# georgeliu233/STrajNet

Measured on AMD Instinct MI355X. Metric: scenes/sec (fwd+bwd, 256x256 grids), higher is better.
Workload: dtype bf16; 1 GPU; STrajNet cfg-256 train step (fwd+OGMFlow_loss+bwd+Nadam), batch 8/GPU, 8 waypoints, obs+occ+flow heads, fg_msa+fg, random-init weights; global_batch=8, grid=256x256x11, parallelism=dp1, hipgraph=True, concurrent_branch_streams=True, optimizer_in_step=True, settle_steps=40

## Files before the change

include/strajnet_hip.h:

```cpp
#ifndef STRAJNET_HIP_H
#define STRAJNET_HIP_H
#include <hip/hip_runtime_api.h>
#ifdef __cplusplus
extern "C" {
#endif

enum stj_status { STJ_OK = 0, STJ_EINVAL = -1, STJ_ELAUNCH = -2, STJ_EUNSUPPORTED = -3 };
enum stj_dtype { STJ_F32 = 0, STJ_BF16 = 1, STJ_F16 = 2 };
enum stj_act { STJ_ACT_NONE = 0, STJ_ACT_GELU = 1, STJ_ACT_ELU = 2 };
enum stj_unary { STJ_U_GELU = 1, STJ_U_ELU = 2, STJ_U_TANH_SCALE = 3 };

const char* stj_last_error(void);
int stj_abi_version(void);

int stj_gemm(const void* A, const void* B, void* C, const float* bias, const void* res, float* colsum,
             int M, int N, int K, int nb1, int nb2,
             long long sAb1, long long sAb2, long long sAm, long long sAk,
             long long sBb1, long long sBb2, long long sBk, long long sBn,
             long long sCb1, long long sCb2, long long ldc,
             long long sBias1, long long sBias2, long long sRes1, long long sRes2, long long ldres,
             int act, float alpha, int dtype, int c_f32, int accumulate, int splitk,
             int nkb, long long sAkb, long long sBkb, void* group, hipStream_t stream);
long long stj_gemm_group_workspace_bytes(void);
int stj_gemm_group_begin(void* group);
// ... 146 lines not shown
  void* dq;
  float* d_w1; float* d_gamma; float* d_beta; float* d_bias;
} stj_fgoff_args;
int stj_fgoff_supported(int H, int W, int C, int G, int dtype);
long long stj_fgoff_pack_workspace_bytes(int dtype);
int stj_fgoff_pack(const float* w, void* out, int dtype, hipStream_t stream);
int stj_fgoff_fwd(const stj_fgoff_args* a, hipStream_t stream);
int stj_fgoff_bwd(const stj_fgoff_args* a, hipStream_t stream);
int stj_fg_bias_fwd(const void* off, const float* table, float* bias, int B, int G, int Hh, int Ww, int dtype, hipStream_t stream);
int stj_fg_bias_bwd(const void* off, const float* table, const void* dbias, float* dtable, float* doff,
                    int B, int G, int Hh, int Ww, int dtype, hipStream_t stream);
int stj_fg_attn_fwd(const void* q, const void* k, const void* v, const void* off, const float* table, void* a, float* lse, int B, int G,
                    int Hh, int Ww, float scale, int dtype, hipStream_t stream);
long long stj_fg_attn_bwd_workspace_bytes(int B, int G, int Hh, int Ww);
int stj_fg_attn_bwd(const void* q, const void* k, const void* v, const void* off, const float* table, const void* a, const float* lse,
                    const void* da, void* dq, void* dk, void* dv, float* dkp, float* dvp, float* dtable, float* doff, int B, int G,
                    int Hh, int Ww, float scale, int dtype, hipStream_t stream);
int stj_fg_offset_fwd(const void* o, const void* W1, const void* W2, const float* b2, const void* qres, void* off, void* fh,
                      int B, int HW, int G, int gc, int C2, float scale, int zmajor, int dtype, hipStream_t stream);
int stj_fg_offset_bwd(const void* o, const void* off, const void* W1, const void* W2, const void* doff, const void* dfh,
                      void* dO, void* dq, void* doff_out, float* dW1, float* dW2, float* db2, int B, int HW, int G, int gc,
                      int C2, float scale, int zmajor, int dtype, hipStream_t stream);

int stj_upconv_prep(const float* W, void* Wf, void* Wd, int Cin, int Cout, int dtype, hipStream_t stream);
int stj_upconv_fold(const float* dWeff, float* dW, int Cin, int Cout, hipStream_t stream);
int stj_upconv_fwd(const void* X, const void* Wf, const float* bias, void* Y, int F, int Hi, int Wi, int Cin,
                   int Cout, int act, int dtype, hipStream_t stream);
int stj_upconv_fwd_res(const void* X, const void* Wf, const float* bias, void* Y, const void* R1, void* Y2, const void* R2, int F, int Hi,
                       int Wi, int Cin, int Cout, int dtype, hipStream_t stream);
int stj_elu_res_bwd(const void* dy, const void* dy2, const void* y, const void* r, void* dpre, void* gsum, long long n, int dtype,
                    hipStream_t stream);
int stj_skip_junction_bwd(const void* dy1, const void* dy2, const void* y, const void* r1, const void* r2, void* dpre, void* dr1,
                          void* dr2, long long n, int dtype, hipStream_t stream);
int stj_upconv_dgrad(const void* dP, const void* Wd, void* dX, const void* Xelu, int F, int Hi, int Wi, int Cin, int Cout,
                     int dtype, hipStream_t stream);
int stj_upconv_wgrad(const void* X, const void* dP, float* dWeff, float* dbias, int db_parts, int F, int Hi, int Wi, int Cin,
                     int Cout, int wg_budget, int dtype, hipStream_t stream);
int stj_outconv_fwd(const void* X, const float* W, const float* bias, float* Y, int F, int Hh, int Ww, int C, int Tn,
                    long long y_bstride, long long y_tstride, long long y_pstride, int dtype, hipStream_t stream);
int stj_outconv_pair_fwd(const void* X0, const void* X1, const float* W0, const float* W1, const float* bias0, const float* bias1,
                         float* Y, int B, int Tn, int H, int W, int C, int t_major, int dtype, hipStream_t stream);
int stj_upconv_fwd_head(const void* X, const void* Wf, const float* bias, const float* Whead, void* Z, int F, int Hi, int Wi, int Cin,
                        int Cout, int dtype, hipStream_t stream);
int stj_outconv_pair_gather(const void* Z0, const void* Z1, const float* bias0, const float* bias1, float* Y, int B, int Tn, int H, int W,
                            int t_major, int dtype, hipStream_t stream);
int stj_quantize_waypoints(const float* Y, uint8_t* Q, int B, int Tn, int H, int W, hipStream_t stream);
int stj_outconv_pair_gather_q(const void* Z0, const void* Z1, const float* bias0, const float* bias1, uint8_t* Q, int B, int Tn, int H,
                              int W, int t_major, int dtype, hipStream_t stream);
int stj_compress_sizes(int B, int Tn, int H, int W, long long* work_bytes, long long* out_capacity);
int stj_compress_waypoints(const uint8_t* Q, void* work, uint8_t* out, uint32_t* offsets, int B, int Tn, int H, int W, hipStream_t stream);
int stj_compress_waypoints_level(const uint8_t* Q, void* work, uint8_t* out, uint32_t* offsets, int B, int Tn, int H, int W, int level,
                                 hipStream_t stream);
int stj_outconv_bwd(const void* X, const float* W, const float* dY, void* dX, float* dW, float* db, int F, int Hh, int Ww,
                    int C, int Tn, long long y_bstride, long long y_tstride, long long y_pstride, int elu_in, void* ws,
                    long long ws_bytes, int dtype, hipStream_t stream);
long long stj_outconv_bwd_workspace_bytes(void);
int stj_im2col_patch(const float* src, void* dst, int B, int H, int W, int Cin, long long pix_stride, int ch_stride,
                     int dtype, hipStream_t stream);
int stj_patch_embed_supported(int Cin, int Cout, int dtype);
int stj_patch_embed_fwd(const float* src, const void* w, const float* bias, const float* gamma, const float* beta, const void* add,
                        const float* gamma2, const float* beta2, void* cols, void* pre, void* x2, void* y, float* mean, float* rstd,
                        float* mean2, float* rstd2, int B, int H, int W, int Cin, long long pix_stride, int ch_stride, int Cout,
                        float eps, int dtype, hipStream_t stream);
int stj_im2col3(const void* x, void* cols, int N, int H, int W, int G, int Cg, int dtype, hipStream_t stream);
int stj_col2im3(const void* dcols, void* dx, int N, int H, int W, int G, int Cg, int dtype, hipStream_t stream);

int stj_loss_auc_gate(const float* gt_obs, const float* gt_occ, const float* gt_flow, const float* origin,
                      int* hist, float* gate, float* auc_out, int B, int H, int W, hipStream_t stream);
int stj_loss_fwd(const float* logits, const float* gt_obs, const float* gt_occ, const float* gt_flow, const float* origin,
                 const float* gate, float* sums, float* loss, float* coef, int B, int H, int W, float ogm_w, float occ_w,
                 float flow_origin_w, float replica, int flags, hipStream_t stream);
int stj_loss_bwd(const float* logits, const float* gt_obs, const float* gt_occ, const float* gt_flow, const float* origin,
                 const float* coef, const float* upstream, float* dlogits, int B, int H, int W, int flags, hipStream_t stream);
int stj_loss_coef(const float* gt_flow, const float* gate, int* cnt, float* coef, int B, int H, int W, float ogm_w, float occ_w,
                  float flow_origin_w, float replica, int flags, hipStream_t stream);
int stj_loss_finalize(const float* sums, const float* gate, float* loss, float* coef_out, int B, int H, int W, float ogm_w,
                      float occ_w, float flow_origin_w, float replica, int flags, hipStream_t stream);
int stj_loss_gate_coef(const float* gt_obs, const float* gt_occ, const float* gt_flow, const float* origin, int* hist, float* gate,
                       float* auc_out, float* coef, int B, int H, int W, float ogm_w, float occ_w, float flow_origin_w,
                       float replica, int flags, hipStream_t stream);
int stj_loss_fwd_bwd(const float* logits, const float* gt_obs, const float* gt_occ, const float* gt_flow, const float* origin,
                     const float* gate, const float* coef_in, float* sums, float* loss, float* coef_out, float* dlogits,
                     int B, int H, int W, float ogm_w, float occ_w, float flow_origin_w, float replica, int flags, hipStream_t stream);

int stj_decode_raw(const void* src, int kind, float* dst, long long n_outer, int H, int W, int C, int y0, int x0, int Ho,
                   int Wo, float scale, hipStream_t stream);

int stj_unpack_bits(const uint32_t* bits, float* dst, long long n_total, hipStream_t stream);
int stj_unpack_sparse(const uint32_t* mask, const uint32_t* offs, const uint32_t* val_base, const float* vals, long long n_vals,
                      float* dst, int B, long long n, hipStream_t stream);

int stj_gather_bits(const uint32_t* pool, const int* idx, int N, float* dst, int B, long long n, hipStream_t stream);
int stj_gather_sparse(const uint32_t* mask, const uint32_t* offs, const long long* val_base, const float* vals, long long n_vals,
                      const int* idx, int N, float* dst, int B, long long n, hipStream_t stream);
int stj_gather_raw(const void* pool, int kind, const int* idx, int N, float* dst, int B, long long n, float scale, hipStream_t stream);

int stj_pack_bits(const uint8_t* src, const int* ok, const int* slots, int N, uint32_t* pool_words, int B, int T, int H, int W, int C, int y0,
                  int x0, int Ho, int Wo, hipStream_t stream);
int stj_pack_sparse_count(const float* src, uint32_t* offs_stage, int B, int T, int H, int W, int C, int y0, int x0, int Ho, int Wo,
                          hipStream_t stream);
int stj_pool_admit(uint32_t* offs_stage, int nblk, const long long* val_base, const int* slots, int N, int* ok, int B, int first,
                   hipStream_t stream);
int stj_pack_sparse_commit(const float* src, const uint32_t* offs_stage, const int* ok, const int* slots, int N, uint32_t* mask_pool,
                           uint32_t* offs_pool, const long long* val_base, float* vals, long long n_vals, int B, int T, int H, int W, int C,
                           int y0, int x0, int Ho, int Wo, hipStream_t stream);
int stj_pool_put_raw(const void* src, int itemsize, const int* ok, const int* slots, int N, void* pool, int B, long long n, hipStream_t stream);

int stj_pool_draw(int* perm, int N, int tail, int n_live, const uint32_t* u, int* idx, int B, hipStream_t stream);
int stj_pool_admit_packed(const uint32_t* offs_src, int nblk, long long n, const long long* src_base, const long long* val_base,
                          const int* slots, int N, int* ok, int B, int first, hipStream_t stream);
int stj_pool_put_vals(const uint32_t* vals_src, const long long* src_base, const int* ok, const int* slots, int N,
                      const long long* val_base, uint32_t* vals, long long n_vals, int B, hipStream_t stream);

int stj_agent_prep(const float* obs, const float* occ, int n_obs, int n_occ, int B, int Tn, void* x5, void* v3, int* vt, int* cmi,
                   void* cmf, int dtype, hipStream_t stream);
int stj_agent_mix_fwd(const void* enc, const void* embed, const void* cm, void* concat, void* qin, int B, int A, int C, int dtype,
                      hipStream_t stream);
int stj_agent_mix_bwd(const void* dconcat, const void* dqin, const void* cm, void* denc, void* dembed, int B, int A, int C, int dtype,
                      hipStream_t stream);
int stj_agent_sum_fwd(const void* enc, const void* value, const void* embed, void* out, int B, int A, int C, int dtype, hipStream_t stream);
int stj_agent_sum_bwd(const void* dout, void* dembed, int B, int A, int C, int dtype, hipStream_t stream);
int stj_agent_out_fwd(const void* enc, const void* value, const void* embed, const float* g0, const float* b0, const float* g1, const float* b1,
                      void* out, void* y, float* mean, float* rstd, int B, int A, int n0, int C, float eps, int dtype, hipStream_t stream);
int stj_agent_out_bwd(const void* dy, const void* out, const float* mean, const float* rstd, const float* g0, const float* g1, void* dout,
                      void* dembed, float* dg0, float* db0, float* dg1, float* db1, int B, int A, int n0, int C, int dtype, hipStream_t stream);
int stj_time_collapse(const float* W, void* Wz, long long n, int dtype, hipStream_t stream);
int stj_time_fold(const float* dWz, float* dW, long long n, hipStream_t stream);
int stj_fold_parts(float* g, const long long* idx, float* parts, long long n, hipStream_t stream);

int stj_crc32c(const void* data, long long n, unsigned int* crc);

int stj_metrics(const float* pred, const float* gt_obs, const float* gt_occ, const float* gt_flow, const float* origin,
                int* hist, float* sums, float* auc, float* out, int B, int H, int W, int pred_is_logits, int use_warp,
                hipStream_t stream);

long long stj_eval_workspace_bytes(int B, int H, int W);
int stj_eval_fwd(const float* logits, const float* gt_obs, const float* gt_occ, const float* gt_flow, const float* origin,
                 void* workspace, float* loss, float* metrics, float* gate, float* auc, double* running, int B, int H, int W,
                 float ogm_w, float occ_w, float flow_origin_w, float replica, float loss_scale, int flags, hipStream_t stream);

int stj_rng_advance(long long* state, hipStream_t stream);
int stj_rng_advance_snap(long long* state, long long* snap, hipStream_t stream);
int stj_dropout(const void* x, const void* res, void* y, long long n, long long inner, float p, const long long* state,
                int site, int dtype, hipStream_t stream);
int stj_dropout_mask(unsigned char* mask, long long ndraw, float p, const long long* state, int site, hipStream_t stream);
int stj_nadam_step(float* w, const float* g, float* m, float* v, long long n, float lr, float b1, float b2, float eps,
                   float cg, float cm, float vhat_scale, float gscale, hipStream_t stream);

enum stj_optim { STJ_GRADNORM_PARTS = 256, STJ_SCHED_CONSTANT = 0, STJ_SCHED_COSINE_RESTARTS = 1, STJ_SCHED_CUSTOM = 2,
                 STJ_NADAM_SKIP_NONFINITE = 1, STJ_TENSOR_CHUNK = 4096, STJ_TENSOR_GRID = 1024 };
int stj_gradnorm_partials(const float* g, long long n, double* partials, hipStream_t stream);
int stj_nadam_prepare(double* state, const double* sched, const double* partials, float* coef, const float* losses, double* running,
                      float b1, float b2, float gscale, float clipnorm, float loss_scale, int flags, hipStream_t stream);
int stj_nadam_apply(float* w, const float* g, float* m, float* v, long long n, const float* coef, float b1, float b2, float eps,
                    hipStream_t stream);

int stj_tensor_partials(const float* g, long long n, const int* chunks, int n_chunks, int S, double* gpart, hipStream_t stream);
int stj_nadam_prepare_tensors(double* state, const double* sched, const double* gpart, const int* chunk0, int n_chunks, int S, float* coef,
                              float* mult, double* tsum, int* nfcount, const float* losses, double* running, float b1, float b2,
                              float gscale, float global_clipnorm, float clipnorm, float loss_scale, int flags, hipStream_t stream);
int stj_nadam_apply_tensors(float* w, const float* g, float* m, float* v, long long n, const int* chunks, int n_chunks, int S,
                            const float* coef, const float* mult, float b1, float b2, float eps, hipStream_t stream);

#ifdef __cplusplus
}
#endif
#endif
```

strajnet_amd/csrc/loss.hip:

```cpp
#include "loss_pixel.h"

#define LOSS_PARTS 32
enum { S_OBS = 0, S_OCC = 1, S_L1 = 2, S_EX = 3, S_WARP = 4, S_N = 5 };

__global__ __launch_bounds__(256) void auc_hist_kernel(const float* gt_obs, const float* gt_occ, const float* gt_flow,
                                                       const float* origin, int* hist, int* cnt, int B, int H, int W) {
  __shared__ int sh[2 * 101 + 1];
  const int k = blockIdx.y;
  for (int i = threadIdx.x; i < 203; i += 256) sh[i] = 0;
  __syncthreads();
  int nex = 0;
  const long long npix = (long long)B * H * W;
  for (long long i = blockIdx.x * 256ll + threadIdx.x; i < npix; i += gridDim.x * 256ll) {
    const int x = (int)(i % W); long long t = i / W;
    const int y = (int)(t % H); const long long b = t / H;
    const long long g = ((b * NWP + k) * H + y) * W + x;
    const float ta = fminf(fmaxf(gt_obs[g] + gt_occ[g], 0.f), 1.f);
    const float* img = origin + (b * NWP + k) * (long long)H * W;
    const float fx = gt_flow[2 * g], fy = gt_flow[2 * g + 1];
    nex += (fx != 0.f || fy != 0.f) ? 1 : 0;
    const float wp = warp_sample(img, H, W, (float)x + fx, (float)y + fy, nullptr, nullptr);
    const float pred = wp * ta;
    const int bk = auc_bucket(pred);
    atomicAdd(&sh[(ta != 0.f ? 101 : 0) + bk], 1);
  }
  if (cnt) {
#pragma unroll
    for (int o = 32; o > 0; o >>= 1) nex += __shfl_xor(nex, o, 64);
    if ((threadIdx.x & 63) == 0 && nex) atomicAdd(&sh[202], nex);
  }
  __syncthreads();
  for (int i = threadIdx.x; i < 202; i += 256)
    if (sh[i]) atomicAdd(hist + k * 202 + i, sh[i]);
  if (cnt && threadIdx.x == 0 && sh[202]) atomicAdd(cnt + k, sh[202]);
}
__global__ __launch_bounds__(128) void auc_gate_kernel(const int* hist, float* gate, float* auc_out) {
  __shared__ AucScratch s;
  const int k = blockIdx.x;
  const double auc = auc_pr_block(hist + k * 202, s);
  if (threadIdx.x == 0) {
    if (gate) gate[k] = ((1.0 - auc) < 1.0) ? 1.f : 0.f;
    if (auc_out) auc_out[k] = (float)auc;
  }
}

template <bool FOCAL, bool PRED>
__global__ __launch_bounds__(256) void loss_fwd_kernel(const float* logits, const float* gt_obs, const float* gt_occ,
                                                       const float* gt_flow, const float* origin, float* sums,
                                                       int B, int H, int W, int use_warp) {
  __shared__ float red[4][NWP * S_N];
  const float inv_hw = 1.f / ((float)H * (float)W);
  float acc[S_N];
#pragma unroll
  for (int i = 0; i < S_N; ++i) acc[i] = 0.f;
  const long long nitem = (long long)B * H * W * NWP;
  const int k = threadIdx.x & 7;
  for (long long it = blockIdx.x * 256ll + threadIdx.x; it < nitem; it += gridDim.x * 256ll) {
    const long long i = it >> 3;
    const int x = (int)(i % W); long long t = i / W;
    const int y = (int)(t % H); const long long b = t / H;
    const float4 lg = reinterpret_cast<const float4*>(logits)[it];
    const long long g = ((b * NWP + k) * H + y) * W + x;
    const float to = gt_obs[g], tc = gt_occ[g];
    const float2 fl = reinterpret_cast<const float2*>(gt_flow)[g];
    const float fx = fl.x, fy = fl.y;
    acc[S_OBS] += FOCAL ? xe_focal_logits(to, lg.x, nullptr) : xe_logits(to, lg.x);
    acc[S_OCC] += FOCAL ? xe_focal_logits(tc, lg.y, nullptr) : xe_logits(tc, lg.y);
    const float ex = (fx != 0.f || fy != 0.f) ? 1.f : 0.f;
    acc[S_L1] += (fabsf(fx - lg.z) + fabsf(fy - lg.w)) * ex;
    acc[S_EX] += ex;
    if (use_warp) {
      const float* img = origin + (b * NWP + k) * (long long)H * W;
      const float wp = warp_sample(img, H, W, (float)x + lg.z, (float)y + lg.w, nullptr, nullptr);
      const float sg = PRED ? fminf(fmaxf(sigmoidf(lg.x) + sigmoidf(lg.y), 0.f), 1.f)
                            : fminf(fmaxf(sigmoidf(to) + sigmoidf(tc), 0.f), 1.f);
      const float ta = fminf(fmaxf(to + tc, 0.f), 1.f);
      acc[S_WARP] += warp_term<FOCAL, PRED>(ta, sg * wp, inv_hw, nullptr);
    }
  }
  const int lane = threadIdx.x & 63, w = threadIdx.x >> 6;
#pragma unroll
  for (int i = 0; i < S_N; ++i) {
    float v = acc[i];
    v += __shfl_xor(v, 8, 64); v += __shfl_xor(v, 16, 64); v += __shfl_xor(v, 32, 64);
    if (lane < 8) red[w][lane * S_N + i] = v;
  }
  __syncthreads();
  if (threadIdx.x < NWP * S_N)
    atomicAdd(sums + (blockIdx.x % LOSS_PARTS) * (NWP * S_N) + threadIdx.x, red[0][threadIdx.x] + red[1][threadIdx.x] + red[2][threadIdx.x] + red[3][threadIdx.x]);
}

struct LossCfg { float ogm_w, occ_w, fow, replica; int use_warp; };

__global__ void loss_finalize_kernel(const float* sums_parts, int nparts, const float* gate, float* loss, float* coef, float npix, LossCfg c) {
  __shared__ float sums[NWP * S_N], part[6][NWP * S_N];
  if (threadIdx.x < 6 * NWP * S_N) {
    const int slot = threadIdx.x % (NWP * S_N), j = threadIdx.x / (NWP * S_N);
    float a = 0.f;
#pragma unroll 8
    for (int q = j; q < nparts; q += 6) a += sums_parts[q * (NWP * S_N) + slot];
    part[j][slot] = a;
  }
  __syncthreads();
  if (threadIdx.x < NWP * S_N) {
    const int t = threadIdx.x;
    sums[t] = ((((part[0][t] + part[1][t]) + part[2][t]) + part[3][t]) + part[4][t]) + part[5][t];
  }
  __syncthreads();
  if (threadIdx.x != 0) return;
  float so = 0.f, sc = 0.f, sf = 0.f, sw = 0.f, fc = 0.f;
  for (int k = 0; k < NWP; ++k) fc += gate[k];
  for (int k = 0; k < NWP; ++k) {
    const float* s = sums + k * S_N;
    so += c.ogm_w * s[S_OBS] / (npix * c.replica);
    sc += c.occ_w * s[S_OCC] / (npix * c.replica);
    const float den = s[S_EX] * c.replica / 2.f;
    const float fl = den != 0.f ? s[S_L1] / den : 0.f;
    sf += gate[k] * fl;
    sw += gate[k] * c.fow * s[S_WARP] / (npix * c.replica);
    coef[k * 4 + 0] = c.ogm_w / (npix * c.replica) / NWP;
    coef[k * 4 + 1] = c.occ_w / (npix * c.replica) / NWP;
    coef[k * 4 + 2] = den != 0.f ? gate[k] / fc / den : 0.f;
    coef[k * 4 + 3] = c.use_warp ? gate[k] / fc * c.fow / (npix * c.replica) : 0.f;
  }
  loss[0] = so / NWP;
  loss[1] = sc / NWP;
  loss[2] = sf / fc;
  loss[3] = c.use_warp ? sw / fc : 0.f;
  loss[4] = loss[0] + loss[1] + loss[2] + loss[3];
}

template <bool FOCAL, bool PRED>
__global__ __launch_bounds__(256) void loss_bwd_kernel(const float* logits, const float* gt_obs, const float* gt_occ,
                                                       const float* gt_flow, const float* origin, const float* coef,
                                                       const float* up, float* dlogits, int B, int H, int W, int use_warp, int up1) {
  const int k = threadIdx.x & 7;
  const float c0 = coef[4 * k] * up[0], c1 = coef[4 * k + 1] * up[up1 ? 0 : 1], c2 = coef[4 * k + 2] * up[up1 ? 0 : 2], c3 = coef[4 * k + 3] * up[up1 ? 0 : 3];
  const long long nitem = (long long)B * H * W * NWP;
  const float inv_hw = 1.f / ((float)H * (float)W);
  for (long long it = blockIdx.x * 256ll + threadIdx.x; it < nitem; it += gridDim.x * 256ll) {
    const long long i = it >> 3;
    const int x = (int)(i % W); long long t = i / W;
    const int y = (int)(t % H); const long long b = t / H;
    const float4 lg = reinterpret_cast<const float4*>(logits)[it];
    const long long g = ((b * NWP + k) * H + y) * W + x;
    const float to = gt_obs[g], tc = gt_occ[g];
    const float2 fl = reinterpret_cast<const float2*>(gt_flow)[g];
    const float fx = fl.x, fy = fl.y;
    float g0, g1;
    if (FOCAL) { xe_focal_logits(to, lg.x, &g0); xe_focal_logits(tc, lg.y, &g1); }
    else { g0 = sigmoidf(lg.x) - to; g1 = sigmoidf(lg.y) - tc; }
    g0 *= c0; g1 *= c1;
    const float ex = (fx != 0.f || fy != 0.f) ? 1.f : 0.f;
    const float d0 = fx - lg.z, d1 = fy - lg.w;
    float g2 = -c2 * ex * (d0 > 0.f ? 1.f : (d0 < 0.f ? -1.f : 0.f));
    float g3 = -c2 * ex * (d1 > 0.f ? 1.f : (d1 < 0.f ? -1.f : 0.f));
    if (use_warp && c3 != 0.f) {
      const float* img = origin + (b * NWP + k) * (long long)H * W;
      float ddx, ddy;
      const float wp = warp_sample(img, H, W, (float)x + lg.z, (float)y + lg.w, &ddx, &ddy);
      const float sa = sigmoidf(PRED ? lg.x : to), sb = sigmoidf(PRED ? lg.y : tc);
      const float ssum = sa + sb;
      const float sg = fminf(fmaxf(ssum, 0.f), 1.f);
      const float ta = fminf(fmaxf(to + tc, 0.f), 1.f);
      float dq;
      warp_term<FOCAL, PRED>(ta, sg * wp, inv_hw, &dq);
      dq *= c3;
      g2 += dq * sg * ddx;
      g3 += dq * sg * ddy;
      if (PRED && ssum <= 1.f) {
        g0 += dq * wp * sa * (1.f - sa);
        g1 += dq * wp * sb * (1.f - sb);
      }
    }
    reinterpret_cast<float4*>(dlogits)[it] = make_float4(g0, g1, g2, g3);
  }
}

#define LOSS_PARTS_FUSED 128
#ifndef LOSS_FB_MAXG
#define LOSS_FB_MAXG 16384
#endif
template <bool FOCAL, bool PRED>
__global__ __launch_bounds__(256) void loss_fwd_bwd_kernel(const float* logits, const float* gt_obs, const float* gt_occ,
                                                           const float* gt_flow, const float* origin, const float* coef,
                                                           float* sums, float* dlogits, int B, int H, int W, int use_warp) {
  __shared__ float red[4][NWP * S_N];
  const float inv_hw = 1.f / ((float)H * (float)W);
  float acc[S_N];
#pragma unroll
  for (int i = 0; i < S_N; ++i) acc[i] = 0.f;
  const long long nitem = (long long)B * H * W * NWP;
  const int k = threadIdx.x & 7;
  const float c0 = coef[4 * k], c1 = coef[4 * k + 1], c2 = coef[4 * k + 2], c3 = coef[4 * k + 3];
  for (long long it = blockIdx.x * 256ll + threadIdx.x; it < nitem; it += gridDim.x * 256ll) {
    const long long i = it >> 3;
    const int x = (int)(i % W); long long t = i / W;
    const int y = (int)(t % H); const long long b = t / H;
    const float4 lg = reinterpret_cast<const float4*>(logits)[it];
    const long long g = ((b * NWP + k) * H + y) * W + x;
    const float to = gt_obs[g], tc = gt_occ[g];
    const float2 fl = reinterpret_cast<const float2*>(gt_flow)[g];
    const float fx = fl.x, fy = fl.y;
    float g0, g1;
    if (FOCAL) { acc[S_OBS] += xe_focal_logits(to, lg.x, &g0); acc[S_OCC] += xe_focal_logits(tc, lg.y, &g1); }
    else {
      acc[S_OBS] += xe_logits(to, lg.x); acc[S_OCC] += xe_logits(tc, lg.y);
      g0 = sigmoidf(lg.x) - to; g1 = sigmoidf(lg.y) - tc;
    }
    g0 *= c0; g1 *= c1;
    const float ex = (fx != 0.f || fy != 0.f) ? 1.f : 0.f;
    const float d0 = fx - lg.z, d1 = fy - lg.w;
    acc[S_L1] += (fabsf(d0) + fabsf(d1)) * ex;
    acc[S_EX] += ex;
    float g2 = -c2 * ex * (d0 > 0.f ? 1.f : (d0 < 0.f ? -1.f : 0.f));
    float g3 = -c2 * ex * (d1 > 0.f ? 1.f : (d1 < 0.f ? -1.f : 0.f));
    if (use_warp) {
      const float* img = origin + (b * NWP + k) * (long long)H * W;
      float ddx, ddy;
      const float wp = warp_sample(img, H, W, (float)x + lg.z, (float)y + lg.w, &ddx, &ddy);
      const float sa = sigmoidf(PRED ? lg.x : to), sb = sigmoidf(PRED ? lg.y : tc);
      const float ssum = sa + sb;
      const float sg = fminf(fmaxf(ssum, 0.f), 1.f);
      const float ta = fminf(fmaxf(to + tc, 0.f), 1.f);
      float dq;
      acc[S_WARP] += warp_term<FOCAL, PRED>(ta, sg * wp, inv_hw, &dq);
      if (c3 != 0.f) {
        dq *= c3;
        g2 += dq * sg * ddx;
        g3 += dq * sg * ddy;
        if (PRED && ssum <= 1.f) {
          g0 += dq * wp * sa * (1.f - sa);
          g1 += dq * wp * sb * (1.f - sb);
        }
      }
    }
    reinterpret_cast<float4*>(dlogits)[it] = make_float4(g0, g1, g2, g3);
  }
  const int lane = threadIdx.x & 63, w = threadIdx.x >> 6;
#pragma unroll
  for (int i = 0; i < S_N; ++i) {
    float v = acc[i];
    v += __shfl_xor(v, 8, 64); v += __shfl_xor(v, 16, 64); v += __shfl_xor(v, 32, 64);
    if (lane < 8) red[w][lane * S_N + i] = v;
  }
  __syncthreads();
  if (threadIdx.x < NWP * S_N)
    atomicAdd(sums + (blockIdx.x % LOSS_PARTS_FUSED) * (NWP * S_N) + threadIdx.x, red[0][threadIdx.x] + red[1][threadIdx.x] + red[2][threadIdx.x] + red[3][threadIdx.x]);
}

template <bool VEC4>
__global__ __launch_bounds__(256) void loss_flow_count_kernel(const float* gt_flow, int* cnt, long long plane) {
  __shared__ int red[4];
  const int k = blockIdx.y % NWP;
  const float* fp = gt_flow + (long long)blockIdx.y * plane * 2;
  int n = 0;
  if (VEC4) {
    const float4* f = reinterpret_cast<const float4*>(fp);
    for (long long i = blockIdx.x * 256ll + threadIdx.x; i < plane / 2; i += gridDim.x * 256ll) {
      const float4 v = f[i];
      n += ((v.x != 0.f || v.y != 0.f) ? 1 : 0) + ((v.z != 0.f || v.w != 0.f) ? 1 : 0);
    }
  } else {
    const float2* f = reinterpret_cast<const float2*>(fp);
    for (long long i = blockIdx.x * 256ll + threadIdx.x; i < plane; i += gridDim.x * 256ll) {
      const float2 v = f[i];
      n += (v.x != 0.f || v.y != 0.f) ? 1 : 0;
    }
  }
#pragma unroll
  for (int o = 32; o > 0; o >>= 1) n += __shfl_xor(n, o, 64);
  if ((threadIdx.x & 63) == 0) red[threadIdx.x >> 6] = n;
  __syncthreads();
  if (threadIdx.x == 0) { const int s = red[0] + red[1] + red[2] + red[3]; if (s) atomicAdd(cnt + k, s); }
}
__global__ void loss_coef_kernel(const int* cnt, const float* gate, float* coef, float npix, LossCfg c) {
  if (threadIdx.x != 0) return;
  float fc = 0.f;
  for (int k = 0; k < NWP; ++k) fc += gate[k];
  for (int k = 0; k < NWP; ++k) {
    const float den = (float)cnt[k] * c.replica / 2.f;
    coef[k * 4 + 0] = c.ogm_w / (npix * c.replica) / NWP;
    coef[k * 4 + 1] = c.occ_w / (npix * c.replica) / NWP;
    coef[k * 4 + 2] = den != 0.f ? gate[k] / fc / den : 0.f;
    coef[k * 4 + 3] = c.use_warp ? gate[k] / fc * c.fow / (npix * c.replica) : 0.f;
  }
}

extern "C" int stj_loss_auc_gate(const float* gt_obs, const float* gt_occ, const float* gt_flow, const float* origin,
                                 int* hist, float* gate, float* auc_out, int B, int H, int W, hipStream_t stream) {
  const long long npix = (long long)B * H * W;
  const int gx = (int)min(256ll, (npix + 255) / 256);
  hipLaunchKernelGGL(auc_hist_kernel, dim3(gx, NWP), dim3(256), 0, stream, gt_obs, gt_occ, gt_flow, origin, hist, (int*)nullptr, B, H, W);
  hipLaunchKernelGGL(auc_gate_kernel, dim3(NWP), dim3(128), 0, stream, hist, gate, auc_out);
  return stj_check_launch("stj_loss_auc_gate");
}
extern "C" int stj_loss_fwd(const float* logits, const float* gt_obs, const float* gt_occ, const float* gt_flow, const float* origin,
                            const float* gate, float* sums, float* loss, float* coef, int B, int H, int W, float ogm_w, float occ_w,
                            float flow_origin_w, float replica, int flags, hipStream_t stream) {
  if (((uintptr_t)logits) & 15) { stj_set_error("loss: logits must be 16-byte aligned"); return STJ_EINVAL; }
  if (((uintptr_t)gt_flow) & 7) { stj_set_error("loss: gt_flow must be 8-byte aligned"); return STJ_EINVAL; }
  if (flags & ~7) { stj_set_error("loss: unknown flag bits %d", flags); return STJ_EINVAL; }
  const long long npix = (long long)B * H * W;
  const int gx = (int)min(4096ll, (npix * NWP + 255) / 256);
  const int use_warp = flags & 1, focal = (flags >> 1) & 1, pred = (flags >> 2) & 1;
#define LOSS_FWD(FO, PR) hipLaunchKernelGGL((loss_fwd_kernel<FO, PR>), dim3(gx), dim3(256), 0, stream, logits, gt_obs, gt_occ, gt_flow, origin, sums, B, H, W, use_warp)
  if (focal && pred) LOSS_FWD(true, true); else if (focal) LOSS_FWD(true, false); else if (pred) LOSS_FWD(false, true); else LOSS_FWD(false, false);
#undef LOSS_FWD
  LossCfg c; c.ogm_w = ogm_w; c.occ_w = occ_w; c.fow = flow_origin_w; c.replica = replica; c.use_warp = use_warp;
  hipLaunchKernelGGL(loss_finalize_kernel, dim3(1), dim3(256), 0, stream, sums, LOSS_PARTS, gate, loss, coef, (float)npix, c);
  return stj_check_launch("stj_loss_fwd");
}
extern "C" int stj_loss_bwd(const float* logits, const float* gt_obs, const float* gt_occ, const float* gt_flow, const float* origin,
                            const float* coef, const float* upstream, float* dlogits, int B, int H, int W, int flags, hipStream_t stream) {
  if (flags & ~15) { stj_set_error("loss: unknown flag bits %d", flags); return STJ_EINVAL; }
  if ((((uintptr_t)logits) | ((uintptr_t)dlogits)) & 15) { stj_set_error("loss: logits / dlogits must be 16-byte aligned"); return STJ_EINVAL; }
  if (((uintptr_t)gt_flow) & 7) { stj_set_error("loss: gt_flow must be 8-byte aligned"); return STJ_EINVAL; }
  const long long npix = (long long)B * H * W;
  const int gx = (int)min(8192ll, (npix * NWP + 255) / 256);
  const int use_warp = flags & 1, focal = (flags >> 1) & 1, pred = (flags >> 2) & 1;
#define LOSS_BWD(FO, PR) hipLaunchKernelGGL((loss_bwd_kernel<FO, PR>), dim3(gx), dim3(256), 0, stream, logits, gt_obs, gt_occ, gt_flow, origin, coef, upstream, dlogits, B, H, W, use_warp, (flags >> 3) & 1)
  if (focal && pred) LOSS_BWD(true, true); else if (focal) LOSS_BWD(true, false); else if (pred) LOSS_BWD(false, true); else LOSS_BWD(false, false);
#undef LOSS_BWD
  return stj_check_launch("stj_loss_bwd");
}

extern "C" int stj_loss_coef(const float* gt_flow, const float* gate, int* cnt, float* coef, int B, int H, int W, float ogm_w, float occ_w,
                             float flow_origin_w, float replica, int flags, hipStream_t stream) {
  if (((uintptr_t)gt_flow) & 7) { stj_set_error("loss: gt_flow must be 8-byte aligned"); return STJ_EINVAL; }
  if (flags & ~7) { stj_set_error("loss: unknown flag bits %d", flags); return STJ_EINVAL; }
  const long long plane = (long long)H * W;
  if (B > 0 && plane > 0) {
    const int gx = (int)min(16ll, (plane / 2 + 255) / 256);
    if (plane % 2 == 0 && (((uintptr_t)gt_flow) & 15) == 0)
      hipLaunchKernelGGL(loss_flow_count_kernel<true>, dim3(gx, B * NWP), dim3(256), 0, stream, gt_flow, cnt, plane);
    else
      hipLaunchKernelGGL(loss_flow_count_kernel<false>, dim3(gx, B * NWP), dim3(256), 0, stream, gt_flow, cnt, plane);
  }
  LossCfg c; c.ogm_w = ogm_w; c.occ_w = occ_w; c.fow = flow_origin_w; c.replica = replica; c.use_warp = flags & 1;
  hipLaunchKernelGGL(loss_coef_kernel, dim3(1), dim3(64), 0, stream, cnt, gate, coef, (float)((long long)B * H * W), c);
  return stj_check_launch("stj_loss_coef");
}
extern "C" int stj_loss_gate_coef(const float* gt_obs, const float* gt_occ, const float* gt_flow, const float* origin, int* hist, float* gate,
                                  float* auc_out, float* coef, int B, int H, int W, float ogm_w, float occ_w, float flow_origin_w,
                                  float replica, int flags, hipStream_t stream) {
  if (flags & ~7) { stj_set_error("loss: unknown flag bits %d", flags); return STJ_EINVAL; }
  const long long npix = (long long)B * H * W;
  const int gx = (int)min(256ll, (npix + 255) / 256);
  int* cnt = hist + NWP * 202;
  if (gx > 0) hipLaunchKernelGGL(auc_hist_kernel, dim3(gx, NWP), dim3(256), 0, stream, gt_obs, gt_occ, gt_flow, origin, hist, cnt, B, H, W);
  hipLaunchKernelGGL(auc_gate_kernel, dim3(NWP), dim3(128), 0, stream, hist, gate, auc_out);
  LossCfg c; c.ogm_w = ogm_w; c.occ_w = occ_w; c.fow = flow_origin_w; c.replica = replica; c.use_warp = flags & 1;
  hipLaunchKernelGGL(loss_coef_kernel, dim3(1), dim3(64), 0, stream, cnt, gate, coef, (float)npix, c);
  return stj_check_launch("stj_loss_gate_coef");
}
extern "C" int stj_loss_fwd_bwd(const float* logits, const float* gt_obs, const float* gt_occ, const float* gt_flow, const float* origin,
                                const float* gate, const float* coef_in, float* sums, float* loss, float* coef_out, float* dlogits,
                                int B, int H, int W, float ogm_w, float occ_w, float flow_origin_w, float replica, int flags,
                                hipStream_t stream) {
  if ((((uintptr_t)logits) | ((uintptr_t)dlogits)) & 15) { stj_set_error("loss: logits / dlogits must be 16-byte aligned"); return STJ_EINVAL; }
  if (((uintptr_t)gt_flow) & 7) { stj_set_error("loss: gt_flow must be 8-byte aligned"); return STJ_EINVAL; }
  if (flags & ~7) { stj_set_error("loss: unknown flag bits %d", flags); return STJ_EINVAL; }
  const long long npix = (long long)B * H * W;
  const int gx = (int)min((long long)LOSS_FB_MAXG, (npix * NWP + 255) / 256);
  const int use_warp = flags & 1, focal = (flags >> 1) & 1, pred = (flags >> 2) & 1;
  if (gx > 0) {
#define LOSS_FB(FO, PR) hipLaunchKernelGGL((loss_fwd_bwd_kernel<FO, PR>), dim3(gx), dim3(256), 0, stream, logits, gt_obs, gt_occ, gt_flow, origin, coef_in, sums, dlogits, B, H, W, use_warp)
    if (focal && pred) LOSS_FB(true, true); else if (focal) LOSS_FB(true, false); else if (pred) LOSS_FB(false, true); else LOSS_FB(false, false);
#undef LOSS_FB
  }
  if (loss == nullptr) return stj_check_launch("stj_loss_fwd_bwd");
  LossCfg c; c.ogm_w = ogm_w; c.occ_w = occ_w; c.fow = flow_origin_w; c.replica = replica; c.use_warp = use_warp;
  hipLaunchKernelGGL(loss_finalize_kernel, dim3(1), dim3(256), 0, stream, sums, LOSS_PARTS_FUSED, gate, loss, coef_out, (float)npix, c);
  return stj_check_launch("stj_loss_fwd_bwd");
}
extern "C" int stj_loss_finalize(const float* sums, const float* gate, float* loss, float* coef_out, int B, int H, int W, float ogm_w,
                                 float occ_w, float flow_origin_w, float replica, int flags, hipStream_t stream) {
  if (flags & ~7) { stj_set_error("loss: unknown flag bits %d", flags); return STJ_EINVAL; }
  LossCfg c; c.ogm_w = ogm_w; c.occ_w = occ_w; c.fow = flow_origin_w; c.replica = replica; c.use_warp = flags & 1;
  hipLaunchKernelGGL(loss_finalize_kernel, dim3(1), dim3(256), 0, stream, sums, LOSS_PARTS_FUSED, gate, loss, coef_out, (float)((long long)B * H * W), c);
  return stj_check_launch("stj_loss_finalize");
}


enum { M_IO = 0, M_TO, M_PO, M_IC, M_TC, M_PC, M_EPE, M_EX, M_IW, M_TW, M_PW, M_N };
__global__ __launch_bounds__(256) void metrics_kernel(const float* pred, const float* gt_obs, const float* gt_occ, const float* gt_flow,
                                                      const float* origin, int* hist, float* sums, int B, int H, int W,
                                                      int pred_is_logits, int use_warp) {
  __shared__ int sh[3 * 202];
  __shared__ float red[4][M_N];
  const int k = blockIdx.y;
  for (int i = threadIdx.x; i < 3 * 202; i += 256) sh[i] = 0;
  __syncthreads();
  float acc[M_N];
#pragma unroll
  for (int i = 0; i < M_N; ++i) acc[i] = 0.f;
  const long long npix = (long long)B * H * W;
  for (long long i = blockIdx.x * 256ll + threadIdx.x; i < npix; i += gridDim.x * 256ll) {
    const int x = (int)(i % W); long long t = i / W;
    const int y = (int)(t % H); const long long b = t / H;
    const float4 q = reinterpret_cast<const float4*>(pred + i * 32)[k];
    const float po = pred_is_logits ? sigmoidf(q.x) : q.x, pc = pred_is_logits ? sigmoidf(q.y) : q.y;
    const long long g = ((b * NWP + k) * H + y) * W + x;
    const float to = gt_obs[g], tc = gt_occ[g];
    const float fx = gt_flow[2 * g], fy = gt_flow[2 * g + 1];
    atomicAdd(&sh[0 * 202 + (to != 0.f ? 101 : 0) + auc_bucket(po)], 1);
    atomicAdd(&sh[1 * 202 + (tc != 0.f ? 101 : 0) + auc_bucket(pc)], 1);
    acc[M_IO] += po * to; acc[M_TO] += to; acc[M_PO] += po;
    acc[M_IC] += pc * tc; acc[M_TC] += tc; acc[M_PC] += pc;
    const float ex = (fx != 0.f || fy != 0.f) ? 1.f : 0.f;
    const float dx = (fx - q.z) * ex, dy = (fy - q.w) * ex;
    acc[M_EPE] += sqrtf(dx * dx + dy * dy);
    acc[M_EX] += ex;
    if (use_warp) {
      const float* img = origin + (b * NWP + k) * (long long)H * W;
      const float wp = warp_sample(img, H, W, (float)x + q.z, (float)y + q.w, nullptr, nullptr);
      const float ta = fminf(fmaxf(to + tc, 0.f), 1.f);
      const float fg = fminf(fmaxf(po + pc, 0.f), 1.f) * wp;
      atomicAdd(&sh[2 * 202 + (fg != 0.f ? 101 : 0) + auc_bucket(ta)], 1);
      acc[M_IW] += ta * fg; acc[M_TW] += fg; acc[M_PW] += ta;
    }
  }
  const int lane = threadIdx.x & 63, w = threadIdx.x >> 6;
#pragma unroll
  for (int i = 0; i < M_N; ++i) {
    const float s = wave_sum(acc[i]);
    if (lane == 0) red[w][i] = s;
  }
  __syncthreads();
  if (threadIdx.x < M_N) atomicAdd(sums + k * M_N + threadIdx.x, red[0][threadIdx.x] + red[1][threadIdx.x] + red[2][threadIdx.x] + red[3][threadIdx.x]);
  for (int i = threadIdx.x; i < 3 * 202; i += 256)
    if (sh[i]) atomicAdd(hist + (k * 3 + i / 202) * 202 + i % 202, sh[i]);
}
__global__ void metrics_finalize_kernel(const float* auc, const float* sums, float* out, int use_warp) {
  if (threadIdx.x != 0) return;
  float m[7] = {0.f, 0.f, 0.f, 0.f, 0.f, 0.f, 0.f};
  for (int k = 0; k < NWP; ++k) {
    const float* s = sums + k * M_N;
    auto iou = [](float i, float t, float p) { const float d = p + t - i; return d != 0.f ? i / d : 0.f; };
    m[0] += auc[k * 3 + 0]; m[1] += auc[k * 3 + 1];
    m[2] += iou(s[M_IO], s[M_TO], s[M_PO]); m[3] += iou(s[M_IC], s[M_TC], s[M_PC]);
    m[4] += s[M_EX] != 0.f ? s[M_EPE] / s[M_EX] : 0.f;
    if (use_warp) { m[5] += auc[k * 3 + 2]; m[6] += iou(s[M_IW], s[M_TW], s[M_PW]); }
  }
  for (int i = 0; i < 7; ++i) out[i] = m[i] / NWP;
}
extern "C" int stj_metrics(const float* pred, const float* gt_obs, const float* gt_occ, const float* gt_flow, const float* origin,
                           int* hist, float* sums, float* auc, float* out, int B, int H, int W, int pred_is_logits, int use_warp,
                           hipStream_t stream) {
  if (((uintptr_t)pred) & 15) { stj_set_error("metrics: pred must be 16-byte aligned"); return STJ_EINVAL; }
  const long long npix = (long long)B * H * W;
  if (npix <= 0) return STJ_OK;
  const int gx = (int)min(256ll, (npix + 255) / 256);
  hipLaunchKernelGGL(metrics_kernel, dim3(gx, NWP), dim3(256), 0, stream, pred, gt_obs, gt_occ, gt_flow, origin, hist, sums, B, H, W, pred_is_logits, use_warp);
  hipLaunchKernelGGL(auc_gate_kernel, dim3(NWP * 3), dim3(128), 0, stream, hist, (float*)nullptr, auc);
  hipLaunchKernelGGL(metrics_finalize_kernel, dim3(1), dim3(64), 0, stream, auc, sums, out, use_warp);
  return stj_check_launch("stj_metrics");
// ... 2 lines not shown
```

strajnet_amd/csrc/nadam.h:

```cpp
#pragma once

__device__ __forceinline__ void nadam_update(float& w, float g, float& m, float& v, float lr, float b1, float b2, float eps, float cg,
                                             float cm, float vhat_scale, float gscale) {
  const float gg = g * gscale;
  m = b1 * m + (1.f - b1) * gg;
  v = b2 * v + (1.f - b2) * gg * gg;
  w -= lr * (cg * gg + cm * m) / (sqrtf(v * vhat_scale) + eps);
}
```

strajnet_amd/csrc/optim.hip:

```cpp
#include "common.h"
#include "nadam.h"
#include "optim_dev.h"

#define GRADNORM_THREADS 512
static_assert(STJ_GRADNORM_PARTS == 256, "nadam_prepare_kernel folds one partial per thread of its 256");

__global__ __launch_bounds__(GRADNORM_THREADS) void gradnorm_partials_kernel(const float* __restrict__ g, long long n,
                                                                             double* __restrict__ partials) {
  __shared__ double red[GRADNORM_THREADS / 64];
  const long long nv = n / 4;
  double s = 0.0;
#pragma unroll 4
  for (long long i = blockIdx.x * (long long)GRADNORM_THREADS + threadIdx.x; i < nv; i += gridDim.x * (long long)GRADNORM_THREADS) {
    const float4 G = reinterpret_cast<const float4*>(g)[i];
    s += (double)G.x * (double)G.x + (double)G.y * (double)G.y + (double)G.z * (double)G.z + (double)G.w * (double)G.w;
  }
  if (blockIdx.x == 0 && threadIdx.x < (n & 3)) {
    const double x = g[nv * 4 + threadIdx.x];
    s += x * x;
  }
  s = block_sum_f64<GRADNORM_THREADS / 64>(s, red);
  if (threadIdx.x == 0) partials[blockIdx.x] = s;
}

__global__ __launch_bounds__(256) void nadam_prepare_kernel(double* __restrict__ state, const double* __restrict__ sched,
                                                            const double* __restrict__ partials, float* __restrict__ coef,
                                                            const float* __restrict__ losses, double* __restrict__ running, PrepareCfg c) {
  __shared__ double red[4];
  double sumsq = 0.0;
  if (partials) sumsq = block_sum_f64<4>(partials[threadIdx.x], red);
  if (threadIdx.x != 0) return;
  nadam_prepare_step(state, sched, coef, losses, running, c, partials != nullptr, sumsq);
}

__global__ __launch_bounds__(256) void nadam_apply_kernel(float* __restrict__ w, const float* __restrict__ g, float* __restrict__ m,
                                                          float* __restrict__ v, long long n, const float* __restrict__ coef, float b1,
                                                          float b2, float eps) {
  if (coef[5] == 0.f) return;
  const float lr = coef[0], cg = coef[1], cm = coef[2], vhat_scale = coef[3], gscale = coef[4];
  const long long nv = n / 4;
  for (long long i = blockIdx.x * 256ll + threadIdx.x; i < nv; i += gridDim.x * 256ll) {
    float4 W = reinterpret_cast<float4*>(w)[i], G = reinterpret_cast<const float4*>(g)[i];
    float4 M = reinterpret_cast<float4*>(m)[i], V = reinterpret_cast<float4*>(v)[i];
    float* wp = &W.x; float* gp = &G.x; float* mp = &M.x; float* vp = &V.x;
#pragma unroll
    for (int e = 0; e < 4; ++e) nadam_update(wp[e], gp[e], mp[e], vp[e], lr, b1, b2, eps, cg, cm, vhat_scale, gscale);
    reinterpret_cast<float4*>(w)[i] = W; reinterpret_cast<float4*>(m)[i] = M; reinterpret_cast<float4*>(v)[i] = V;
  }
  if (blockIdx.x == 0 && threadIdx.x < (n & 3)) {
    const long long i = nv * 4 + threadIdx.x;
    nadam_update(w[i], g[i], m[i], v[i], lr, b1, b2, eps, cg, cm, vhat_scale, gscale);
  }
}

extern "C" int stj_gradnorm_partials(const float* g, long long n, double* partials, hipStream_t stream) {
  if (n < 0) { stj_set_error("stj_gradnorm_partials: n must not be negative (got %lld)", n); return STJ_EINVAL; }
  if (!partials || (n > 0 && !g)) { stj_set_error("stj_gradnorm_partials: null pointer"); return STJ_EINVAL; }
  if (((uintptr_t)g) & 15) { stj_set_error("stj_gradnorm_partials: g must be 16-byte aligned"); return STJ_EINVAL; }
  if (((uintptr_t)partials) & 7) { stj_set_error("stj_gradnorm_partials: partials must be 8-byte aligned"); return STJ_EINVAL; }
  hipLaunchKernelGGL(gradnorm_partials_kernel, dim3(STJ_GRADNORM_PARTS), dim3(GRADNORM_THREADS), 0, stream, g, n, partials);
  return stj_check_launch("stj_gradnorm_partials");
}

extern "C" int stj_nadam_prepare(double* state, const double* sched, const double* partials, float* coef, const float* losses,
                                 double* running, float b1, float b2, float gscale, float clipnorm, float loss_scale, int flags,
                                 hipStream_t stream) {
  if (!state || !sched || !coef) { stj_set_error("stj_nadam_prepare: state, sched and coef must not be null"); return STJ_EINVAL; }
  if ((losses == nullptr) != (running == nullptr)) { stj_set_error("stj_nadam_prepare: losses and running go together"); return STJ_EINVAL; }
  if (((uintptr_t)state | (uintptr_t)sched | (uintptr_t)partials | (uintptr_t)running) & 7) {
    stj_set_error("stj_nadam_prepare: state, sched, partials and running must be 8-byte aligned"); return STJ_EINVAL;
  }
  if (((uintptr_t)coef) & 15) { stj_set_error("stj_nadam_prepare: coef must be 16-byte aligned"); return STJ_EINVAL; }
  if (((uintptr_t)losses) & 3) { stj_set_error("stj_nadam_prepare: losses must be 4-byte aligned"); return STJ_EINVAL; }
  if (flags & ~STJ_NADAM_SKIP_NONFINITE) { stj_set_error("stj_nadam_prepare: unknown flag bits %d", flags); return STJ_EINVAL; }
  PrepareCfg c; c.b1 = b1; c.b2 = b2; c.gscale = gscale; c.clipnorm = clipnorm; c.loss_scale = loss_scale; c.flags = flags;
  hipLaunchKernelGGL(nadam_prepare_kernel, dim3(1), dim3(256), 0, stream, state, sched, partials, coef, losses, running, c);
  return stj_check_launch("stj_nadam_prepare");
}

extern "C" int stj_nadam_apply(float* w, const float* g, float* m, float* v, long long n, const float* coef, float b1, float b2, float eps,
                               hipStream_t stream) {
  if (n < 0) { stj_set_error("stj_nadam_apply: n must not be negative (got %lld)", n); return STJ_EINVAL; }
  if (n == 0) return STJ_OK;
  if (!w || !g || !m || !v || !coef) { stj_set_error("stj_nadam_apply: null pointer"); return STJ_EINVAL; }
  if ((((uintptr_t)w) | ((uintptr_t)g) | ((uintptr_t)m) | ((uintptr_t)v) | ((uintptr_t)coef)) & 15) {
    stj_set_error("stj_nadam_apply: buffers must be 16-byte aligned"); return STJ_EINVAL;
  }
  long long b = (n / 4 + 255) / 256;
  const int grid = (int)(b < 1 ? 1 : (b > 4096 ? 4096 : b));
  hipLaunchKernelGGL(nadam_apply_kernel, dim3(grid), dim3(256), 0, stream, w, g, m, v, n, coef, b1, b2, eps);
  return stj_check_launch("stj_nadam_apply");
}
```

strajnet_amd/csrc/rng.hip:

```cpp
#include "common.h"
#include "nadam.h"
#include "rng.h"

template <typename T>
__global__ __launch_bounds__(256) void dropout_elem_kernel(const T* __restrict__ x, const T* __restrict__ res, T* __restrict__ y,
                                                           long long n, float p, float scale, const long long* __restrict__ state, int site) {
  const long long ng = (n + 3) / 4;
  for (long long gi = blockIdx.x * 256ll + threadIdx.x; gi < ng; gi += gridDim.x * 256ll) {
    bool k[4];
    keep4(state, site, gi, p, k);
#pragma unroll
    for (int e = 0; e < 4; ++e) {
      const long long i = gi * 4 + e;
      if (i < n) {
        float v = k[e] ? ldf(x + i) * scale : 0.f;
        if (res) v += ldf(res + i);
        stf(y + i, v);
      }
    }
  }
}
template <typename T>
__global__ __launch_bounds__(256) void dropout_group_kernel(const T* __restrict__ x, const T* __restrict__ res, T* __restrict__ y,
                                                            long long n, long long inner, float p, float scale,
// ... 16 lines not shown
  for (long long vi = blockIdx.x * 256ll + threadIdx.x; vi < nv; vi += gridDim.x * 256ll) {
    float v[VN], r[VN];
    ld16(x + vi * VN, v);
    if (res) ld16(res + vi * VN, r);
    bool k[VN];
    if constexpr (GROUP) {
      const long long d = vi * VN / inner;
      bool k4[4];
      keep4(state, site, d >> 2, p, k4);
#pragma unroll
      for (int e = 0; e < VN; ++e) k[e] = k4[d & 3];
    } else {
#pragma unroll
      for (int q = 0; q < VN / 4; ++q) keep4(state, site, vi * (VN / 4) + q, p, k + 4 * q);
    }
#pragma unroll
    for (int e = 0; e < VN; ++e) v[e] = (k[e] ? v[e] * scale : 0.f) + (res ? r[e] : 0.f);
    st16(y + vi * VN, v);
  }
}
__global__ __launch_bounds__(256) void dropout_mask_kernel(unsigned char* mask, long long ndraw, float p, const long long* state, int site) {
  const long long ng = (ndraw + 3) / 4;
  for (long long gi = blockIdx.x * 256ll + threadIdx.x; gi < ng; gi += gridDim.x * 256ll) {
    bool k[4];
    keep4(state, site, gi, p, k);
#pragma unroll
    for (int e = 0; e < 4; ++e)
      if (gi * 4 + e < ndraw) mask[gi * 4 + e] = k[e] ? 1 : 0;
  }
}
__global__ void rng_advance_kernel(long long* state) { state[1] += 1; }

static inline int rng_grid(long long n) {
  long long b = (n + 255) / 256;
  return (int)(b < 1 ? 1 : (b > 8192 ? 8192 : b));
}

extern "C" int stj_rng_advance(long long* state, hipStream_t stream) {
  hipLaunchKernelGGL(rng_advance_kernel, dim3(1), dim3(1), 0, stream, state);
  return stj_check_launch("stj_rng_advance");
}
__global__ void rng_advance_snap_kernel(long long* state, long long* snap) { const long long s = state[1] + 1; state[1] = s; snap[0] = state[0]; snap[1] = s; }
extern "C" int stj_rng_advance_snap(long long* state, long long* snap, hipStream_t stream) {
  if (!state || !snap) { stj_set_error("stj_rng_advance_snap: null pointer"); return STJ_EINVAL; }
  hipLaunchKernelGGL(rng_advance_snap_kernel, dim3(1), dim3(1), 0, stream, state, snap);
  return stj_check_launch("stj_rng_advance_snap");
}
extern "C" int stj_dropout(const void* x, const void* res, void* y, long long n, long long inner, float p, const long long* state,
                           int site, int dtype, hipStream_t stream) {
  if (n <= 0) return STJ_OK;
  if (!(p >= 0.f && p < 1.f) || inner < 1 || !state) { stj_set_error("stj_dropout: need 0 <= p < 1, inner >= 1, state != NULL"); return STJ_EINVAL; }
  const float scale = 1.0f / (1.0f - p);
  const int vn = stj_vec_elems(dtype);
  const bool vec = n % vn == 0 && (inner == 1 || inner % vn == 0) && !((((uintptr_t)x) | ((uintptr_t)res) | ((uintptr_t)y)) & 15);
  bool known;
  if (vec) {
    const int g = rng_grid(n / vn);
    known = stj_with_dtype(dtype, [&](auto t) { typedef typename decltype(t)::type T;
      if (inner == 1) hipLaunchKernelGGL((dropout_vec_kernel<T, false>), dim3(g), dim3(256), 0, stream, (const T*)x, (const T*)res, (T*)y, n, inner, p, scale, state, site);
      else hipLaunchKernelGGL((dropout_vec_kernel<T, true>), dim3(g), dim3(256), 0, stream, (const T*)x, (const T*)res, (T*)y, n, inner, p, scale, state, site);
    });
  } else if (inner == 1) {
    const int g = rng_grid((n + 3) / 4);
    known = stj_with_dtype(dtype, [&](auto t) { typedef typename decltype(t)::type T;
      hipLaunchKernelGGL(dropout_elem_kernel<T>, dim3(g), dim3(256), 0, stream, (const T*)x, (const T*)res, (T*)y, n, p, scale, state, site);
    });
  } else {
    const int g = rng_grid(n);
    known = stj_with_dtype(dtype, [&](auto t) { typedef typename decltype(t)::type T;
      hipLaunchKernelGGL(dropout_group_kernel<T>, dim3(g), dim3(256), 0, stream, (const T*)x, (const T*)res, (T*)y, n, inner, p, scale, state, site);
    });
  }
  if (!known) { stj_set_error("stj_dropout: bad dtype %d", dtype); return STJ_EINVAL; }
  return stj_check_launch("stj_dropout");
}
extern "C" int stj_dropout_mask(unsigned char* mask, long long ndraw, float p, const long long* state, int site, hipStream_t stream) {
  if (ndraw <= 0) return STJ_OK;
  hipLaunchKernelGGL(dropout_mask_kernel, dim3(rng_grid((ndraw + 3) / 4)), dim3(256), 0, stream, mask, ndraw, p, state, site);
  return stj_check_launch("stj_dropout_mask");
}

__global__ __launch_bounds__(256) void nadam_kernel(float* __restrict__ w, const float* __restrict__ g, float* __restrict__ m,
                                                    float* __restrict__ v, long long n, float lr, float b1, float b2, float eps,
                                                    float cg, float cm, float vhat_scale, float gscale) {
  const long long nv = n / 4;
  for (long long i = blockIdx.x * 256ll + threadIdx.x; i < nv; i += gridDim.x * 256ll) {
    float4 W = reinterpret_cast<float4*>(w)[i], G = reinterpret_cast<const float4*>(g)[i];
    float4 M = reinterpret_cast<float4*>(m)[i], V = reinterpret_cast<float4*>(v)[i];
    float* wp = &W.x; float* gp = &G.x; float* mp = &M.x; float* vp = &V.x;
#pragma unroll
    for (int e = 0; e < 4; ++e) nadam_update(wp[e], gp[e], mp[e], vp[e], lr, b1, b2, eps, cg, cm, vhat_scale, gscale);
    reinterpret_cast<float4*>(w)[i] = W; reinterpret_cast<float4*>(m)[i] = M; reinterpret_cast<float4*>(v)[i] = V;
  }
  if (blockIdx.x == 0 && threadIdx.x < (n & 3)) {
    const long long i = nv * 4 + threadIdx.x;
    nadam_update(w[i], g[i], m[i], v[i], lr, b1, b2, eps, cg, cm, vhat_scale, gscale);
  }
}
extern "C" int stj_nadam_step(float* w, const float* g, float* m, float* v, long long n, float lr, float b1, float b2, float eps,
                              float cg, float cm, float vhat_scale, float gscale, hipStream_t stream) {
  if (n <= 0) return STJ_OK;
  if ((((uintptr_t)w) | ((uintptr_t)g) | ((uintptr_t)m) | ((uintptr_t)v)) & 15) { stj_set_error("stj_nadam_step: buffers must be 16-byte aligned"); return STJ_EINVAL; }
  long long b = (n / 4 + 255) / 256;
  const int grid = (int)(b < 1 ? 1 : (b > 4096 ? 4096 : b));
  hipLaunchKernelGGL(nadam_kernel, dim3(grid), dim3(256), 0, stream, w, g, m, v, n, lr, b1, b2, eps, cg, cm, vhat_scale, gscale);
  return stj_check_launch("stj_nadam_step");
}
```

strajnet_amd/csrc/util.hip:

```cpp
#include "common.h"
#include "rawcast.h"
#include <stdarg.h>
#include <stdio.h>
#include <stdlib.h>
#include <string.h>

static thread_local char g_err[512] = "";

void stj_set_error(const char* fmt, ...) {
  va_list ap;
  va_start(ap, fmt);
  vsnprintf(g_err, sizeof(g_err), fmt, ap);
  va_end(ap);
}
int stj_check_launch(const char* what) {
  hipError_t e = hipGetLastError();
  if (e != hipSuccess) {
    stj_set_error("%s: launch failed: %s", what, hipGetErrorString(e));
    return STJ_ELAUNCH;
  }
  return STJ_OK;
}
extern "C" const char* stj_last_error(void) { return g_err; }
bool stj_no_ws() {
// ... 174 lines not shown

template <typename T>
__global__ __launch_bounds__(256) void maxpool_fwd_kernel(const T* x, T* y, int* idx, long long outer, int Tn, int C) {
  for (long long i = blockIdx.x * 256ll + threadIdx.x; i < outer * C; i += gridDim.x * 256ll) {
    long long o = i / C; int c = (int)(i % C);
    float best = -INFINITY; int bi = 0;
    for (int t = 0; t < Tn; ++t) {
      float v = ldf(x + (o * Tn + t) * C + c);
      if (v > best) { best = v; bi = t; }
    }
    stf(y + i, best);
    idx[i] = bi;
  }
}
template <typename T>
__global__ __launch_bounds__(256) void maxpool_bwd_kernel(const T* dy, const T* x, const T* y, T* dx, long long outer, int Tn, int C) {
  for (long long i = blockIdx.x * 256ll + threadIdx.x; i < outer * C; i += gridDim.x * 256ll) {
    long long o = i / C; int c = (int)(i % C);
    const float m = ldf(y + i), g = ldf(dy + i);
    int cnt = 0;
    for (int t = 0; t < Tn; ++t) cnt += ldf(x + (o * Tn + t) * C + c) == m ? 1 : 0;
    const float gg = g / (float)(cnt > 0 ? cnt : 1);
    for (int t = 0; t < Tn; ++t) stf(dx + (o * Tn + t) * C + c, ldf(x + (o * Tn + t) * C + c) == m ? gg : 0.f);
  }
}
extern "C" int stj_maxpool_fwd(const void* x, void* y, int* idx, long long outer, int Tn, int C, int dtype, hipStream_t stream) {
  if (outer <= 0) return STJ_OK;
  int g = ew_grid(outer * C);
  if (!stj_with_dtype(dtype, [&](auto t) { typedef typename decltype(t)::type T;
        hipLaunchKernelGGL(maxpool_fwd_kernel<T>, dim3(g), dim3(256), 0, stream, (const T*)x, (T*)y, idx, outer, Tn, C);
      })) { stj_set_error("stj_maxpool_fwd: bad dtype %d", dtype); return STJ_EINVAL; }
  return stj_check_launch("stj_maxpool_fwd");
}
extern "C" int stj_maxpool_bwd(const void* dy, const void* x, const void* y, void* dx, long long outer, int Tn, int C, int dtype, hipStream_t stream) {
  if (outer <= 0) return STJ_OK;
  int g = ew_grid(outer * C);
  if (!stj_with_dtype(dtype, [&](auto t) { typedef typename decltype(t)::type T;
        hipLaunchKernelGGL(maxpool_bwd_kernel<T>, dim3(g), dim3(256), 0, stream, (const T*)dy, (const T*)x, (const T*)y, (T*)dx, outer, Tn, C);
      })) { stj_set_error("stj_maxpool_bwd: bad dtype %d", dtype); return STJ_EINVAL; }
  return stj_check_launch("stj_maxpool_bwd");
}

template <int KIND>
__global__ __launch_bounds__(256) void decode_raw_kernel(const void* __restrict__ src, float* __restrict__ dst, long long n_out, int H, int W,
                                                         int C, int y0, int x0, int Ho, int Wo, float scale) {
  for (long long i = blockIdx.x * 256ll + threadIdx.x; i < n_out; i += gridDim.x * 256ll) {
    const int c = (int)(i % C); long long t = i / C;
    const int x = (int)(t % Wo); t /= Wo;
    const int y = (int)(t % Ho); const long long n = t / Ho;
    const long long s = ((n * H + y0 + y) * W + x0 + x) * C + c;
    dst[i] = raw_to_f32<KIND>(src, s) * scale;
  }
}
extern "C" int stj_decode_raw(const void* src, int kind, float* dst, long long n_outer, int H, int W, int C, int y0, int x0, int Ho,
                              int Wo, float scale, hipStream_t stream) {
  if (n_outer <= 0) return STJ_OK;
  if (kind < 0 || kind > 3 || y0 < 0 || x0 < 0 || y0 + Ho > H || x0 + Wo > W || C <= 0) { stj_set_error("stj_decode_raw: bad kind / crop"); return STJ_EINVAL; }
  const long long n_out = n_outer * Ho * Wo * C;
  const int g = ew_grid(n_out);
  if (kind == 0) hipLaunchKernelGGL(decode_raw_kernel<0>, dim3(g), dim3(256), 0, stream, src, dst, n_out, H, W, C, y0, x0, Ho, Wo, scale);
  else if (kind == 1) hipLaunchKernelGGL(decode_raw_kernel<1>, dim3(g), dim3(256), 0, stream, src, dst, n_out, H, W, C, y0, x0, Ho, Wo, scale);
  else if (kind == 2) hipLaunchKernelGGL(decode_raw_kernel<2>, dim3(g), dim3(256), 0, stream, src, dst, n_out, H, W, C, y0, x0, Ho, Wo, scale);
  else hipLaunchKernelGGL(decode_raw_kernel<3>, dim3(g), dim3(256), 0, stream, src, dst, n_out, H, W, C, y0, x0, Ho, Wo, scale);
  return stj_check_launch("stj_decode_raw");
}

template <typename T>
__global__ __launch_bounds__(256) void time_collapse_kernel(const float* __restrict__ W, T* __restrict__ Wz, long long n) {
  for (long long i = blockIdx.x * 256ll + threadIdx.x; i < n; i += gridDim.x * 256ll) {
    float w[8];
#pragma unroll
    for (int j = 0; j < 8; ++j) w[j] = W[j * n + i];
#pragma unroll
    for (int t = 0; t < 8; ++t) {
      float a = 0.f;
#pragma unroll
      for (int j = 0; j < 8; ++j)
        if (j >= 3 - t && j <= 10 - t) a += w[j];
      stf(Wz + t * n + i, a);
    }
  }
}
__global__ __launch_bounds__(256) void time_fold_kernel(const float* __restrict__ dWz, float* __restrict__ dW, long long n) {
  for (long long i = blockIdx.x * 256ll + threadIdx.x; i < n; i += gridDim.x * 256ll) {
    float g[8];
#pragma unroll
    for (int t = 0; t < 8; ++t) g[t] = dWz[t * n + i];
#pragma unroll
    for (int j = 0; j < 8; ++j) {
      float a = 0.f;
#pragma unroll
      for (int t = 0; t < 8; ++t)
        if (j >= 3 - t && j <= 10 - t) a += g[t];
      dW[j * n + i] += a;
    }
  }
}
template <typename T>
__global__ __launch_bounds__(256) void agent_prep_kernel(const float* __restrict__ obs, const float* __restrict__ occ, int n_obs, int n_occ, int B,
                                                         int Tn, T* __restrict__ x5, T* __restrict__ v3, int* __restrict__ vt,
                                                         int* __restrict__ cmi, T* __restrict__ cmf) {
  const int A = n_obs + n_occ;
  for (int it = blockIdx.x * 256 + threadIdx.x; it < B * A * Tn; it += gridDim.x * 256) {
    const int i = it / Tn, t = it % Tn;
    const int b = i / A, a = i % A;
    const float* src = a < n_obs ? obs + ((long long)b * n_obs + a) * Tn * 8 : occ + ((long long)b * n_occ + (a - n_obs)) * Tn * 8;
    const float4 lo = *reinterpret_cast<const float4*>(src + t * 8), hi = *reinterpret_cast<const float4*>(src + t * 8 + 4);
    T* o = x5 + (long long)it * 5;
    stf(o, lo.x); stf(o + 1, lo.y); stf(o + 2, lo.z); stf(o + 3, lo.w); stf(o + 4, hi.x);
    vt[it] = lo.x != 0.f;
    if (t == 0) {
      stf(v3 + i * 3, hi.y); stf(v3 + i * 3 + 1, hi.z); stf(v3 + i * 3 + 2, hi.w);
      int any = 0;
      for (int u = 0; u < Tn; ++u) any |= src[u * 8] != 0.f;
      cmi[i] = any;
      stf(cmf + i, any ? 1.f : 0.f);
    }
  }
}
template <typename T>
__global__ __launch_bounds__(256) void agent_mix_fwd_kernel(const T* __restrict__ enc, const T* __restrict__ embed, const T* __restrict__ cm,
                                                            T* __restrict__ concat, T* __restrict__ qin, int B, int A, int C) {
  const long long n = (long long)B * A * C;
  for (long long i = blockIdx.x * 256ll + threadIdx.x; i < n; i += gridDim.x * 256ll) {
    const int c = (int)(i % C); const long long ba = i / C; const int a = (int)(ba % A);
    T t;
    stf(&t, ldf(enc + i) * ldf(cm + ba));
    concat[i] = t;
    stf(qin + i, ldf(&t) + ldf(embed + (long long)a * C + c));
  }
}
template <typename T>
__global__ __launch_bounds__(256) void agent_mix_bwd_kernel(const T* __restrict__ dconcat, const T* __restrict__ dqin, const T* __restrict__ cm,
                                                            T* __restrict__ denc, T* __restrict__ dembed, int B, int A, int C) {
  for (int j = blockIdx.x * 256 + threadIdx.x; j < A * C; j += gridDim.x * 256) {
    const int a = j / C;
    float s = 0.f;
    for (int b = 0; b < B; ++b) {
      const long long i = (long long)b * A * C + j;
      const float dq = dqin ? ldf(dqin + i) : 0.f;
      s += dq;
      stf(denc + i, ((dconcat ? ldf(dconcat + i) : 0.f) + dq) * ldf(cm + (long long)b * A + a));
    }
    if (dembed) stf(dembed + j, s);
  }
}
template <typename T>
__global__ __launch_bounds__(256) void agent_sum_fwd_kernel(const T* __restrict__ enc, const T* __restrict__ value, const T* __restrict__ embed,
                                                            T* __restrict__ out, int B, int A, int C) {
  const long long n = (long long)B * A * C;
  for (long long i = blockIdx.x * 256ll + threadIdx.x; i < n; i += gridDim.x * 256ll) {
    T t;
    stf(&t, ldf(enc + i) + ldf(value + i));
    stf(out + i, ldf(&t) + ldf(embed + i % ((long long)A * C)));
  }
}
template <typename T>
__global__ __launch_bounds__(256) void agent_sum_bwd_kernel(const T* __restrict__ dout, T* __restrict__ dembed, int B, int A, int C) {
  for (int j = blockIdx.x * 256 + threadIdx.x; j < A * C; j += gridDim.x * 256) {
    float s = 0.f;
    for (int b = 0; b < B; ++b) s += ldf(dout + (long long)b * A * C + j);
    stf(dembed + j, s);
  }
}
extern "C" int stj_agent_prep(const float* obs, const float* occ, int n_obs, int n_occ, int B, int Tn, void* x5, void* v3, int* vt, int* cmi,
                              void* cmf, int dtype, hipStream_t stream) {
// ... 101 lines not shown
#pragma unroll
  for (int j = 0; j < NJ; ++j)
#pragma unroll
    for (int e = 0; e < 2; ++e) { de[j][e] = dg[j][e] = db[j][e] = 0.f; gv[j][e] = gm[128 * j + 2 * lane + e]; }
  for (int b = 0; b < B; ++b) {
    const long long row = (long long)b * A + a;
    const float mu = mean[row], rs = rstd[row];
    float xh[NJ][2], t[NJ][2];
    float s1 = 0.f, s2 = 0.f;
#pragma unroll
    for (int j = 0; j < NJ; ++j)
#pragma unroll
      for (int e = 0; e < 2; ++e) {
        const int c = 128 * j + 2 * lane + e;
        const float d = ldf(dy + row * C + c);
        xh[j][e] = (ldf(out + row * C + c) - mu) * rs;
        dg[j][e] += d * xh[j][e];
        db[j][e] += d;
        t[j][e] = d * gv[j][e];
        s1 += t[j][e]; s2 += t[j][e] * xh[j][e];
      }
#pragma unroll
    for (int o = 32; o > 0; o >>= 1) { s1 += __shfl_xor(s1, o, 64); s2 += __shfl_xor(s2, o, 64); }
    s1 *= (1.f / C); s2 *= (1.f / C);
#pragma unroll
    for (int j = 0; j < NJ; ++j)
#pragma unroll
      for (int e = 0; e < 2; ++e) {
        const int c = 128 * j + 2 * lane + e;
        T r;
        stf(&r, rs * (t[j][e] - s1 - xh[j][e] * s2));
        dout[row * C + c] = r;
        de[j][e] += ldf(&r);
      }
  }
  float* dgp = a < n0 ? dg0 : dg1;
  float* dbp = a < n0 ? db0 : db1;
#pragma unroll
  for (int j = 0; j < NJ; ++j)
#pragma unroll
    for (int e = 0; e < 2; ++e) {
      const int c = 128 * j + 2 * lane + e;
      stf(dembed + (long long)a * C + c, de[j][e]);
      atomicAdd(dgp + c, dg[j][e]);
      atomicAdd(dbp + c, db[j][e]);
    }
}
extern "C" int stj_agent_out_fwd(const void* enc, const void* value, const void* embed, const float* g0, const float* b0, const float* g1,
                                 const float* b1, void* out, void* y, float* mean, float* rstd, int B, int A, int n0, int C, float eps, int dtype,
                                 hipStream_t stream) {
  if ((long long)B * A <= 0) return STJ_OK;
  if (C != 384 || n0 < 0 || n0 > A) { stj_set_error("stj_agent_out_fwd: C must be 384 and 0 <= n0 <= A (got C = %d, n0 = %d)", C, n0); return STJ_EUNSUPPORTED; }
  const int g = (B * A + 3) / 4;
  if (!stj_with_dtype(dtype, [&](auto t) { typedef typename decltype(t)::type T;
        hipLaunchKernelGGL((agent_out_fwd_kernel<T, 3>), dim3(g), dim3(256), 0, stream, (const T*)enc, (const T*)value, (const T*)embed, g0, b0, g1, b1, (T*)out, (T*)y, mean, rstd, B, A, n0, eps);
      })) { stj_set_error("stj_agent_out_fwd: bad dtype %d", dtype); return STJ_EINVAL; }
  return stj_check_launch("stj_agent_out_fwd");
}
extern "C" int stj_agent_out_bwd(const void* dy, const void* out, const float* mean, const float* rstd, const float* g0, const float* g1, void* dout,
                                 void* dembed, float* dg0, float* db0, float* dg1, float* db1, int B, int A, int n0, int C, int dtype,
                                 hipStream_t stream) {
  if ((long long)B * A <= 0) return STJ_OK;
  if (C != 384 || n0 < 0 || n0 > A) { stj_set_error("stj_agent_out_bwd: C must be 384 and 0 <= n0 <= A (got C = %d, n0 = %d)", C, n0); return STJ_EUNSUPPORTED; }
  const int g = (A + 3) / 4;
  if (!stj_with_dtype(dtype, [&](auto t) { typedef typename decltype(t)::type T;
        hipLaunchKernelGGL((agent_out_bwd_kernel<T, 3>), dim3(g), dim3(256), 0, stream, (const T*)dy, (const T*)out, mean, rstd, g0, g1, (T*)dout, (T*)dembed, dg0, db0, dg1, db1, B, A, n0);
      })) { stj_set_error("stj_agent_out_bwd: bad dtype %d", dtype); return STJ_EINVAL; }
  return stj_check_launch("stj_agent_out_bwd");
}

extern "C" int stj_time_collapse(const float* W, void* Wz, long long n, int dtype, hipStream_t stream) {
  if (n <= 0) return STJ_OK;
  const int g = ew_grid(n);
  if (!stj_with_dtype(dtype, [&](auto t) { typedef typename decltype(t)::type T;
        hipLaunchKernelGGL(time_collapse_kernel<T>, dim3(g), dim3(256), 0, stream, W, (T*)Wz, n);
      })) { stj_set_error("stj_time_collapse: bad dtype %d", dtype); return STJ_EINVAL; }
  return stj_check_launch("stj_time_collapse");
}
extern "C" int stj_time_fold(const float* dWz, float* dW, long long n, hipStream_t stream) {
  if (n <= 0) return STJ_OK;
  hipLaunchKernelGGL(time_fold_kernel, dim3(ew_grid(n)), dim3(256), 0, stream, dWz, dW, n);
  return stj_check_launch("stj_time_fold");
}

__global__ __launch_bounds__(256) void fold_parts_kernel(float* __restrict__ g, const long long* __restrict__ idx, float* __restrict__ parts, long long n) {
  for (long long i = blockIdx.x * 256ll + threadIdx.x; i < n; i += gridDim.x * 256ll) {
    const float v = parts[i];
    parts[i] = 0.f;
    if (v != 0.f) atomicAdd(g + idx[i], v);
  }
}
extern "C" int stj_fold_parts(float* g, const long long* idx, float* parts, long long n, hipStream_t stream) {
  if (n <= 0) return STJ_OK;
  if (!g || !idx || !parts) { stj_set_error("stj_fold_parts: null pointer"); return STJ_EINVAL; }
  hipLaunchKernelGGL(fold_parts_kernel, dim3(ew_grid(n)), dim3(256), 0, stream, g, idx, parts, n);
  return stj_check_launch("stj_fold_parts");
}

namespace {
struct Crc32cTables {
  uint32_t t[8][256];
  Crc32cTables() {
    for (uint32_t i = 0; i < 256; i++) {
      uint32_t c = i;
      for (int k = 0; k < 8; k++) c = (c & 1) ? (c >> 1) ^ 0x82F63B78u : c >> 1;
      t[0][i] = c;
    }
    for (uint32_t i = 0; i < 256; i++)
      for (int s = 1; s < 8; s++) t[s][i] = (t[s - 1][i] >> 8) ^ t[0][t[s - 1][i] & 0xFF];
  }
};
}
extern "C" int stj_crc32c(const void* data, long long n, unsigned int* crc) {
  if (!crc || (n > 0 && !data) || n < 0) { stj_set_error("stj_crc32c: null pointer / negative size"); return STJ_EINVAL; }
  static const Crc32cTables T;
  const unsigned char* p = (const unsigned char*)data;
  uint32_t c = ~*crc;
  while (n > 0 && ((uintptr_t)p & 7)) { c = T.t[0][(c ^ *p++) & 0xFF] ^ (c >> 8); n--; }
  while (n >= 8) {
    uint64_t w;
    memcpy(&w, p, 8);
    w ^= c;
    c = T.t[7][w & 0xFF] ^ T.t[6][(w >> 8) & 0xFF] ^ T.t[5][(w >> 16) & 0xFF] ^ T.t[4][(w >> 24) & 0xFF] ^
        T.t[3][(w >> 32) & 0xFF] ^ T.t[2][(w >> 40) & 0xFF] ^ T.t[1][(w >> 48) & 0xFF] ^ T.t[0][w >> 56];
    p += 8; n -= 8;
  }
  while (n-- > 0) c = T.t[0][(c ^ *p++) & 0xFF] ^ (c >> 8);
  *crc = ~c;
  return STJ_OK;
}
```

strajnet_amd/graph.py:

```python
import torch

from . import ops
from .loss import get_pred_waypoint_logits, warpped_gt


class GraphedTrainStep:

    def __init__(self, model, loss_fn, batch, warmup=2, training=True, split=False, keep_graph=False, optimizer=None):
        if optimizer is not None and split:
            raise ValueError('GraphedTrainStep: optimizer= cannot be captured with split=True (the update must follow the all-reduce, '
                             'which stays outside the graph): call optimizer.step() after sync.head_and_wait()')
        if optimizer is not None and not getattr(optimizer, 'capturable', False):
            raise ValueError('GraphedTrainStep: optimizer= needs an optimizer whose step() is launches only (optim.DeviceNadam); a '
                             'host-state optimizer\'s coefficients would freeze at capture time')
        self.model, self.loss_fn, self.training, self.split, self.optimizer = model, loss_fn, training, split, optimizer
        self.static = {k: v.clone() for k, v in batch.items()}
        self.graph = self.graph_b = None
        self._side = None
        self.losses = None
        self._one = torch.ones((), dtype=torch.float32, device=next(iter(batch.values())).device)
        if hasattr(loss_fn, 'unit_grad'):
            loss_fn.unit_grad = self._one
        if split:
            model.cut_encoder = True
        trained = optimizer.tensors() if optimizer is not None else []
        snap = [t.clone() for t in trained]
        side = ops.role_stream(torch.cuda.current_device(), 'warmup')
        side.wait_stream(torch.cuda.current_stream())
        with torch.cuda.stream(side):
            for _ in range(warmup):
                self._eager()
                if split:
                    model.backward_encoder()
            for t, s in zip(trained, snap):
                t.copy_(s)
            if trained:
                model._sync_compute_weights()
        torch.cuda.current_stream().wait_stream(side)
        torch.cuda.synchronize()
        g = torch.cuda.CUDAGraph(keep_graph=True) if keep_graph else torch.cuda.CUDAGraph()
        with torch.cuda.graph(g, capture_error_mode='thread_local'):
            self.losses = self._eager()
        self.graph = g
        if split:
            gb = torch.cuda.CUDAGraph()
            with torch.cuda.graph(gb, pool=g.pool(), capture_error_mode='thread_local'):
                model.backward_encoder()
            self.graph_b = gb

    def _eager(self):
        x, m = self.static, self.model
        m.zero_grad()
        tw = warpped_gt(x['gt_obs'], x['gt_occ'], x['gt_flow'], x['origin_flow'])
        main = torch.cuda.current_stream()
        if hasattr(self.loss_fn, 'prepare'):
            if self._side is None:
                self._side = ops.role_stream(torch.cuda.current_device(), 'loss_prep')

            def prepare():
                self._side.wait_stream(torch.cuda.current_stream())
                with torch.cuda.stream(self._side):
                    self.loss_fn.prepare(tw)
            m.mid_forward_hook = prepare
        try:
            out = m(x['ogm'], x['map_img'], training=self.training, obs=x['obs'], occ=x['occ'], mapt=x.get('mapt'), flow=x['flow'])
        finally:
            m.mid_forward_hook = None
        if self._side is not None:
            main.wait_stream(self._side)
        d = self.loss_fn(get_pred_waypoint_logits(out), tw, None)
        total = d.total
        total.backward(self._one)
        self.total = total.detach()
        if self.optimizer is not None:
            if self.optimizer.loss_scale is not None:
                self.optimizer.attach_loss_means(d.packed, self.optimizer.loss_scale)
            self.optimizer.step()
        return d.packed

    def load(self, batch):
        for k, v in batch.items():
            if k in self.static:
                self.static[k].copy_(v, non_blocking=True)

    def __call__(self, batch=None, between=None):
        if batch is not None:
            self.load(batch)
        self.graph.replay()
        if self.graph_b is not None:
            if between is not None:
                between()
            self.graph_b.replay()
        return self.losses


class GraphedForward:

    def __init__(self, model, batch, warmup=2, pipeline_agents=False, quantized=False, compressed=False, compress_level=1):
        if compressed and not quantized:
            raise ValueError('GraphedForward: compressed=True compresses the quantised output: pass quantized=True with it')
        if compress_level not in (1, 2):
            raise ValueError(f'GraphedForward: compress_level 1 or 2, got {compress_level!r}')
        self.compress_level = compress_level
        self.model = model
        self.quantized = quantized
        self.compressed = compressed
        self.static = {k: v.clone() for k, v in batch.items() if k in ('ogm', 'map_img', 'obs', 'occ', 'flow')}
        self.pipeline_agents = pipeline_agents
        self._prefetched = False
        self._staged = None
        self._weights_seen = -1
        side = ops.role_stream(torch.cuda.current_device(), 'warmup')
        side.wait_stream(torch.cuda.current_stream())
        with torch.cuda.stream(side), torch.no_grad():
            for _ in range(warmup):
                self._eager()
        torch.cuda.current_stream().wait_stream(side)
        torch.cuda.synchronize()
        if pipeline_agents:
            self.agent_stream = model._streams[0] if model._streams[0] is not None else ops.role_stream(torch.cuda.current_device(), 'side')
            self.agent_done, self.agent_free = torch.cuda.Event(), torch.cuda.Event()
            with torch.no_grad():
                self.agent_next = model.agent_encode(self.static['obs'], self.static['occ'])
            self.agent_cur = tuple(t.clone() for t in self.agent_next)
            torch.cuda.synchronize()
            model.agent_override = self.agent_cur
        try:
            self.graph = torch.cuda.CUDAGraph()
            with torch.no_grad(), torch.cuda.graph(self.graph, capture_error_mode='thread_local'):
                self.out = self._eager()
        finally:
            model.agent_override = None
        if pipeline_agents:
            self.agent_free.record(torch.cuda.current_stream())

    def _eager(self):
        x = self.static
        if self.compressed:
            return self.model.predict_compressed(x['ogm'], x['map_img'], obs=x['obs'], occ=x['occ'], mapt=None, flow=x['flow'],
                                                 level=self.compress_level)
        if self.quantized:
            return self.model.predict_quantized(x['ogm'], x['map_img'], obs=x['obs'], occ=x['occ'], mapt=None, flow=x['flow'])
        return self.model(x['ogm'], x['map_img'], training=False, obs=x['obs'], occ=x['occ'], mapt=None, flow=x['flow'])

    def prefetch_agents(self, batch=None, ready=None):
        if not self.pipeline_agents:
            return
        st = self.agent_stream
        st.wait_event(self.agent_free)
        if batch is not None:
            if ready is not None:
                st.wait_event(ready)
            else:
                st.wait_stream(torch.cuda.current_stream())
        if self._staged is not None:
            st.wait_event(self._staged)
            self._staged = None
        with torch.cuda.stream(st):
            if batch is not None:
                for k in ('obs', 'occ'):
                    if k in batch:
                        self.static[k].copy_(batch[k], non_blocking=True)
                        batch[k].record_stream(st)
            with torch.no_grad():
                self.agent_next = self.model.agent_encode(self.static['obs'], self.static['occ'], cast=False)
            self.agent_done.record(st)
        self._prefetched = True
        self._weights_seen = self.model.weights_version

    def __call__(self, batch=None, next_batch=None):
        main = torch.cuda.current_stream()
        if self.pipeline_agents and self._prefetched and self._weights_seen != self.model.weights_version:
            self._prefetched = False
        if self.pipeline_agents and not self._prefetched:
            self.model._sync_compute_weights()
            self.agent_stream.wait_stream(main)
            self.prefetch_agents(batch)
        if batch is not None:
            for k, v in batch.items():
                if k in self.static and not (self.pipeline_agents and k in ('obs', 'occ')):
                    self.static[k].copy_(v, non_blocking=True)
        if self.pipeline_agents:
            main.wait_event(self.agent_done)
            for d, s_ in zip(self.agent_cur, self.agent_next):
                d.copy_(s_, non_blocking=True)
            self.agent_free.record(main)
            self._prefetched = False
            if next_batch is not None:
                for k in ('obs', 'occ'):
                    if k in next_batch:
                        self.static[k].copy_(next_batch[k], non_blocking=True)
                self._staged = torch.cuda.Event()
                self._staged.record(main)
        self.graph.replay()
        if self.pipeline_agents and next_batch is not None:
            self.prefetch_agents()
        return self.out


class GraphedEvalStep:

    KEYS = ('ogm', 'map_img', 'obs', 'occ', 'flow', 'gt_obs', 'gt_occ', 'gt_flow', 'origin_flow')

    def __init__(self, model, loss_fn, batch, warmup=2, no_warp=False):
        from .evaluate import eval_loss_metrics
        self._pass = eval_loss_metrics
        self.model, self.loss_fn, self.no_warp = model, loss_fn, no_warp
        self.static = {k: v.clone() for k, v in batch.items() if k in self.KEYS}
        dev = self.static['ogm'].device
        self.running = torch.zeros(12, dtype=torch.float64, device=dev)
        B, H, W = self.static['gt_obs'].shape[0], self.static['gt_obs'].shape[2], self.static['gt_obs'].shape[3]
        self._ws = ops.eval_workspace(B, H, W, dev)
        side = ops.role_stream(torch.cuda.current_device(), 'warmup')
        side.wait_stream(torch.cuda.current_stream())
        with torch.cuda.stream(side), torch.no_grad():
            for _ in range(warmup):
                self._eager()
        torch.cuda.current_stream().wait_stream(side)
        torch.cuda.synchronize()
        self.running.zero_()
        torch.cuda.synchronize()
        self.graph = torch.cuda.CUDAGraph()
        with torch.no_grad(), torch.cuda.graph(self.graph, capture_error_mode='thread_local'):
            self.logits, self.losses, self.metrics = self._eager()

    def _eager(self):
        x = self.static
        out = self.model(x['ogm'], x['map_img'], training=False, obs=x['obs'], occ=x['occ'], mapt=None, flow=x['flow'])
        d, m = self._pass(self.loss_fn, get_pred_waypoint_logits(out), warpped_gt(x['gt_obs'], x['gt_occ'], x['gt_flow'], x['origin_flow']),
                          no_warp=self.no_warp, running=self.running, workspace=self._ws)
        return out, d.packed, m.values

    def load(self, batch):
        for k, v in batch.items():
            if k in self.static:
                self.static[k].copy_(v, non_blocking=True)

    def __call__(self, batch=None):
        if batch is not None:
            self.load(batch)
        self.graph.replay()
        return self.losses, self.metrics

    def result(self):
        from .evaluate import LOSS_KEYS, METRIC_KEYS
        r = self.running.tolist()
        n = r[0]
        keys = LOSS_KEYS + (METRIC_KEYS[:5] if self.no_warp else METRIC_KEYS)
        return {k: (v / n if n else 0.0) for k, v in zip(keys, r[1:])}

    def reset(self):
        self.running.zero_()
```

strajnet_amd/modules.py:

```python
import math
import os
from collections import OrderedDict

import numpy as np
import torch

from . import ops
from .ops import Param, ACT_NONE, ACT_ELU


def _param_spec(cfg, hb, fg_msa, fg):
    C, ws, heads, depths = cfg['embed_dim'], cfg['window_size'], cfg['num_heads'], cfg['depths']
    sp = OrderedDict()

    def add(name, shape, init):
        assert name not in sp
        sp[name] = (tuple(shape), init)

    def dense(n, i, o, bias=True):
        add(n + '/kernel', (i, o), 'glorot')
        if bias:
            add(n + '/bias', (o,), 'zeros')

    def conv(n, kh, kw, i, o, bias=True):
# ... 153 lines not shown
        self._zstride = offs['cross_attn_obs1/norm1/gamma'] - offs['cross_attn_obs0/norm1/gamma']
        for n in spec:
            if n.startswith('cross_attn_obs0/'):
                for z in range(1, 8):
                    assert offs[n.replace('obs0', f'obs{z}')] - offs[n] == z * self._zstride
        self._flat = torch.zeros(off, dtype=torch.float32, device=self.device)
        self._goff8 = (off + ops._ZeroArena.ALIGN - 1) // ops._ZeroArena.ALIGN * ops._ZeroArena.ALIGN
        self._gbuf = torch.zeros(self._goff8 + ops._ZeroArena.FLOATS, dtype=torch.float32, device=self.device)
        self._gflat = self._gbuf[:off]
        self._cflat = self._flat if dtype == torch.float32 else torch.zeros(off, dtype=dtype, device=self.device)
        gen = torch.Generator().manual_seed(seed)
        dpr = np.linspace(0.0, 0.1, sum(cfg['depths']))
        self.drop_path_rate = {}
        for i, d in enumerate(cfg['depths']):
            for j in range(d):
                self.drop_path_rate[f'layers{i}/blocks{j}'] = float(dpr[sum(cfg['depths'][:i]) + j])
        for j in range(cfg['depths'][0]):
            self.drop_path_rate[f'flow_layers0/blocks{j}'] = float(dpr[j])
        self._seg_onehot = {}
        self.dropctx = ops.DropCtx(self.device, seed if dropout_seed is None else dropout_seed)
        self._arena = ops._ZeroArena()
        self._arena.adopt(self._gbuf[self._goff8:])
        self._dctx = None
        self._side = ops.role_stream(self.device, 'side') if (self.device.type == 'cuda' and os.environ.get('STJ_NO_SIDE_STREAM') != '1') else None
        self._side2 = ops.role_stream(self.device, 'side2') if (self._side is not None and os.environ.get('STJ_NO_SIDE_STREAM') != '2') else None
        self._streams = (self._side, self._side2)
        self.serial = False
        self.taps = None
        self.fused_mlp = self.fused_attn = os.environ.get('STJ_FUSED_SWIN', '1') != '0'
        self.fused_attn_dims = (96, 192, 384)
        self.fused_mlp_dims = (96, 192, 384)
        self.fused_xattn = True
        self.fused_stem = True
        self.agent_override = None
        self._quantize_heads = False
        self.mid_forward_hook = None
        self.fused_fgattn = True
        self.fused_agent = True
        self.fused_agent_int = True
        self.fused_quantize = True
        self.fused_fgoff = True
        self._agent_pack = None
        self._agent_pack_event = None
        self._agent_pack_stale = True
        self._fgoff_pack = None
        self._fgoff_pack_event = None
        self._fgoff_pack_stale = True
        self._xattn_pack = None
        self.params = OrderedDict()
        for n, (s, kind) in spec.items():
            k = int(np.prod(s))
            sl = slice(offs[n], offs[n] + k)
            self._flat[sl] = _init_tensor(s, kind, gen).reshape(-1).to(self.device)
            master = self._flat[sl].view(s).requires_grad_(True)
            grad = self._gflat[sl].view(s)
            master.grad = grad
            self.params[n] = Param(n, s, master, self._cflat[sl].view(s), grad)
        def wants_parts(n):
            leaf = n.rsplit('/', 1)[-1]
            if n.startswith('cross_attn_obs'):
                return False
            return leaf in ('gamma', 'beta', 'relative_position_bias_table') or (leaf == 'bias' and '/upconv' in n)
        names = [n for n in spec if wants_parts(n)]
        P = self.PARTS
        self._parts = torch.zeros(P * sum(int(np.prod(spec[n][0])) for n in names), dtype=torch.float32, device=self.device)
        idx, o = [], 0
        for n in names:
            k = int(np.prod(spec[n][0]))
            self.params[n].part = (self._parts[o:o + k], P, k)
            idx.append(torch.arange(offs[n], offs[n] + k).repeat(P))
            o += P * k
        self._fold_index = torch.cat(idx).to(self.device)
        enc = ('patch_embed', 'flow_norm', 'all_patch_norm', 'flow_layers', 'layers')
        first_tail = next(n for n in spec if not n.startswith(enc))
        assert all(not n.startswith(enc) for n in list(spec)[list(spec).index(first_tail):])
        self.bucket_split = offs[first_tail]
        self._parts_split = P * sum(int(np.prod(spec[n][0])) for n in names if n.startswith(enc))
        self.cut_encoder = False
        self._cut_src = self._cut_leaf = None
        self._upconv_prep = {}
        self._xattn_pack_stale = True
        self._prep_event = None
        self.weights_version = 0
        self._sync_compute_weights()

    def _sync_compute_weights(self):
        if self.dtype != torch.float32:
            ops.call('stj_cast', ops._p(self._flat), 0, ops._p(self._cflat), ops.DTYPE_CODE[self.dtype], self._flat.numel(), ops._st())

    def state_dict(self):
        return OrderedDict((n, p.master.detach().cpu().numpy().copy()) for n, p in self.params.items())

    def save_weights(self, path):
        from . import checkpoint
        checkpoint.save_tf_checkpoint(path, self.state_dict(), self.cfg, self.fg_msa, self.fg)

    def load_weights(self, weights):
        if isinstance(weights, (str, os.PathLike)):
            from . import checkpoint
            weights = checkpoint.load_tf_checkpoint(os.fspath(weights), self.cfg, self.fg_msa, self.fg)
        missing = [n for n in self.params if n not in weights]
        extra = [n for n in weights if n not in self.params]
        if missing or extra:
            raise KeyError(f'load_weights: missing {missing[:5]} extra {extra[:5]}')
        with torch.no_grad():
            for n, p in self.params.items():
                w = torch.from_numpy(np.array(weights[n], dtype=np.float32))
                if tuple(w.shape) != p.shape:
                    raise ValueError(f'{n}: shape {tuple(w.shape)} != {p.shape}')
                p.master.copy_(w.to(self.device))
        self.weights_version += 1
        self._sync_compute_weights()

    def trainable_weights(self):
        return [p.master for p in self.params.values()]

    def parameters(self):
        return self.trainable_weights()

    def flat_grads(self):
        return self._gflat

    def flat_weights(self):
        return self._flat

    def zero_grad(self):
        self._gbuf[:self._goff8 + self._arena.off].zero_()
        self._arena.rearm()
        ops.use_arena(self._arena)

    def _fold_partials(self, which=None):
        k = self._parts_split
        lo, hi = {None: (0, self._parts.numel()), 'encoder': (0, k), 'tail': (k, self._parts.numel())}[which]
        if hi > lo:
            ops.call('stj_fold_parts', ops._p(self._gflat), ops._p(self._fold_index[lo:hi]), ops._p(self._parts[lo:hi]), hi - lo, ops._st())

    def backward_encoder(self):
        if self._cut_src is None:
            raise RuntimeError('backward_encoder(): no cut forward pending (set model.cut_encoder = True before the call)')
        src, leaf = self._cut_src, self._cut_leaf
        self._cut_src = self._cut_leaf = None
        pairs = [(s_, l.grad) for s_, l in zip(src, leaf) if l.grad is not None]
        sched = ops.wgrad_schedule(self.device)
        sched.begin()
        try:
            torch.autograd.backward([a for a, _ in pairs], [g for _, g in pairs])
        finally:
            sched.join(torch.cuda.current_stream(self.device), [st for st in self._streams if st is not None],
                       lambda: self._fold_partials('encoder'))

    def grads(self):
        return OrderedDict((n, p.grad) for n, p in self.params.items())

    def _p(self, name):
        return self.params[name]

    def _ln(self, x, name, eps, gather_res=0, res=None):
        return ops.layernorm(x, self._p(name + '/gamma'), self._p(name + '/beta'), eps, gather_res, res=res)

    def _ln_skip(self, x, name, eps):
        return ops.layernorm_skip(x, self._p(name + '/gamma'), self._p(name + '/beta'), eps)

    def _dense(self, x, name, act=ACT_NONE, res=None, bias=True):
        return ops.linear(x, self._p(name + '/kernel'), self._p(name + '/bias') if bias else None, act, res)

    def _swin_block(self, x, pre, B, res, heads, shift):
        if res <= 8:
            shift = 0
        dpr = self.drop_path_rate.get(pre, 0.0) if self._dctx is not None else 0.0
        fused_mlp = self.fused_mlp and x.shape[-1] in self.fused_mlp_dims
        if self.fused_attn and x.shape[-1] in self.fused_attn_dims:
            x = ops.swin_attn_half(x, self._p(pre + '/norm1/gamma'), self._p(pre + '/norm1/beta'), self._p(pre + '/attn/qkv/kernel'),
                                   self._p(pre + '/attn/qkv/bias'), self._p(pre + '/attn/relative_position_bias_table'),
                                   self._p(pre + '/attn/proj/kernel'), self._p(pre + '/attn/proj/bias'), B, res, shift, 1e-5,
                                   self._dctx, pre + '/drop_path_attn', dpr)
            if fused_mlp:
                return ops.swin_mlp(x, self._p(pre + '/norm2/gamma'), self._p(pre + '/norm2/beta'), self._p(pre + '/mlp/fc1/kernel'),
                                    self._p(pre + '/mlp/fc1/bias'), self._p(pre + '/mlp/fc2/kernel'), self._p(pre + '/mlp/fc2/bias'), 1e-5,
                                    self._dctx, pre + '/drop_path_mlp', dpr, rows_per_sample=res * res)
            h, x = self._ln_skip(x, pre + '/norm2', 1e-5)
            h = ops.gelu(self._dense(h, pre + '/mlp/fc1'))
            if dpr == 0.0:
                return self._dense(h, pre + '/mlp/fc2', res=x)
            h = self._dense(h, pre + '/mlp/fc2').view(B, -1)
            return ops.dropout(h, dpr, self._dctx, pre + '/drop_path_mlp', res=x.view(B, -1), per_sample=True).view(x.shape)
        h, x = self._ln_skip(x, pre + '/norm1', 1e-5)
        qkv = self._dense(h, pre + '/attn/qkv')
        a = ops.win_attn(qkv, self._p(pre + '/attn/relative_position_bias_table'), B, res, heads, shift)

        def mlp_fused(x):
            return ops.swin_mlp(x, self._p(pre + '/norm2/gamma'), self._p(pre + '/norm2/beta'), self._p(pre + '/mlp/fc1/kernel'),
                                self._p(pre + '/mlp/fc1/bias'), self._p(pre + '/mlp/fc2/kernel'), self._p(pre + '/mlp/fc2/bias'), 1e-5,
                                self._dctx, pre + '/drop_path_mlp', dpr, rows_per_sample=res * res)
        if dpr == 0.0:
            x = self._dense(a, pre + '/attn/proj', res=x)
            if fused_mlp:
                return mlp_fused(x)
            h, x = self._ln_skip(x, pre + '/norm2', 1e-5)
            h = ops.gelu(self._dense(h, pre + '/mlp/fc1'))
            return self._dense(h, pre + '/mlp/fc2', res=x)
        a = self._dense(a, pre + '/attn/proj').view(B, -1)
        x = ops.dropout(a, dpr, self._dctx, pre + '/drop_path_attn', res=x.view(B, -1), per_sample=True).view(x.shape)
        if fused_mlp:
            return mlp_fused(x)
        h, x = self._ln_skip(x, pre + '/norm2', 1e-5)
        h = ops.gelu(self._dense(h, pre + '/mlp/fc1'))
# ... 70 lines not shown
        for i in range(3):
            r, c = self.stage_res[i], self.stage_dim[i]
            x, res = self._basic_layer(x, f'layers{i}', B, r, depths[i], heads[i], i < 2, add=joined_flow_x if i == 0 else None)
            if i < 2:
                x = ops.wgrad_flush_point(x)
            if i == 0:
                res_list.append(crop(flow_res, r, c) if self.large_ogm else flow_res)
                if hook is not None:
                    hook()
            res_list.append(crop(res, r, c) if self.large_ogm else res)
        return res_list

    def _fgmsa(self, x):
        B, Hh, Ww, C = x.shape
        G = 8
        gc = C // G
        HW = Hh * Ww
        with ops.gemm_group():
            q = self._dense(x, 'fg_msa/proj_q')
            k = self._dense(x, 'fg_msa/proj_k')
            v = self._dense(x, 'fg_msa/proj_v')
        if self.fused_fgoff and ops.fgoff_ok(self.dtype, Hh, Ww, C, G):
            pw = self._p('fg_msa/conv_offset_0/kernel')
            if self._fgoff_pack_stale:
                self._fgoff_pack = ops.fgoff_pack(pw, self.dtype, out=self._fgoff_pack)
                self._fgoff_pack_stale = False
            elif self._fgoff_pack_event is not None:
                torch.cuda.current_stream(self.device).wait_event(self._fgoff_pack_event)
                self._fgoff_pack_event = None
            off = ops.fgoff_chain(q, pw, self._p('fg_msa/conv_offset_0/bias'), self._p('fg_msa/conv_norm/gamma'), self._p('fg_msa/conv_norm/beta'),
                                  self._p('fg_msa/conv_offset_proj/kernel'), self._fgoff_pack, Hh / 2.0, 1e-3)
        else:
            o = ops.grouped_conv3(q, self._p('fg_msa/conv_offset_0/kernel'), self._p('fg_msa/conv_offset_0/bias'), G)
            o = ops.gelu(self._ln(o, 'fg_msa/conv_norm', 1e-3))
            off = ops.fg_offset(o, self._p('fg_msa/conv_offset_proj/kernel'), Hh / 2.0, G)
        if self.fused_fgattn and ops.fg_attn_ok(self.dtype, Hh, Ww, gc):
            a = ops.fg_attn(q.view(B, HW, C), k.view(B, HW, C), v.view(B, HW, C), off, self._p('fg_msa/warp_attn_rel_table'), Hh, Ww, gc ** -0.5)
        else:
            a = ops.mha_core(q.view(B, HW, C), k.view(B, HW, C), v.view(B, HW, C), G, gc, gc ** -0.5,
                             fg_off=off, fg=(self._p('fg_msa/warp_attn_rel_table'), Hh, Ww))
        if self.taps is not None:
            y = self._dense(a.view(B, Hh, Ww, C), 'fg_msa/proj_out')
            self._tap('fg_msa_out', y)
            xy = x + y
        else:
            xy = self._dense(a.view(B, Hh, Ww, C), 'fg_msa/proj_out', res=x)
        if self.fg:
            query = ops.fg_query(off, self._p('fg_msa/conv_offset_proj2/kernel'), self._p('fg_msa/conv_offset_proj2/bias'),
                                 qres=xy.view(B, HW, C))
        else:
            query = xy.reshape(1, B, HW, C).expand(8, B, HW, C).contiguous()
        return xy, query

    def _tfa_mha(self, pre, query, key, H, qvalid, kvalid):
        pq, pk, pv = self._p(pre + '/query_kernel'), self._p(pre + '/key_kernel'), self._p(pre + '/value_kernel')
        hs = pq.shape[-1]
        with ops.gemm_group():
            q = ops.linear_heads_in(query, pq)
            k = ops.linear_heads_in(key, pk)
            v = ops.linear_heads_in(key, pv)
        o = ops.mha_core(q, k, v, H, hs, 1.0 / math.sqrt(hs), qvalid=qvalid, kvalid=kvalid,
                         drop=self._attn_drop(pre + '/dropout', (q.shape[0], H, q.shape[1], k.shape[1])))
        return ops.linear_heads_out(o, self._p(pre + '/projection_kernel'), self._p(pre + '/projection_bias'))

    def _attn_drop(self, name, shape, p=0.1):
        if self._dctx is None:
            return None
        return (p, self._dctx.snap, self._dctx.site(name, shape, p))

    def _drop(self, x, name, p=0.1):
        return x if self._dctx is None else ops.dropout(x, p, self._dctx, name)

    def _cross_attention(self, pre, query, key, H, qvalid, kvalid):
        v = self._tfa_mha(pre + '/mha', query, key, H, qvalid, kvalid)
        v = self._ln(v, pre + '/norm1', 1e-3)
        v = self._drop(self._dense(v, pre + '/FFN1', act=ACT_ELU), pre + '/dropout1')
        v = self._drop(self._dense(v, pre + '/FFN2'), pre + '/dropout2')
        return self._ln(v, pre + '/norm2', 1e-3)

    def agent_encode(self, obs, occ, cast=True):
        ops.set_serial(self.serial)
        ops.use_arena(self._arena)
        if cast:
            self._sync_compute_weights()
        self._agent_pack_stale = True
        self._dctx = None
        return tuple(self._traj_net(obs, occ))

    def _agent_ws(self):
        e, c = 'traj_net/traj_encoder', 'traj_net/cross_attention'
        p = self._p
        return {'wn': p(e + '/node_feature/kernel'), 'bn': p(e + '/node_feature/bias'), 'wv3': p(e + '/vector_feature/kernel'),
                'e_wq': p(e + '/node_attention/query_kernel'), 'e_wk': p(e + '/node_attention/key_kernel'),
                'e_wv': p(e + '/node_attention/value_kernel'), 'e_wo': p(e + '/node_attention/projection_kernel'),
                'e_bo': p(e + '/node_attention/projection_bias'), 'e_ws': p(e + '/sublayer/kernel'), 'e_bs': p(e + '/sublayer/bias'),
                'i_wq': p(c + '/mha/query_kernel'), 'i_wk': p(c + '/mha/key_kernel'), 'i_wv': p(c + '/mha/value_kernel'),
                'i_wo': p(c + '/mha/projection_kernel'), 'i_w1': p(c + '/FFN1/kernel'), 'i_w2': p(c + '/FFN2/kernel'),
                'i_bo': p(c + '/mha/projection_bias'), 'g1': p(c + '/norm1/gamma'), 'be1': p(c + '/norm1/beta'), 'b1': p(c + '/FFN1/bias'),
                'b2': p(c + '/FFN2/bias'), 'g2': p(c + '/norm2/gamma'), 'be2': p(c + '/norm2/beta'), 'seg': p('traj_net/seg_embed/kernel'),
                'g_obs': p('traj_net/obs_norm/gamma'), 'b_obs': p('traj_net/obs_norm/beta'), 'g_occ': p('traj_net/occ_norm/gamma'),
                'b_occ': p('traj_net/occ_norm/beta')}

    def _traj_net(self, obs, occ):
        pre = 'traj_net/traj_encoder'
        B, n_obs, T = obs.shape[0], obs.shape[1], obs.shape[2]
        A = n_obs + occ.shape[1]
        if self.fused_agent and ops.agent_enc_ok(n_obs, occ.shape[1], T, self.dtype):
            if self._agent_pack_stale:
                self._agent_pack = ops.agent_pack(self._agent_ws(), self.dtype, out=self._agent_pack)
                self._agent_pack_stale = False
            drop_e = self._attn_drop(pre + '/node_attention/dropout', (B * A, 4, T, T))
            if self.fused_agent_int and ops.agent_int_ok(n_obs, occ.shape[1], self.dtype):
                drop = None
                if self._dctx is not None:
                    c, d = 'traj_net/cross_attention', self._dctx
                    drop = (0.1, d.snap, (drop_e[2], d.site(c + '/mha/dropout', (B, 6, A, A), 0.1), d.site(c + '/dropout1', (B, A, 1536), 0.1),
                                          d.site(c + '/dropout2', (B, A, 384), 0.1)))
                return ops.agent_branch(obs, occ, self._agent_ws(), self._agent_pack, self.dtype, drop)
            enc, cmi = ops.agent_enc(obs, occ, self._agent_ws(), self._agent_pack, self.dtype, drop_e)
            cmf = cmi.to(self.dtype)
        else:
            x5, v3, vt, cmi, cmf = ops.agent_prep(obs, occ, self.dtype)
            nodes = ops.linear(x5, self._p(pre + '/node_feature/kernel'), self._p(pre + '/node_feature/bias'), act=ACT_ELU)
            nodes = nodes.view(B * A, T, 64)
            nodes = self._tfa_mha(pre + '/node_attention', nodes, nodes, 4, vt, vt)
            nodes = ops.maxpool_time(nodes).view(B, A, 320)
            vec = ops.linear(v3.view(B, A, 3), self._p(pre + '/vector_feature/kernel'))
            enc = ops.linear(torch.cat([nodes, vec], -1), self._p(pre + '/sublayer/kernel'), self._p(pre + '/sublayer/bias'), act=ACT_ELU)
        onehot = self._seg_onehot.get((A, n_obs))
        if onehot is None:
            onehot = torch.zeros((A, 2), dtype=self.dtype, device=self.device)
            onehot[:n_obs, 0] = 1
            onehot[n_obs:, 1] = 1
            self._seg_onehot[(A, n_obs)] = onehot
        embed = ops.linear(onehot, self._p('traj_net/seg_embed/kernel'))
        concat, q_in = ops.agent_mix(enc, embed, cmf)
        value = self._cross_attention('traj_net/cross_attention', q_in, concat, 6, cmi, cmi)
        if enc.shape[-1] == 384:
            key = ops.agent_out(enc, value, embed, self._p('traj_net/obs_norm/gamma'), self._p('traj_net/obs_norm/beta'),
                                self._p('traj_net/occ_norm/gamma'), self._p('traj_net/occ_norm/beta'), n_obs, 1e-3)
            return key, cmi
        out = ops.agent_sum(enc, value, embed)
        o1 = self._ln(out[:, :n_obs].contiguous(), 'traj_net/obs_norm', 1e-3)
        o2 = self._ln(out[:, n_obs:].contiguous(), 'traj_net/occ_norm', 1e-3)
        return torch.cat([o1, o2], 1), cmi

    def _resconv(self, skip, name, grad_is_pre):
        pw, pb = self._p(name + '/kernel'), self._p(name + '/bias')
        Ci, Co = pw.shape[3], pw.shape[4]
        wz = torch.empty((8, Ci, Co), dtype=self.dtype, device=self.device)
        ops.call('stj_time_collapse', ops._p(pw.master), ops._p(wz), Ci * Co, ops.DTYPE_CODE[self.dtype], ops._st())
        gwz = ops.zeros_f32((8, Ci, Co), self.device)

        def fold():
            ops.call('stj_time_fold', ops._p(gwz), ops._p(pw.grad), Ci * Co, ops._st())
        return ops.linear_z(skip, pw.master, wz[0], Ci * Co, pb.master.detach(), 0, gwz[0], Ci * Co, pb.grad, 8,
                            act=ACT_ELU, shared_x=True, fold=fold, grad_is_pre=grad_is_pre)

    def _zp(self, suffix):
        return self._p('cross_attn_obs0/' + suffix)

    def _xattn_params(self):
        z = self._zp
        return {'wq': z('mha/query_kernel'), 'wo': z('mha/projection_kernel'), 'bo': z('mha/projection_bias'), 'g1': z('norm1/gamma'),
                'be1': z('norm1/beta'), 'w1': z('FFN1/kernel'), 'b1': z('FFN1/bias'), 'w2': z('FFN2/kernel'), 'b2': z('FFN2/bias'),
                'g2': z('norm2/gamma'), 'be2': z('norm2/beta')}

    def _pack_xattn(self):
        self._xattn_pack = ops.xattn_pack(self._xattn_params(), self._zstride, 8, self.dtype, out=self._xattn_pack)
        self._xattn_pack_stale = False

    def _xattn_kv(self, key):
        zs = self._zstride
        with ops.gemm_group():
            pk, pv = self._zp('mha/key_kernel'), self._zp('mha/value_kernel')
            k = ops.linear_heads_in_z(key, pk.master, pk.c, pk.grad, zs, 8, True)
            v = ops.linear_heads_in_z(key, pv.master, pv.c, pv.grad, zs, 8, True)
        return k, v

    def _cross_attention_z(self, query, key, tmask):
        Z, B, HW, Cb = query.shape
        zs = self._zstride
        hs = 128 // 3
        A = key.shape[1]

        def proj_in(x, suffix, shared):
            p0 = self._zp(suffix)
            return ops.linear_heads_in_z(x, p0.master, p0.c, p0.grad, zs, 8, shared)
        if self.fused_xattn and A == 64 and HW % 64 == 0 and Cb == 384:
            k, v = self._xattn_kv(key)
            ps = self._xattn_params()
            if self._xattn_pack_stale:
                self._pack_xattn()
            return ops.xattn(query, k, v, tmask, self._xattn_pack, ps, zs, self._dctx,
                             ('cross_attn_obs/mha/dropout', 'cross_attn_obs/dropout1', 'cross_attn_obs/dropout2'))
        with ops.gemm_group():
            q = proj_in(query, 'mha/query_kernel', False)
            k = proj_in(key, 'mha/key_kernel', True)
            v = proj_in(key, 'mha/value_kernel', True)
        kvalid = tmask[None].expand(Z, B, A).reshape(Z * B, A).contiguous()
        o = ops.mha_core(q.view(Z * B, HW, 3 * hs), k.view(Z * B, A, 3 * hs), v.view(Z * B, A, 3 * hs), 3, hs,
                         1.0 / math.sqrt(hs), kvalid=kvalid, drop=self._attn_drop('cross_attn_obs/mha/dropout', (Z, B, 3, HW, A)))
        pw, pb = self._zp('mha/projection_kernel'), self._zp('mha/projection_bias')
        H_, hs_, O_ = pw.shape
        v1 = ops.linear_z(o.view(Z, B * HW, 3 * hs), pw.master, pw.c.view(H_ * hs_, O_), zs, pb.master.detach(), zs,
                          pw.grad.view(H_ * hs_, O_), zs, pb.grad, 8)
        v1 = ops.layernorm(v1, self._zp('norm1/gamma'), self._zp('norm1/beta'), 1e-3, group_rows=B * HW, ngroups=8, gstride=zs)
        pw, pb = self._zp('FFN1/kernel'), self._zp('FFN1/bias')
        v1 = self._drop(ops.linear_z(v1, pw.master, pw.c, zs, pb.master.detach(), zs, pw.grad, zs, pb.grad, 8, act=ACT_ELU),
                        'cross_attn_obs/dropout1')
        pw, pb = self._zp('FFN2/kernel'), self._zp('FFN2/bias')
        v1 = self._drop(ops.linear_z(v1, pw.master, pw.c, zs, pb.master.detach(), zs, pw.grad, zs, pb.grad, 8),
                        'cross_attn_obs/dropout2')
        v1 = ops.layernorm(v1, self._zp('norm2/gamma'), self._zp('norm2/beta'), 1e-3, group_rows=B * HW, ngroups=8, gstride=zs,
                           res=query.reshape(v1.shape))
        return v1.view(Z, B, HW, Cb)

    def _decoder(self, x, res_list, B, skips=None, skips_pre=False):
        hb = self.hb
        flow_res, r0, r1 = res_list[0], res_list[1], res_list[2]

        def up(t, name, grad_is_pre=False, x_is_elu_out=False):
            return ops.upconv(t, self._p(name + '/kernel'), self._p(name + '/bias'), grad_is_pre, x_is_elu_out,
                              prep=self._upconv_prep.get(name))
        x = x.view(8 * B, hb, hb, -1)
        if self._prep_event is not None:
            torch.cuda.current_stream(self.device).wait_event(self._prep_event)
        if skips is not None:
            main = torch.cuda.current_stream(self.device)
            main.wait_stream(self._side2)
            for t in skips:
                t.record_stream(main)
            s3, s2, sf = skips
        else:
            s3, s2, sf = (self._resconv(r1, 'decoder/resconv_3', skips_pre), self._resconv(r0, 'decoder/resconv_2', skips_pre),
                          self._resconv(flow_res, 'decoder/resconv_f', skips_pre))

        def up_add(t, name, ra, rb=None):
            return ops.upconv_add(t, self._p(name + '/kernel'), self._p(name + '/bias'), ra, rb, prep=self._upconv_prep.get(name),
                                  skips_pre=skips_pre)
        x = up_add(x, 'decoder/upconv_3_0', s3)
        self._tap('decoder/level3', x)
        x, fx = up_add(x, 'decoder/upconv_2_0', s2, sf)
        self._tap('decoder/level2', x)
        self._tap('decoder/level2_flow', fx)
        oc = ('decoder/outconv/kernel', 'decoder/outconv/bias', 'decoder/outconv_f/kernel', 'decoder/outconv_f/bias')
        if ops.upconv_head_ok(2 * x.shape[1], 2 * x.shape[2], self._p('decoder/upconv_0_0/kernel'), x.dtype, 8) and self.taps is None:
            def last(t, n1, n0, head):
                t = up(t, n1)
                return ops.upconv_head(t, self._p(n0 + '/kernel'), self._p(n0 + '/bias'), self._p(head), prep=self._upconv_prep.get(n0))
            zo = last(x, 'decoder/upconv_1_0', 'decoder/upconv_0_0', oc[0])
            zf = last(fx, 'decoder/upconvf_1_0', 'decoder/upconvf_0_0', oc[2])
            if self._quantize_heads and self.fused_quantize:
                return ops.heads_gather_q(zo, zf, self._p(oc[1]), self._p(oc[3]), B, 8, t_major=True)
            return ops.heads_gather(zo, zf, self._p(oc[1]), self._p(oc[3]), B, 8, t_major=True)
        if self._side2 is not None:
            main = torch.cuda.current_stream(self.device)
            self._side2.wait_stream(main)
            fx.record_stream(self._side2)
            with torch.cuda.stream(self._side2):
                fx = up(up(fx, 'decoder/upconvf_1_0', grad_is_pre=True), 'decoder/upconvf_0_0', grad_is_pre=True, x_is_elu_out=True)
            x = up(up(x, 'decoder/upconv_1_0', grad_is_pre=True), 'decoder/upconv_0_0', grad_is_pre=True, x_is_elu_out=True)
            main.wait_stream(self._side2)
            fx.record_stream(main)
        else:
            x = up(up(x, 'decoder/upconv_1_0', grad_is_pre=True), 'decoder/upconv_0_0', grad_is_pre=True, x_is_elu_out=True)
            fx = up(up(fx, 'decoder/upconvf_1_0', grad_is_pre=True), 'decoder/upconvf_0_0', grad_is_pre=True, x_is_elu_out=True)
        self._tap('decoder/level0', x)
        self._tap('decoder/level0_flow', fx)
        return ops.outconv_pair(x, fx, self._p('decoder/outconv/kernel'), self._p('decoder/outconv/bias'),
                                self._p('decoder/outconv_f/kernel'), self._p('decoder/outconv_f/bias'), B, 8, t_major=True, x_is_elu_out=True,
                                side=self._side2)

    def __call__(self, ogm, map_img, training=True, obs=None, occ=None, mapt=None, flow=None, dense_vec=None, dense_map=None):
        return self.call(ogm, map_img, training, obs, occ, mapt, flow, dense_vec, dense_map)

    def predict_quantized(self, ogm, map_img, obs=None, occ=None, mapt=None, flow=None):
        from .submission import QuantizedWaypoints, quantize_waypoints
        with torch.no_grad():
            self._quantize_heads = True
            try:
                out = self.call(ogm, map_img, False, obs, occ, mapt, flow)
            finally:
                self._quantize_heads = False
            if out.dtype == torch.uint8:
                H = self.cfg['input_size'][0]
                return QuantizedWaypoints(out, H, H)
            return quantize_waypoints(out)

    def predict_compressed(self, ogm, map_img, obs=None, occ=None, mapt=None, flow=None, out=None, level=1):
        from .submission import compress_waypoints
        if level not in (1, 2):
            raise ValueError(f'predict_compressed: level 1 or 2, got {level!r}')
        return compress_waypoints(self.predict_quantized(ogm, map_img, obs=obs, occ=occ, mapt=mapt, flow=flow), out=out, level=level)

    def call(self, ogm, map_img, training=True, obs=None, occ=None, mapt=None, flow=None, dense_vec=None, dense_map=None):
        if obs is None or occ is None or flow is None:
            raise ValueError('obs, occ and flow are required (reference modules.py:818,834)')
        H = self.cfg['input_size'][0]
        if ogm.dim() != 5 or tuple(ogm.shape[1:]) != (H, H, 11, 2):
            raise ValueError(f'ogm must be [B,{H},{H},11,2], got {tuple(ogm.shape)}')
        B = ogm.shape[0]
        if tuple(map_img.shape) != (B, self.map_size, self.map_size, 3):
            raise ValueError(f'map_img must be [B,{self.map_size},{self.map_size},3], got {tuple(map_img.shape)}')
        if tuple(flow.shape) != (B, H, H, 2):
            raise ValueError(f'flow must be [B,{H},{H},2], got {tuple(flow.shape)}')
        if tuple(obs.shape[2:]) != (11, 8) or tuple(occ.shape[2:]) != (11, 8):
            raise ValueError('obs/occ must be [B,n,11,8]')
        for t in (ogm, map_img, flow, obs, occ):
            if not t.is_cuda:
                raise RuntimeError('inputs must be CUDA (ROCm) tensors: the HIP path has no CPU fallback')
        self._side, self._side2 = (None, None) if self.serial else self._streams
        ops.set_serial(self.serial)
        ops.wgrad_schedule(self.device).reset()
        ops.use_arena(self._arena)
        self._sync_compute_weights()
        self._dctx = None
        if training:
            self.dropctx.begin()
            self._dctx = self.dropctx
        ogm, map_img, flow = ogm.float().contiguous(), map_img.float().contiguous(), flow.float().contiguous()
        hb, Cb = self.hb, self.stage_dim[2]
        names = ('decoder/upconv_3_0', 'decoder/upconv_2_0', 'decoder/upconv_1_0', 'decoder/upconv_0_0', 'decoder/upconvf_1_0',
                 'decoder/upconvf_0_0')
        self._prep_event = None
        self._xattn_pack_stale = True
        self._agent_pack_stale = True
        self._agent_pack_event = None
        self._fgoff_pack_stale = True
        self._fgoff_pack_event = None

        def issue_prep():
            if self._side2 is not None:
                self._side2.wait_stream(torch.cuda.current_stream(self.device))
                with torch.cuda.stream(self._side2):
                    if self.fused_fgoff and self.fg_msa and ops.fgoff_ok(self.dtype, hb, hb, Cb, 8):
                        self._fgoff_pack = ops.fgoff_pack(self._p('fg_msa/conv_offset_0/kernel'), self.dtype, out=self._fgoff_pack)
                        self._fgoff_pack_stale = False
                        self._fgoff_pack_event = torch.cuda.Event()
                        self._fgoff_pack_event.record(self._side2)
                    if self.fused_agent and self._agent_pack_stale:
                        self._agent_pack = ops.agent_pack(self._agent_ws(), self.dtype, out=self._agent_pack)
                        self._agent_pack_stale = False
                        self._agent_pack_event = torch.cuda.Event()
                        self._agent_pack_event.record(self._side2)
                    if self.fused_xattn:
                        self._pack_xattn()
                    self._upconv_prep = {n: ops.upconv_prep(self._p(n + '/kernel'), self.dtype) for n in names}
                    self._prep_event = torch.cuda.Event()
                    self._prep_event.record(self._side2)
            else:
                if self.fused_xattn:
                    self._pack_xattn()
                self._upconv_prep = {n: ops.upconv_prep(self._p(n + '/kernel'), self.dtype) for n in names}
        agent = []
        if self.agent_override is not None:
            agent.extend(self.agent_override)
        elif self._side is None:
            agent.extend(self._traj_net(obs, occ))
        branch = self._side is not None and self.agent_override is None
        if branch:
            main = torch.cuda.current_stream(self.device)
            fork = torch.cuda.Event()
            fork.record(main)

        def issue_agent():
            self._side.wait_event(fork)
            if self._agent_pack_event is not None:
                self._side.wait_event(self._agent_pack_event)
            with torch.cuda.stream(self._side):
                agent.extend(self._traj_net(obs, occ))
        late = branch and self._side2 is not None
        if not late:
            issue_prep()

        def hook():
            if late:
                issue_prep()
            if branch:
                issue_agent()
            if self.mid_forward_hook is not None:
                self.mid_forward_hook()
        res_list = self._encoder(ogm, map_img, flow, hook=hook)
        fold = self._fold_partials
        if self.cut_encoder and torch.is_grad_enabled():
            self._cut_src = res_list
            res_list = [t.detach().requires_grad_(True) for t in res_list]
            self._cut_leaf = res_list
            fold = lambda: self._fold_partials('tail')
        skips_pre = ops.skips_pre_ok(self.dtype)
        skips = None
        if self._side2 is not None:
            self._side2.wait_stream(torch.cuda.current_stream(self.device))
            for t in res_list[:3]:
                t.record_stream(self._side2)
            with torch.cuda.stream(self._side2):
                skips = (self._resconv(res_list[2], 'decoder/resconv_3', skips_pre), self._resconv(res_list[1], 'decoder/resconv_2', skips_pre),
                         self._resconv(res_list[0], 'decoder/resconv_f', skips_pre))
        q = ops.wgrad_flush_point(res_list[-1]).reshape(B, hb, hb, Cb)
# ... 20 lines not shown
```

strajnet_amd/ops.py:

```python
import contextlib
import ctypes

import os
import threading

import torch

from . import prof
from ._lib import call as _raw_call, ENUMS as _ENUMS


def call(name, *args):
    if prof.ACTIVE is None:
        return _raw_call(name, *args)
    prof.record(name, args, lambda: _raw_call(name, *args))


GROUP_GEMMS = os.environ.get('STJ_GEMM_GROUP', '1') != '0'
WS_KERNELS = os.environ.get('STJ_NO_WS') != '1'
class _GroupState(threading.local):
    def __init__(self):
        self.h = [None, None]
        self.depth = [0]

# ... 85 lines not shown
    ws = _WS.get(key)
    if ws is None:
        from ._lib import lib
        ws = _WS[key] = torch.zeros(int(getattr(lib(), size_fn)()), dtype=torch.uint8, device=device)
    return ws


class _ZeroArena:
    FLOATS = 8 << 20
    ALIGN = 64

    def __init__(self):
        self.buf, self.off, self.armed = None, 0, False
        self.split_ws = {}
        self.split_ws_stream = {}
        self.split_ws_captured = {}

    def _here(self, device):
        d = torch.device(device)
        return self.buf is not None and self.buf.device.type == d.type and (d.index is None or d.index == self.buf.device.index)

    def adopt(self, buf):
        self.buf, self.off, self.armed, self.external = buf, 0, False, True

    def rearm(self):
        self.off, self.armed = 0, True

    def arm(self, device):
        if not self._here(device):
            self.buf = torch.zeros(self.FLOATS, dtype=torch.float32, device=device)
        elif self.off:
            self.buf[:self.off].zero_()
        self.off, self.armed = 0, True

    def take(self, n, device):
        A = self.ALIGN
        n8 = (n + A - 1) // A * A
        if not self.armed or not self._here(device) or self.off + n8 > self.buf.numel():
            return None
        v = self.buf[self.off:self.off + n]
        self.off += n8
        return v


_ARENA = _ZeroArena()


def use_arena(arena):
    global _ARENA
    _ARENA = arena


def zeros_f32(shape, device):
    n = 1
    for d in (shape if isinstance(shape, (tuple, list)) else (shape,)):
        n *= int(d)
    v = _ARENA.take(n, device)
    if v is None:
        return torch.zeros(shape, dtype=torch.float32, device=device)
    return v.view(shape)


_ROLE_STREAMS = {}


def role_stream(device, role, priority=0):
    dev = torch.device(device)
    idx = dev.index if dev.index is not None else torch.cuda.current_device()
    st = _ROLE_STREAMS.get((idx, role))
    if st is None:
        st = _ROLE_STREAMS[(idx, role)] = torch.cuda.Stream(torch.device('cuda', idx), priority=priority)
    return st


_SERIAL = False


def set_serial(flag):
    global _SERIAL
    _SERIAL = bool(flag)


WGRAD_SK = os.environ.get('STJ_WGRAD_SK', '1') != '0'


class _WgradSchedule:
    def __init__(self, idx):
        self.idx = idx
        self.side = None
        self.keep, self.armed, self.main = [], False, None
        self.dense_on, self.jobs = False, []
        self.defer, self.upconvs = False, []

    def side_stream(self, *operands):
        if _SERIAL:
            return contextlib.nullcontext()
        if self.side is None:
            self.side = role_stream(self.idx, 'wgrad')
        main = torch.cuda.current_stream(self.idx)
        self.side.wait_stream(main)
        self.keep.extend(operands)
        if not self.armed:
            self.armed, self.main = True, main
            torch.autograd.Variable._execution_engine.queue_callback(self._join_side)
        return torch.cuda.stream(self.side)

    def _join_side(self):
        self.main.wait_stream(self.side)
        self.keep.clear()
        self.armed = False

    def begin(self):
        assert not self.jobs, 'wgrad schedule: jobs of another backward pass are still queued on this device'
        self.dense_on = WGRAD_SK

    def reset(self):
        self.dense_on, self.jobs = False, []

    def push(self, job, post):
        st = torch.cuda.current_stream(self.idx)
        ev = None
        if not _SERIAL:
            ev = torch.cuda.Event()
            ev.record(st)
        self.jobs.append((job, post, st, ev))

    def flush(self):
        self._flush_upconvs()
        self._flush_dense()

    def _flush_upconvs(self):
        items, self.upconvs = self.upconvs, []
        if not items:
            return
        items = sorted(items, key=lambda it: -it[1].shape[-1])
        with self.side_stream(*[t for it in items for t in it[1:]]):
            for wg, _, _ in items:
                wg()

    def _flush_dense(self):
        items, self.jobs = self.jobs, []
        if not items:
            return
        cur = torch.cuda.current_stream(self.idx)
        last = {}
        for job, post, st, ev in items:
            if ev is not None and st != cur:
                last[st] = ev
                for t in (job.x, job.dy):
                    if isinstance(t, torch.Tensor):
                        t.record_stream(cur)
        for ev in last.values():
            cur.wait_event(ev)
        wgrad_group([it[0] for it in items])
        for _, post, _, _ in items:
            if post is not None:
                post()

    def join(self, main, streams, post):
        for s in streams:
            main.wait_stream(s)
        with torch.cuda.stream(main), torch.no_grad():
            self._flush_dense()
            self.dense_on = False
            self._flush_upconvs()
            if self.armed:
                main.wait_stream(self.side)
            if post is not None:
                post()


_SCHEDULES = {}


def wgrad_schedule(dev=None):
    if dev is not None and getattr(dev, 'type', 'cuda') == 'cuda' and getattr(dev, 'index', None) is not None:
        idx = dev.index
    else:
        idx = torch.cuda.current_device() if torch.cuda.is_available() else -1
    s = _SCHEDULES.get(idx)
    if s is None:
        s = _SCHEDULES[idx] = _WgradSchedule(idx)
    return s


def wgrad_join_now(main):
    side = wgrad_schedule(main.device).side
    if side is not None:
        main.wait_stream(side)


class _FlushWgrads(torch.autograd.Function):
    @staticmethod
    def forward(ctx, x):
        return x.view_as(x)

    @staticmethod
    def backward(ctx, g):
        wgrad_schedule(g.device).flush()
        return g


def wgrad_flush_point(x):
    if WGRAD_SK and x.requires_grad and torch.is_grad_enabled():
        return _FlushWgrads.apply(x)
    return x


@contextlib.contextmanager
def deferred_upconv_wgrads(x):
    s = wgrad_schedule(x.device)
    s.defer, s.upconvs = x.requires_grad and torch.is_grad_enabled(), []
    try:
        yield _FlushWgrads.apply(x) if s.defer else x
    finally:
        s.defer = False


class _JoinAfterBackward(torch.autograd.Function):
    @staticmethod
    def forward(ctx, out, streams, post):
        ctx.streams, ctx.post = streams, post
        return out.view_as(out)

    @staticmethod
    def backward(ctx, g):
        streams, post = ctx.streams, ctx.post
        main = torch.cuda.current_stream(g.device)
        s = wgrad_schedule(g.device)
        s.begin()
        torch.autograd.Variable._execution_engine.queue_callback(lambda: s.join(main, streams, post))
        return g, None, None


def join_after_backward(out, streams, post=None):
    streams = [s for s in streams if s is not None]
    if (not streams and post is None) or not out.requires_grad:
        return out
    return _JoinAfterBackward.apply(out, streams, post)

# ... 1730 lines not shown
            call('stj_outconv_fwd', _p(xf), _p(p2w.master), _p(p2b.master), vp(out.data_ptr() + 8), F_, H, W, C, inner, ybs, yts, yps, dt, _st())
        ctx.ps = (p1w, p1b, p2w, p2b)
        ctx.geo = (F_, H, W, C, inner, ybs, yts, yps)
        ctx.elu_in = int(bool(x_is_elu_out))
        ctx.save_for_backward(xo, xf)
        return out

    @staticmethod
    def backward(ctx, dout):
        xo, xf = ctx.saved_tensors
        p1w, p1b, p2w, p2b = ctx.ps
        F_, H, W, C, Tn, ybs, yts, yps = ctx.geo
        dout = dout.contiguous().float()
        dt = _dt(xo)
        dxo, dxf = torch.empty_like(xo), torch.empty_like(xf)
        ws = _outconv_workspace(xo.device)
        call('stj_outconv_bwd', _p(xo), _p(p1w.master), vp(dout.data_ptr()), _p(dxo), _p(p1w.grad), _p(p1b.grad), F_, H, W, C, Tn,
             ybs, yts, yps, ctx.elu_in, _p(ws), ws.numel(), dt, _st())
        side = None if _SERIAL else ctx.side
        if side is not None:
            ws2 = _workspace(xo.device, 'stj_outconv_bwd_workspace_bytes', 1)
            main = torch.cuda.current_stream(xo.device)
            side.wait_stream(main)
            with torch.cuda.stream(side):
                call('stj_outconv_bwd', _p(xf), _p(p2w.master), vp(dout.data_ptr() + 8), _p(dxf), _p(p2w.grad), _p(p2b.grad), F_, H, W, C, Tn,
                     ybs, yts, yps, ctx.elu_in, _p(ws2), ws2.numel(), dt, _st())
            for t in (dxf, dout, xf):
                t.record_stream(side)
        else:
            call('stj_outconv_bwd', _p(xf), _p(p2w.master), vp(dout.data_ptr() + 8), _p(dxf), _p(p2w.grad), _p(p2b.grad), F_, H, W, C, Tn,
                 ybs, yts, yps, ctx.elu_in, _p(ws), ws.numel(), dt, _st())
        return (dxo, dxf) + (None,) * 13


def upconv_head_ok(Hi, Wi, pw, dtype, Tn):
    return (not torch.is_grad_enabled() and dtype != torch.float32 and tuple(pw.master.shape[2:]) == (96, 48) and Hi % 8 == 0 and Wi % 16 == 0
            and Tn == 8 and WS_KERNELS)


HEAD_CZ = 20


def upconv_head(x, pw, pb, phead, prep=None):
    _req_cuda(x)
    F_, Hi, Wi, Cin = x.shape
    wf, _ = prep if prep is not None else upconv_prep(pw, x.dtype)
    z = torch.empty((F_, 2 * Hi, 2 * Wi, HEAD_CZ), dtype=x.dtype, device=x.device)
    call('stj_upconv_fwd_head', _p(x.contiguous()), _p(wf), _p(pb.master), _p(phead.master), _p(z), F_, Hi, Wi, Cin, 48, _dt(x), _st())
    return z


def heads_gather(zo, zf, p1b, p2b, B, Tn, t_major=False):
    F_, H, W, _ = zo.shape
    out = torch.empty((B, H, W, 4 * Tn), dtype=torch.float32, device=zo.device)
    call('stj_outconv_pair_gather', _p(zo), _p(zf), _p(p1b.master), _p(p2b.master), _p(out), B, Tn, H, W, 1 if t_major else 0, _dt(zo), _st())
    return out


def heads_gather_q(zo, zf, p1b, p2b, B, Tn, t_major=False):
    F_, H, W, _ = zo.shape
    q = torch.empty((B, 4 * Tn * H * W), dtype=torch.uint8, device=zo.device)
    call('stj_outconv_pair_gather_q', _p(zo), _p(zf), _p(p1b.master), _p(p2b.master), _p(q), B, Tn, H, W, 1 if t_major else 0, _dt(zo), _st())
    return q


def outconv_pair(xo, xf, p1w, p1b, p2w, p2b, B, Tn, t_major=False, x_is_elu_out=False, side=None):
    return _OutConvPair.apply(xo, xf, p1w.master, p1b.master, p2w.master, p2b.master, p1w, p1b, p2w, p2b, B, Tn, t_major, x_is_elu_out, side)


class _OgmFlowLoss(torch.autograd.Function):
    @staticmethod
    def forward(ctx, logits, gt_obs, gt_occ, gt_flow, origin, gate, ogm_w, occ_w, fow, replica, flags, coef_pre=None, unit=None):
        _req_cuda(logits)
        logits = logits.contiguous().float()
        B, H, W, _ = logits.shape
        dev = logits.device
        loss = torch.empty(5, dtype=torch.float32, device=dev)
        coef = torch.empty(32, dtype=torch.float32, device=dev)
        ctx.unit_grad = None
        if coef_pre is not None and unit is not None and LOSS_FUSED_BWD:
            sums = zeros_f32(128 * 40, dev)
            dlogits = torch.empty_like(logits)
            w = (B, H, W, float(ogm_w), float(occ_w), float(fow), float(replica), int(flags))
            call('stj_loss_fwd_bwd', _p(logits), _p(gt_obs), _p(gt_occ), _p(gt_flow), _p(origin), _p(gate), _p(coef_pre), _p(sums), _p(loss),
                 _p(coef), _p(dlogits), *w, _st())
            ctx.unit_grad, ctx.dlogits = unit, dlogits
        else:
            sums = zeros_f32(32 * 40, dev)
            call('stj_loss_fwd', _p(logits), _p(gt_obs), _p(gt_occ), _p(gt_flow), _p(origin), _p(gate), _p(sums), _p(loss), _p(coef),
                 B, H, W, float(ogm_w), float(occ_w), float(fow), float(replica), int(flags), _st())
        ctx.geo = (B, H, W, int(flags))
        ctx.set_materialize_grads(False)
        ctx.save_for_backward(logits, gt_obs, gt_occ, gt_flow, origin, coef)
        terms = loss[:4]
        ctx.mark_non_differentiable(terms)
        return tuple(terms.unbind(0)) + (loss[4], terms)

    @staticmethod
    def backward(ctx, g0, g1, g2, g3, gt, _gvec):
        logits, gt_obs, gt_occ, gt_flow, origin, coef = ctx.saved_tensors
        B, H, W, flags = ctx.geo
        parts = (g0, g1, g2, g3)
        if all(g is None for g in parts) and gt is None:
            return (None,) * 13
        if ctx.unit_grad is not None and ctx.dlogits is not None and all(g is None for g in parts) and gt.data_ptr() == ctx.unit_grad.data_ptr():
            LOSS_FUSED_STATS['hits'] += 1
            dl, ctx.dlogits = ctx.dlogits, None
            return (dl,) + (None,) * 12
        if ctx.unit_grad is not None:
            LOSS_FUSED_STATS['misses'] += 1
            ctx.dlogits = None
        if all(g is None for g in parts):
            up = gt.float().contiguous()
            flags |= 8
        else:
            z = torch.zeros((), dtype=torch.float32, device=logits.device)
            up = torch.stack([(g.float() if g is not None else z) for g in parts])
            if gt is not None:
                up = up + gt.float()
        dlogits = torch.empty_like(logits)
        call('stj_loss_bwd', _p(logits), _p(gt_obs), _p(gt_occ), _p(gt_flow), _p(origin), _p(coef), _p(up), _p(dlogits), B, H, W,
             flags, _st())
        return (dlogits,) + (None,) * 12


LOSS_FUSED_BWD = True
LOSS_FUSED_STATS = {'hits': 0, 'misses': 0}


def loss_coef(gt_flow, gate, ogm_w, occ_w, fow, replica, flags):
    _req_cuda(gt_flow)
    B, _, H, W, _ = gt_flow.shape
    cnt = zeros_f32(8, gt_flow.device).view(torch.int32)
    coef = torch.empty(32, dtype=torch.float32, device=gt_flow.device)
    call('stj_loss_coef', _p(gt_flow), _p(gate), _p(cnt), _p(coef), B, H, W, float(ogm_w), float(occ_w), float(fow), float(replica),
         int(flags) & 7, _st())
    return coef


def auc_gate_coef(gt_obs, gt_occ, gt_flow, origin, ogm_w, occ_w, fow, replica, flags):
    _req_cuda(gt_obs)
    B, _, H, W, _ = gt_obs.shape
    dev = gt_obs.device
    hist = zeros_f32(8 * 202 + 8, dev).view(torch.int32)
    gate = torch.empty(8, dtype=torch.float32, device=dev)
    coef = torch.empty(32, dtype=torch.float32, device=dev)
    call('stj_loss_gate_coef', _p(gt_obs), _p(gt_occ), _p(gt_flow), _p(origin), _p(hist), _p(gate), None, _p(coef), B, H, W,
         float(ogm_w), float(occ_w), float(fow), float(replica), int(flags) & 7, _st())
    return gate, coef


def auc_gate(gt_obs, gt_occ, gt_flow, origin, return_auc=False):
    _req_cuda(gt_obs)
    B, _, H, W, _ = gt_obs.shape
    dev = gt_obs.device
    hist = zeros_f32(8 * 202, dev).view(torch.int32)
    gate = torch.empty(8, dtype=torch.float32, device=dev)
    auc = torch.empty(8, dtype=torch.float32, device=dev)
    call('stj_loss_auc_gate', _p(gt_obs), _p(gt_occ), _p(gt_flow), _p(origin), _p(hist), _p(gate), _p(auc), B, H, W, _st())
    return (gate, auc) if return_auc else gate


def ogm_flow_loss(logits, gt_obs, gt_occ, gt_flow, origin, gate, ogm_w, occ_w, fow, replica, use_warp, coef=None, unit=None):
    return _OgmFlowLoss.apply(logits, gt_obs, gt_occ, gt_flow, origin, gate, ogm_w, occ_w, fow, replica, use_warp, coef, unit)


EVAL_USE_GT, EVAL_NO_WARP = 8, 16


def eval_workspace_bytes(B, H, W):
    from ._lib import lib
    return int(lib().stj_eval_workspace_bytes(int(B), int(H), int(W)))


def eval_workspace(B, H, W, device):
    return torch.empty(eval_workspace_bytes(B, H, W), dtype=torch.uint8, device=device)


def eval_loss_metrics(logits, gt_obs, gt_occ, gt_flow, origin, ogm_w, occ_w, fow, replica, flags, running=None, loss_scale=1.0,
                      workspace=None, with_gate=False):
    _req_cuda(logits, gt_obs, gt_occ, gt_flow, origin, running, workspace)
    logits = logits.detach().contiguous().float()
    gt_obs, gt_occ, gt_flow, origin = (t.detach().contiguous().float() for t in (gt_obs, gt_occ, gt_flow, origin))
    B, H, W, C = logits.shape
    if C != 32 or tuple(gt_obs.shape) != (B, 8, H, W, 1) or tuple(gt_occ.shape) != (B, 8, H, W, 1) or \
            tuple(gt_flow.shape) != (B, 8, H, W, 2) or tuple(origin.shape) != (B, 8, H, W, 1):
        raise ValueError('eval_loss_metrics: logits must be [B,H,W,32] and the ground truth [B,8,H,W,{1,1,2,1}]')
    if running is not None and (running.dtype != torch.float64 or running.numel() != 12 or not running.is_contiguous()):
        raise ValueError('eval_loss_metrics: running must be a contiguous float64 tensor of 12 elements')
    dev = logits.device
    if workspace is None:
        workspace = eval_workspace(B, H, W, dev)
    elif workspace.numel() * workspace.element_size() < eval_workspace_bytes(B, H, W):
        raise ValueError('eval_loss_metrics: the workspace is smaller than stj_eval_workspace_bytes')
    loss = torch.empty(5, dtype=torch.float32, device=dev)
    met = torch.empty(7, dtype=torch.float32, device=dev)
    gate = torch.empty(8, dtype=torch.float32, device=dev) if with_gate else None
    auc = torch.empty(8, 4, dtype=torch.float32, device=dev) if with_gate else None
    if B * H * W == 0:
        loss.zero_(), met.zero_()
    call('stj_eval_fwd', _p(logits), _p(gt_obs), _p(gt_occ), _p(gt_flow), _p(origin), _p(workspace), _p(loss), _p(met), _p(gate), _p(auc),
         _p(running), B, H, W, float(ogm_w), float(occ_w), float(fow), float(replica), float(loss_scale), int(flags), _st())
    return (loss, met, gate, auc) if with_gate else (loss, met)
```

strajnet_amd/optim.py:

```python
import math
from collections import OrderedDict

import numpy as np
import torch

from ._lib import ENUMS
from .ops import _p, _st, call

_OPT = ENUMS['stj_optim']
LOSS_MEAN_KEYS = ('train_loss', 'train_loss_occ', 'train_loss_flow', 'train_loss_wp')


class Nadam:
    def __init__(self, flat_weights, flat_grads, lr=1e-4, beta_1=0.9, beta_2=0.999, epsilon=1e-7):
        if flat_weights.dtype != torch.float32 or flat_grads.dtype != torch.float32 or flat_weights.shape != flat_grads.shape:
            raise ValueError('Nadam needs matching flat float32 weight and gradient buffers')
        if not flat_weights.is_cuda:
            raise RuntimeError('Nadam: CUDA (ROCm) buffers only: the HIP path has no CPU fallback')
        self.w, self.g = flat_weights, flat_grads
        self.lr, self.b1, self.b2, self.eps = float(lr), float(beta_1), float(beta_2), float(epsilon)
        self.m = torch.zeros_like(flat_weights)
        self.v = torch.zeros_like(flat_weights)
        self.t = 0
        self.m_schedule = 1.0

    @classmethod
    def for_model(cls, model, **kw):
        return cls(model._flat, model._gflat, **kw)

    def _mu(self, t):
        return self.b1 * (1.0 - 0.5 * 0.96 ** (0.004 * t))

    def step(self, grad_scale=1.0):
        self.t += 1
        mu_t, mu_n = self._mu(self.t), self._mu(self.t + 1)
        sched_t = self.m_schedule * mu_t
        sched_n = sched_t * mu_n
        self.m_schedule = sched_t
        cg = (1.0 - mu_t) / (1.0 - sched_t)
        cm = mu_n / (1.0 - sched_n)
        vs = 1.0 / (1.0 - self.b2 ** self.t)
        call('stj_nadam_step', _p(self.w), _p(self.g), _p(self.m), _p(self.v), self.w.numel(), self.lr, self.b1, self.b2, self.eps,
             cg, cm, vs, float(grad_scale), _st())


class CosineDecayRestarts:

    def __init__(self, initial_learning_rate, first_decay_steps, t_mul=2.0, m_mul=1.0, alpha=0.0):
        self.initial_learning_rate, self.first_decay_steps = float(initial_learning_rate), float(first_decay_steps)
        self.t_mul, self.m_mul, self.alpha = float(t_mul), float(m_mul), float(alpha)
        if self.first_decay_steps <= 0 or self.t_mul <= 0:
            raise ValueError('CosineDecayRestarts: first_decay_steps and t_mul must be positive')

    def __call__(self, step):
        frac = float(step) / self.first_decay_steps
        if self.t_mul == 1.0:
            i_restart = math.floor(frac)
            frac -= i_restart
        else:
            i_restart = math.floor(math.log(1.0 - frac * (1.0 - self.t_mul)) / math.log(self.t_mul))
            length = self.t_mul ** i_restart
            frac = (frac - (1.0 - length) / (1.0 - self.t_mul)) / length
        cosine = 0.5 * self.m_mul ** i_restart * (1.0 + math.cos(math.pi * frac))
        return self.initial_learning_rate * ((1.0 - self.alpha) * cosine + self.alpha)

    def encode(self):
        return [_OPT['STJ_SCHED_COSINE_RESTARTS'], self.initial_learning_rate, self.first_decay_steps, self.t_mul, self.m_mul, self.alpha, 0.0, 0.0]


class CustomSchedule:

    def __init__(self, d_model, warmup_steps=4000):
        self.d_model, self.warmup_steps = float(d_model), float(warmup_steps)
        if self.d_model <= 0 or self.warmup_steps <= 0:
            raise ValueError('CustomSchedule: d_model and warmup_steps must be positive')

    def __call__(self, step):
        step = float(step)
        arg1 = math.inf if step == 0.0 else 1.0 / math.sqrt(step)
        return (1.0 / math.sqrt(self.d_model)) * min(arg1, step * self.warmup_steps ** -1.5)

    def encode(self):
        return [_OPT['STJ_SCHED_CUSTOM'], self.d_model, self.warmup_steps, 0.0, 0.0, 0.0, 0.0, 0.0]


def check_tensor_options(global_clipnorm, clipnorm, locate_nonfinite, segments):
    if clipnorm is not None and not float(clipnorm) > 0.0:
        raise ValueError('DeviceNadam: clipnorm must be positive (None: off)')
    if clipnorm is not None and global_clipnorm is not None:
        raise ValueError('DeviceNadam: global_clipnorm and clipnorm exclude each other')
    on = clipnorm is not None or bool(locate_nonfinite)
    if on and segments is None:
        raise ValueError('DeviceNadam: clipnorm and locate_nonfinite need segments= (DeviceNadam.for_model derives them from the model)')
    return on


def model_segments(model):
    return OrderedDict((n, (p.master.storage_offset() - model._flat.storage_offset(), p.master.numel())) for n, p in model.params.items())


def validate_segments(segments, n):
    if segments is None or not hasattr(segments, 'items') or len(segments) < 1:
        raise ValueError('DeviceNadam: segments must be a non-empty ordered mapping of name -> (start, len)')
    names, starts, lens = [], [], []
    end = 0
    for name, (start, length) in segments.items():
        start, length = int(start), int(length)
        if length < 1:
            raise ValueError(f'DeviceNadam: segment {name!r} has len {length} (must be at least 1)')
        if start % 4 != 0:
            raise ValueError(f'DeviceNadam: segment {name!r} starts at {start}, not a multiple of 4')
        if not names and start != 0:
            raise ValueError(f'DeviceNadam: the first segment ({name!r}) must start at 0, not {start}')
        if start < end:
            raise ValueError(f'DeviceNadam: segment {name!r} at {start} overlaps its predecessor, which ends at {end} (ascending, disjoint)')
        end = start + length
        names.append(name)
        starts.append(start)
        lens.append(length)
    if end > int(n):
        raise ValueError(f'DeviceNadam: the last segment ends at {end}, past the buffer\'s {int(n)} elements')
    if int(n) // 4 >= 2 ** 31:
        raise ValueError('DeviceNadam: the chunk table indexes 16-byte vectors with 32 bits: n must be below 2^33')
    return names, starts, lens


def chunk_table(starts, lens, n, chunk=_OPT['STJ_TENSOR_CHUNK']):
    starts, lens = np.asarray(starts, dtype=np.int64), np.asarray(lens, dtype=np.int64)
    ends = np.append(starts[1:], np.int64(n))
    per = (ends - starts + chunk - 1) // chunk
    chunk0 = np.zeros(len(starts) + 1, dtype=np.int64)
    np.cumsum(per, out=chunk0[1:])
    tensor = np.repeat(np.arange(len(starts), dtype=np.int64), per)
    first = starts[tensor] + (np.arange(chunk0[-1], dtype=np.int64) - chunk0[tensor]) * chunk
    n_apply = np.minimum(ends[tensor] - first, chunk)
    n_stat = np.clip(starts[tensor] + lens[tensor] - first, 0, n_apply)
    chunks = np.stack([first // 4, n_stat, n_apply, tensor], axis=1).astype(np.int32)
    return np.ascontiguousarray(chunks), chunk0.astype(np.int32)


class DeviceNadam:

    capturable = True

    def __init__(self, flat_weights, flat_grads, lr=1e-4, beta_1=0.9, beta_2=0.999, epsilon=1e-7, global_clipnorm=None, skip_nonfinite=False,
                 clipnorm=None, locate_nonfinite=False, segments=None):
        if flat_weights.dtype != torch.float32 or flat_grads.dtype != torch.float32 or flat_weights.shape != flat_grads.shape:
            raise ValueError('DeviceNadam needs matching flat float32 weight and gradient buffers')
        if not flat_weights.is_cuda or not flat_grads.is_cuda:
            raise RuntimeError('DeviceNadam: CUDA (ROCm) buffers only: the HIP path has no CPU fallback')
        if flat_weights.device != flat_grads.device or not flat_weights.is_contiguous() or not flat_grads.is_contiguous():
            raise ValueError('DeviceNadam needs contiguous weight and gradient buffers on one device')
        if global_clipnorm is not None and not float(global_clipnorm) > 0.0:
            raise ValueError('DeviceNadam: global_clipnorm must be positive (None: no clipping)')
        self.per_tensor = check_tensor_options(global_clipnorm, clipnorm, locate_nonfinite, segments)
        table = None
        if self.per_tensor:
            if flat_weights.dim() != 1:
                raise ValueError('DeviceNadam: the per-tensor options need one-dimensional flat buffers')
            names, starts, lens = validate_segments(segments, flat_weights.numel())
            table = chunk_table(starts, lens, flat_weights.numel())
            self.segments = OrderedDict((k, (a, b)) for k, a, b in zip(names, starts, lens))
        self.tensor_clipnorm = 0.0 if clipnorm is None else float(clipnorm)
        self.w, self.g = flat_weights, flat_grads
        self.schedule = lr if hasattr(lr, 'encode') else None
        self.b1, self.b2, self.eps = float(beta_1), float(beta_2), float(epsilon)
        self.clipnorm = 0.0 if global_clipnorm is None else float(global_clipnorm)
        self.skip_nonfinite = bool(skip_nonfinite)
        dev = flat_weights.device
        self.m = torch.zeros_like(flat_weights)
        self.v = torch.zeros_like(flat_weights)
        sched = self.schedule.encode() if self.schedule is not None else [_OPT['STJ_SCHED_CONSTANT'], float(lr)] + [0.0] * 6
        self.state = torch.tensor([0.0, 1.0] + [0.0] * 6, dtype=torch.float64).to(dev)
        self.sched = torch.tensor(sched, dtype=torch.float64).to(dev)
        self.coef = torch.zeros(8, dtype=torch.float32, device=dev)
        self.partials = torch.zeros(_OPT['STJ_GRADNORM_PARTS'], dtype=torch.float64, device=dev)
        self.running = torch.zeros(5, dtype=torch.float64, device=dev)
        self.loss_scale = None
        self._losses = None
        if self.per_tensor:
            chunks, chunk0 = table
            S, C = len(chunk0) - 1, len(chunks)
            self.n_tensors, self.n_chunks = S, C
            self.chunks, self.chunk0 = torch.from_numpy(chunks).to(dev), torch.from_numpy(chunk0).to(dev)
            self.gpart = torch.zeros(C, dtype=torch.float64, device=dev)
            self.mult = torch.zeros(S, dtype=torch.float32, device=dev)
            self.tsum = torch.zeros(S, dtype=torch.float64, device=dev)
            self.nfcount = torch.zeros(S, dtype=torch.int32, device=dev)

    @classmethod
    def for_model(cls, model, **kw):
        if 'segments' not in kw and any(kw.get(k) for k in ('clipnorm', 'locate_nonfinite')):
            kw['segments'] = model_segments(model)
        return cls(model._flat, model._gflat, **kw)

    iterations = property(lambda self: self.state[0], doc='updates applied (device scalar)')
    skipped = property(lambda self: self.state[2], doc='steps skipped for a non-finite gradient (device scalar)')
    grad_norm = property(lambda self: self.state[3], doc='global gradient norm of the last step, after grad_scale and before clipping; 0 '
                                                         'when neither global_clipnorm nor skip_nonfinite asks for it (device scalar)')
    lr = property(lambda self: self.state[4], doc='learning rate of the last applied step (device scalar)')

    first_nonfinite = property(lambda self: self.state[5], doc='with a per-tensor option: lowest index of a tensor whose gradient was '
                                                               'non-finite in the last step(), -1 for none; without one: always 0, '
                                                               'meaningless (device scalar)')
    nonfinite_tensors = property(lambda self: self.state[6], doc='with a per-tensor option: how many tensors were; without one: always 0, '
                                                                 'meaningless (device scalar)')
    calls = property(lambda self: self.state[7], doc='with a per-tensor option: step() calls, skipped ones included; without one: always 0 '
                                                     '(device scalar)')

    def _step_tensors(self, grad_scale):
        st, n, S, C = _st(), self.w.numel(), self.n_tensors, self.n_chunks
        means = self.loss_scale is not None
        if means and self._losses is None:
            raise RuntimeError('DeviceNadam: the loss means are on but no loss tensor is attached (attach_loss_means(losses, loss_scale))')
        flags = _OPT['STJ_NADAM_SKIP_NONFINITE'] if self.skip_nonfinite else 0
        call('stj_tensor_partials', _p(self.g), n, _p(self.chunks), C, S, _p(self.gpart), st)
        call('stj_nadam_prepare_tensors', _p(self.state), _p(self.sched), _p(self.gpart), _p(self.chunk0), C, S, _p(self.coef), _p(self.mult),
             _p(self.tsum), _p(self.nfcount), _p(self._losses if means else None), _p(self.running if means else None), self.b1, self.b2,
             float(grad_scale), self.clipnorm, self.tensor_clipnorm, self.loss_scale if means else 1.0, flags, st)
        call('stj_nadam_apply_tensors', _p(self.w), _p(self.g), _p(self.m), _p(self.v), n, _p(self.chunks), C, S, _p(self.coef), _p(self.mult),
             self.b1, self.b2, self.eps, st)

    grad_sumsq = property(lambda self: self.tsum if self.per_tensor else None,
                          doc='with a per-tensor option: each tensor\'s sum of g^2 of the last step(), float64[S] on the device')

    def nonfinite_counts(self):
        if not self.per_tensor:
            raise RuntimeError('DeviceNadam.nonfinite_counts(): built without a per-tensor option')
        return OrderedDict(zip(self.segments, self.nfcount.tolist()))

    def step(self, grad_scale=1.0):
        if self.per_tensor:
            return self._step_tensors(grad_scale)
        st, n = _st(), self.w.numel()
        partials = None
        if self.clipnorm > 0.0 or self.skip_nonfinite:
            partials = self.partials
            call('stj_gradnorm_partials', _p(self.g), n, _p(partials), st)
        means = self.loss_scale is not None
        if means and self._losses is None:
            raise RuntimeError('DeviceNadam: the loss means are on but no loss tensor is attached (attach_loss_means(losses, loss_scale))')
        call('stj_nadam_prepare', _p(self.state), _p(self.sched), _p(partials), _p(self.coef), _p(self._losses if means else None),
             _p(self.running if means else None), self.b1, self.b2, float(grad_scale), self.clipnorm, self.loss_scale if means else 1.0,
             _OPT['STJ_NADAM_SKIP_NONFINITE'] if self.skip_nonfinite else 0, st)
        call('stj_nadam_apply', _p(self.w), _p(self.g), _p(self.m), _p(self.v), n, _p(self.coef), self.b1, self.b2, self.eps, st)

    def attach_loss_means(self, losses, loss_scale=1.0):
        if losses is not None:
            if losses.dtype != torch.float32 or losses.numel() != 4 or not losses.is_contiguous() or losses.device != self.w.device:
                raise ValueError('DeviceNadam.attach_loss_means: losses must be a contiguous float32[4] on the optimizer\'s device')
        self._losses, self.loss_scale = losses, float(loss_scale)

    def loss_result(self):
        r = self.running.tolist()
        return {k: (v / r[0] if r[0] else 0.0) for k, v in zip(LOSS_MEAN_KEYS, r[1:])}

    def reset_loss_means(self):
        self.running.zero_()

    def tensors(self):
        out = [self.w, self.m, self.v, self.state, self.running]
        if self.per_tensor:
            out += [self.nfcount, self.tsum, self.mult]
        return out

    def state_dict(self):
        src = {'m': self.m, 'v': self.v, 'state': self.state}
        if self.per_tensor:
            src['nonfinite_counts'] = self.nfcount
        out = {k: torch.empty(t.shape, dtype=t.dtype, pin_memory=True) for k, t in src.items()}
        for k, t in src.items():
            out[k].copy_(t, non_blocking=True)
        torch.cuda.current_stream(self.w.device).synchronize()
        return out

    def load_state_dict(self, sd):
        dst = {'m': self.m, 'v': self.v, 'state': self.state}
        for k, t in dst.items():
            if k not in sd or tuple(sd[k].shape) != tuple(t.shape) or sd[k].dtype != t.dtype:
                raise ValueError(f'DeviceNadam.load_state_dict: {k} missing or of another shape / dtype')
        counts = sd.get('nonfinite_counts') if self.per_tensor else None
        if counts is not None:
            if tuple(counts.shape) != tuple(self.nfcount.shape) or counts.dtype != self.nfcount.dtype:
                raise ValueError('DeviceNadam.load_state_dict: nonfinite_counts of another shape / dtype')
            dst['nonfinite_counts'] = self.nfcount
        for k, t in dst.items():
            t.copy_(sd[k], non_blocking=True)
        torch.cuda.current_stream(self.w.device).synchronize()
```

strajnet_amd/prof.py:

```python
import torch

ACTIVE = None
COST = {}


def enable():
    global ACTIVE
    ACTIVE = {}


def disable():
    global ACTIVE
    p, ACTIVE = ACTIVE, None
    return p


def _es(dt):
    return 4 if dt == 0 else 2


def _gemm(a):
    (M, N, K, nb1, nb2) = a[6:11]
    sAb1, sAb2, sAm, sAk, sBb1, sBb2, sBk, sBn = a[11:19]
    act, alpha, dt, c_f32, acc, splitk, nkb = a[27], a[28], a[29], a[30], a[31], a[32], a[33]
# ... 94 lines not shown
    return f'outconv_pair_fwd[{H}x{W},{C}->2,F{F}x2]', 'outconv_fwd', fl, fl, by


def _ln(kind):
    def f(a):
        if kind == 'fwd':
            rows, C, dt = a[6], a[7], a[14]
            by = 2 * _es(dt) * rows * C
        elif kind == 'res_fwd':
            rows, C, dt = a[7], a[8], a[13]
            by = 3 * _es(dt) * rows * C
            return f'layernorm_res_fwd[{rows}x{C}]', 'layernorm_fwd', 9.0 * rows * C, 9.0 * rows * C, by
        else:
            rows, C, dt = a[8], a[9], a[18]
            by = (4 if getattr(a[15], 'value', None) else 3) * _es(dt) * rows * C
        return f'layernorm_{kind}[{rows}x{C}]', 'layernorm_' + kind, 8.0 * rows * C, 8.0 * rows * C, by
    return f


def _win(kind):
    def f(a):
        if kind == 'fwd':
            B, res, heads, dt = a[3], a[4], a[5], a[7]
            nmm, tens = 2, 4
        else:
            B, res, heads, dt = a[6], a[7], a[8], a[10]
            nmm, tens = 5, 8
        items = B * (res // 8) ** 2 * heads
        fl = items * nmm * 2.0 * 64 * 64 * 32
        by = _es(dt) * B * res * res * heads * 32 * tens
        return f'win_attn_{kind}[B{B} {res}x{res} h{heads}]', 'win_attn_' + kind, fl, fl, by
    return f


def _elem(fam, n_idx, dt_idx, tensors, f32=False):
    def f(a):
        n = a[n_idx]
        es = 4 if f32 else _es(a[dt_idx])
        return f'{fam}[{n}]', fam, 0.0, 0.0, tensors * es * n
    return f


def _loss(fam, tens):
    def f(a):
        B, H, W = (a[9], a[10], a[11]) if fam == 'loss_fwd' else ((a[11], a[12], a[13]) if fam == 'loss_fwd_bwd' else (a[8], a[9], a[10]))
        by = 4.0 * B * H * W * (32 * tens + 8 * 5)
        return f'{fam}[B{B} {H}x{W}]', fam, 0.0, 0.0, by
    return f


def _eval(a):
    B, H, W = a[11], a[12], a[13]
    return f'eval_fwd[B{B} {H}x{W}]', 'eval_fwd', 0.0, 0.0, 4.0 * B * H * W * (32 + 8 * 5)


def _patch_embed(a):
    B, H, W, Cin, pix, Cout, dt = a[16], a[17], a[18], a[19], a[20], a[22], a[24]
    es = _es(dt)
    M = B * (H // 4) * (W // 4)
    nz = lambda i: bool(getattr(a[i], 'value', None))
    by = 4.0 * B * H * W * pix + es * M * Cout * (1 + nz(5) + nz(9) + nz(10)) + es * M * 16 * Cin * nz(8)
    fl = 2.0 * M * 16 * Cin * Cout
    return f'patch_embed[{H}x{W},{Cin}->{Cout},B{B}]', 'patch_embed_fwd', fl, fl, by


def _ln_chain(a):
    rows, C, dt = a[15], a[16], a[21]
    return f'ln_bwd_chain[{rows}x{C}]', 'layernorm_bwd', 0.0, 0.0, _es(dt) * rows * C * (4 + bool(getattr(a[9], 'value', None)))


MODELS = {
    'stj_gemm': _gemm,
    'stj_patch_embed_fwd': _patch_embed, 'stj_layernorm_bwd_chain': _ln_chain,
    'stj_upconv_fwd': _upconv('fwd'), 'stj_upconv_fwd_head': _upconv_head, 'stj_outconv_pair_gather': _pair_gather, 'stj_outconv_pair_gather_q': _pair_gather_q, 'stj_quantize_waypoints': _quantize, 'stj_compress_waypoints': _compress, 'stj_upconv_fwd_res': _upconv_res, 'stj_elu_res_bwd': _elu_res, 'stj_upconv_dgrad': _upconv('dgrad'), 'stj_upconv_wgrad': _upconv('wgrad'),
    'stj_outconv_fwd': _outconv('fwd'), 'stj_outconv_pair_fwd': _outconv_pair, 'stj_outconv_bwd': _outconv('bwd'),
    'stj_layernorm_fwd': _ln('fwd'), 'stj_layernorm_bwd': _ln('bwd'), 'stj_layernorm_res_fwd': _ln('res_fwd'),
    'stj_win_attn_fwd': _win('fwd'), 'stj_win_attn_bwd': _win('bwd'),
    'stj_unary_fwd': _elem('unary_fwd', 2, 5, 2), 'stj_unary_bwd': _elem('unary_bwd', 3, 6, 3),
    'stj_dropout': _elem('dropout', 3, 8, 2),
    'stj_loss_fwd': _loss('loss_fwd', 1), 'stj_loss_bwd': _loss('loss_bwd', 2), 'stj_loss_fwd_bwd': _loss('loss_fwd_bwd', 2),
    'stj_eval_fwd': _eval,
    'stj_nadam_step': _elem('nadam', 4, 0, 7, f32=True),
    'stj_gradnorm_partials': _elem('gradnorm', 1, 0, 1, f32=True), 'stj_nadam_apply': _elem('nadam_apply', 4, 0, 7, f32=True),
}
EXTRA_MODELS = {}


def record(name, args, launch):
    m = MODELS.get(name) or EXTRA_MODELS.get(name)
    if m is not None:
        try:
            key, fam, fa, fe, by = m(args)
        except Exception:
            key, fam, fa, fe, by = name, name.replace('stj_', ''), 0.0, 0.0, 0.0
    else:
        key, fam, fa, fe, by = name, name.replace('stj_', ''), 0.0, 0.0, 0.0
    st = torch.cuda.current_stream()
    e0, e1 = torch.cuda.Event(enable_timing=True), torch.cuda.Event(enable_timing=True)
    e0.record(st)
    launch()
    e1.record(st)
    COST[key] = (fam, fa, fe, by)
    ACTIVE.setdefault(key, []).append((e0, e1))


def summarize(events, steps):
    keys = {}
    for k, evs in events.items():
        ms = [a.elapsed_time(b) for a, b in evs]
        fam, fa, fe, by = COST[k]
        keys[k] = dict(family=fam, launches=len(ms) / steps, avg_ms=sum(ms) / len(ms), ms_per_step=sum(ms) / steps,
                       flops_alg=fa, flops_exec=fe, bytes_alg=by)
    fams = {}
    for k, v in keys.items():
        f = fams.setdefault(v['family'], dict(ms_per_step=0.0, launches=0.0, flop_alg=0.0, flop_exec=0.0, bytes=0.0))
        f['ms_per_step'] += v['ms_per_step']
        f['launches'] += v['launches']
        f['flop_alg'] += v['flops_alg'] * v['launches']
        f['flop_exec'] += v['flops_exec'] * v['launches']
        f['bytes'] += v['bytes_alg'] * v['launches']
    return keys, fams
```

Baseline: 1409 scenes/s.

## Fuse optimizer bf16 weight shadow, batch time-fold posts, add in-launch loss finalize

The Nadam apply kernels can now also write a bf16/f16 shadow copy of the updated weights, so a separate cast of the fp32 master weights to the compute dtype is not needed after each step. Consecutive time-fold wgrad post-ops are batched into a single multi-segment launch. An optional loss finalize runs inside the last workgroup of the fused loss kernel, tracked with arrival counters, but it is off by default. The shadow write adds store traffic to the optimizer, and the in-launch finalize depends on cross-workgroup atomic ordering.

```diff
diff --git a/include/strajnet_hip.h b/include/strajnet_hip.h
--- a/include/strajnet_hip.h
+++ b/include/strajnet_hip.h
@@ -252,6 +252,11 @@
 int stj_loss_fwd_bwd(const float* logits, const float* gt_obs, const float* gt_occ, const float* gt_flow, const float* origin,
                      const float* gate, const float* coef_in, float* sums, float* loss, float* coef_out, float* dlogits,
                      int B, int H, int W, float ogm_w, float occ_w, float flow_origin_w, float replica, int flags, hipStream_t stream);
+enum stj_loss { STJ_LOSS_ARRIVE_INTS = 160 };
+int stj_loss_fwd_bwd_fin(const float* logits, const float* gt_obs, const float* gt_occ, const float* gt_flow, const float* origin,
+                         const float* gate, const float* coef_in, float* sums, float* loss, float* coef_out, float* dlogits,
+                         int B, int H, int W, float ogm_w, float occ_w, float flow_origin_w, float replica, int flags, int* arrive,
+                         hipStream_t stream);
 
 int stj_decode_raw(const void* src, int kind, float* dst, long long n_outer, int H, int W, int C, int y0, int x0, int Ho,
                    int Wo, float scale, hipStream_t stream);
@@ -296,6 +301,7 @@
                       void* dembed, float* dg0, float* db0, float* dg1, float* db1, int B, int A, int n0, int C, int dtype, hipStream_t stream);
 int stj_time_collapse(const float* W, void* Wz, long long n, int dtype, hipStream_t stream);
 int stj_time_fold(const float* dWz, float* dW, long long n, hipStream_t stream);
+int stj_time_fold_multi(const float* const* src, float* const* dst, const long long* n, int nseg, hipStream_t stream);
 int stj_fold_parts(float* g, const long long* idx, float* parts, long long n, hipStream_t stream);
 
 int stj_crc32c(const void* data, long long n, unsigned int* crc);
@@ -316,6 +322,8 @@
 int stj_dropout_mask(unsigned char* mask, long long ndraw, float p, const long long* state, int site, hipStream_t stream);
 int stj_nadam_step(float* w, const float* g, float* m, float* v, long long n, float lr, float b1, float b2, float eps,
                    float cg, float cm, float vhat_scale, float gscale, hipStream_t stream);
+int stj_nadam_step_shadow(float* w, const float* g, float* m, float* v, long long n, float lr, float b1, float b2, float eps,
+                          float cg, float cm, float vhat_scale, float gscale, void* shadow, int shadow_dtype, hipStream_t stream);
 
 enum stj_optim { STJ_GRADNORM_PARTS = 256, STJ_SCHED_CONSTANT = 0, STJ_SCHED_COSINE_RESTARTS = 1, STJ_SCHED_CUSTOM = 2,
                  STJ_NADAM_SKIP_NONFINITE = 1, STJ_TENSOR_CHUNK = 4096, STJ_TENSOR_GRID = 1024 };
@@ -324,6 +332,8 @@
                       float b1, float b2, float gscale, float clipnorm, float loss_scale, int flags, hipStream_t stream);
 int stj_nadam_apply(float* w, const float* g, float* m, float* v, long long n, const float* coef, float b1, float b2, float eps,
                     hipStream_t stream);
+int stj_nadam_apply_shadow(float* w, const float* g, float* m, float* v, long long n, const float* coef, float b1, float b2, float eps,
+                           void* shadow, int shadow_dtype, hipStream_t stream);
 
 int stj_tensor_partials(const float* g, long long n, const int* chunks, int n_chunks, int S, double* gpart, hipStream_t stream);
 int stj_nadam_prepare_tensors(double* state, const double* sched, const double* gpart, const int* chunk0, int n_chunks, int S, float* coef,
diff --git a/strajnet_amd/csrc/loss.hip b/strajnet_amd/csrc/loss.hip
--- a/strajnet_amd/csrc/loss.hip
+++ b/strajnet_amd/csrc/loss.hip
@@ -92,22 +92,7 @@
 
 struct LossCfg { float ogm_w, occ_w, fow, replica; int use_warp; };
 
-__global__ void loss_finalize_kernel(const float* sums_parts, int nparts, const float* gate, float* loss, float* coef, float npix, LossCfg c) {
-  __shared__ float sums[NWP * S_N], part[6][NWP * S_N];
-  if (threadIdx.x < 6 * NWP * S_N) {
-    const int slot = threadIdx.x % (NWP * S_N), j = threadIdx.x / (NWP * S_N);
-    float a = 0.f;
-#pragma unroll 8
-    for (int q = j; q < nparts; q += 6) a += sums_parts[q * (NWP * S_N) + slot];
-    part[j][slot] = a;
-  }
-  __syncthreads();
-  if (threadIdx.x < NWP * S_N) {
-    const int t = threadIdx.x;
-    sums[t] = ((((part[0][t] + part[1][t]) + part[2][t]) + part[3][t]) + part[4][t]) + part[5][t];
-  }
-  __syncthreads();
-  if (threadIdx.x != 0) return;
+__device__ __attribute__((noinline)) void loss_write(const float* sums, const float* gate, float* loss, float* coef, float npix, LossCfg c) {
   float so = 0.f, sc = 0.f, sf = 0.f, sw = 0.f, fc = 0.f;
   for (int k = 0; k < NWP; ++k) fc += gate[k];
   for (int k = 0; k < NWP; ++k) {
@@ -128,6 +113,31 @@
   loss[2] = sf / fc;
   loss[3] = c.use_warp ? sw / fc : 0.f;
   loss[4] = loss[0] + loss[1] + loss[2] + loss[3];
+}
+template <bool AGENT>
+__device__ __forceinline__ float loss_fold_share(const float* sums_parts, int nparts, int slot, int j) {
+  float a = 0.f;
+#pragma unroll 8
+  for (int q = j; q < nparts; q += 6) {
+    const float* p = sums_parts + q * (NWP * S_N) + slot;
+    a += AGENT ? __hip_atomic_load(p, __ATOMIC_RELAXED, __HIP_MEMORY_SCOPE_AGENT) : *p;
+  }
+  return a;
+}
+__device__ __forceinline__ float loss_fold_six(const float (*part)[NWP * S_N], int t) {
+  return ((((part[0][t] + part[1][t]) + part[2][t]) + part[3][t]) + part[4][t]) + part[5][t];
+}
+__global__ void loss_finalize_kernel(const float* sums_parts, int nparts, const float* gate, float* loss, float* coef, float npix, LossCfg c) {
+  __shared__ float sums[NWP * S_N], part[6][NWP * S_N];
+  if (threadIdx.x < 6 * NWP * S_N) {
+    const int slot = threadIdx.x % (NWP * S_N), j = threadIdx.x / (NWP * S_N);
+    part[j][slot] = loss_fold_share<false>(sums_parts, nparts, slot, j);
+  }
+  __syncthreads();
+  if (threadIdx.x < NWP * S_N) sums[threadIdx.x] = loss_fold_six(part, threadIdx.x);
+  __syncthreads();
+  if (threadIdx.x != 0) return;
+  loss_write(sums, gate, loss, coef, npix, c);
 }
 
 template <bool FOCAL, bool PRED>
@@ -181,10 +191,12 @@
 #ifndef LOSS_FB_MAXG
 #define LOSS_FB_MAXG 16384
 #endif
-template <bool FOCAL, bool PRED>
+struct LossFin { const float* gate; float* loss; float* coef_out; int* arrive; float npix; LossCfg c; };
+static_assert(NWP * S_N <= 64, "loss_fwd_bwd_kernel<FIN>: one wave issues the workgroup's adds and folds 6 shares of NWP * S_N slots");
+template <bool FOCAL, bool PRED, bool FIN>
 __global__ __launch_bounds__(256) void loss_fwd_bwd_kernel(const float* logits, const float* gt_obs, const float* gt_occ,
                                                            const float* gt_flow, const float* origin, const float* coef,
-                                                           float* sums, float* dlogits, int B, int H, int W, int use_warp) {
+                                                           float* sums, float* dlogits, int B, int H, int W, int use_warp, LossFin fin) {
   __shared__ float red[4][NWP * S_N];
   const float inv_hw = 1.f / ((float)H * (float)W);
   float acc[S_N];
@@ -247,6 +259,29 @@
   __syncthreads();
   if (threadIdx.x < NWP * S_N)
     atomicAdd(sums + (blockIdx.x % LOSS_PARTS_FUSED) * (NWP * S_N) + threadIdx.x, red[0][threadIdx.x] + red[1][threadIdx.x] + red[2][threadIdx.x] + red[3][threadIdx.x]);
+  if constexpr (FIN) {
+    if (threadIdx.x >= 64) return;
+    asm volatile("s_waitcnt vmcnt(0)" ::: "memory");
+    const int copy = blockIdx.x % LOSS_PARTS_FUSED;
+    const int ncopies = min((int)gridDim.x, LOSS_PARTS_FUSED);
+    const int mine = ((int)gridDim.x - copy + LOSS_PARTS_FUSED - 1) / LOSS_PARTS_FUSED;
+    int last = 0;
+    if (threadIdx.x == 0 && __hip_atomic_fetch_add(fin.arrive + copy, 1, __ATOMIC_RELAXED, __HIP_MEMORY_SCOPE_AGENT) == mine - 1) {
+      __hip_atomic_store(fin.arrive + copy, 0, __ATOMIC_RELAXED, __HIP_MEMORY_SCOPE_AGENT);
+      if (__hip_atomic_fetch_add(fin.arrive + LOSS_PARTS_FUSED, 1, __ATOMIC_RELAXED, __HIP_MEMORY_SCOPE_AGENT) == ncopies - 1) {
+        __hip_atomic_store(fin.arrive + LOSS_PARTS_FUSED, 0, __ATOMIC_RELAXED, __HIP_MEMORY_SCOPE_AGENT);
+        last = 1;
+      }
+    }
+    if (!__shfl(last, 0, 64)) return;
+    __shared__ float part[6][NWP * S_N], tot[NWP * S_N];
+    for (int p = threadIdx.x; p < 6 * NWP * S_N; p += 64)
+      part[p / (NWP * S_N)][p % (NWP * S_N)] = loss_fold_share<true>(sums, LOSS_PARTS_FUSED, p % (NWP * S_N), p / (NWP * S_N));
+    __builtin_amdgcn_fence(__ATOMIC_ACQ_REL, "workgroup"); __builtin_amdgcn_wave_barrier();
+    if (threadIdx.x < NWP * S_N) tot[threadIdx.x] = loss_fold_six(part, threadIdx.x);
+    __builtin_amdgcn_fence(__ATOMIC_ACQ_REL, "workgroup"); __builtin_amdgcn_wave_barrier();
+    if (threadIdx.x == 0) loss_write(tot, fin.gate, fin.loss, fin.coef_out, fin.npix, fin.c);
+  }
 }
 
 template <bool VEC4>
@@ -354,25 +389,39 @@
   hipLaunchKernelGGL(loss_coef_kernel, dim3(1), dim3(64), 0, stream, cnt, gate, coef, (float)npix, c);
   return stj_check_launch("stj_loss_gate_coef");
 }
+extern "C" int stj_loss_fwd_bwd_fin(const float* logits, const float* gt_obs, const float* gt_occ, const float* gt_flow, const float* origin,
+                                    const float* gate, const float* coef_in, float* sums, float* loss, float* coef_out, float* dlogits,
+                                    int B, int H, int W, float ogm_w, float occ_w, float flow_origin_w, float replica, int flags,
+                                    int* arrive, hipStream_t stream) {
+  static_assert(STJ_LOSS_ARRIVE_INTS >= LOSS_PARTS_FUSED + 1, "one counter per copy and the final one");
+  if ((((uintptr_t)logits) | ((uintptr_t)dlogits)) & 15) { stj_set_error("loss: logits / dlogits must be 16-byte aligned"); return STJ_EINVAL; }
+  if (((uintptr_t)gt_flow) & 7) { stj_set_error("loss: gt_flow must be 8-byte aligned"); return STJ_EINVAL; }
+  if (flags & ~7) { stj_set_error("loss: unknown flag bits %d", flags); return STJ_EINVAL; }
+  if (((uintptr_t)arrive) & 3) { stj_set_error("loss: arrive must be 4-byte aligned"); return STJ_EINVAL; }
+  if (arrive && (!loss || !coef_out || !gate)) { stj_set_error("loss: arrive needs gate, loss and coef_out"); return STJ_EINVAL; }
+  const long long npix = (long long)B * H * W;
+  const int gx = (int)min((long long)LOSS_FB_MAXG, (npix * NWP + 255) / 256);
+  const int use_warp = flags & 1, focal = (flags >> 1) & 1, pred = (flags >> 2) & 1;
+  LossCfg c; c.ogm_w = ogm_w; c.occ_w = occ_w; c.fow = flow_origin_w; c.replica = replica; c.use_warp = use_warp;
+  LossFin fin; fin.gate = gate; fin.loss = loss; fin.coef_out = coef_out; fin.arrive = arrive; fin.npix = (float)npix; fin.c = c;
+  const bool in_launch = arrive != nullptr && gx > 0;
+  if (gx > 0) {
+#define LOSS_FB(FO, PR, FI) hipLaunchKernelGGL((loss_fwd_bwd_kernel<FO, PR, FI>), dim3(gx), dim3(256), 0, stream, logits, gt_obs, gt_occ, gt_flow, origin, coef_in, sums, dlogits, B, H, W, use_warp, fin)
+#define LOSS_FB2(FO, PR) do { if (in_launch) LOSS_FB(FO, PR, true); else LOSS_FB(FO, PR, false); } while (0)
+    if (focal && pred) LOSS_FB2(true, true); else if (focal) LOSS_FB2(true, false); else if (pred) LOSS_FB2(false, true); else LOSS_FB2(false, false);
+#undef LOSS_FB2
+#undef LOSS_FB
+  }
+  if (loss == nullptr || in_launch) return stj_check_launch("stj_loss_fwd_bwd");
+  hipLaunchKernelGGL(loss_finalize_kernel, dim3(1), dim3(256), 0, stream, sums, LOSS_PARTS_FUSED, gate, loss, coef_out, (float)npix, c);
+  return stj_check_launch("stj_loss_fwd_bwd");
+}
 extern "C" int stj_loss_fwd_bwd(const float* logits, const float* gt_obs, const float* gt_occ, const float* gt_flow, const float* origin,
                                 const float* gate, const float* coef_in, float* sums, float* loss, float* coef_out, float* dlogits,
                                 int B, int H, int W, float ogm_w, float occ_w, float flow_origin_w, float replica, int flags,
                                 hipStream_t stream) {
-  if ((((uintptr_t)logits) | ((uintptr_t)dlogits)) & 15) { stj_set_error("loss: logits / dlogits must be 16-byte aligned"); return STJ_EINVAL; }
-  if (((uintptr_t)gt_flow) & 7) { stj_set_error("loss: gt_flow must be 8-byte aligned"); return STJ_EINVAL; }
-  if (flags & ~7) { stj_set_error("loss: unknown flag bits %d", flags); return STJ_EINVAL; }
-  const long long npix = (long long)B * H * W;
-  const int gx = (int)min((long long)LOSS_FB_MAXG, (npix * NWP + 255) / 256);
-  const int use_warp = flags & 1, focal = (flags >> 1) & 1, pred = (flags >> 2) & 1;
-  if (gx > 0) {
-#define LOSS_FB(FO, PR) hipLaunchKernelGGL((loss_fwd_bwd_kernel<FO, PR>), dim3(gx), dim3(256), 0, stream, logits, gt_obs, gt_occ, gt_flow, origin, coef_in, sums, dlogits, B, H, W, use_warp)
-    if (focal && pred) LOSS_FB(true, true); else if (focal) LOSS_FB(true, false); else if (pred) LOSS_FB(false, true); else LOSS_FB(false, false);
-#undef LOSS_FB
-  }
-  if (loss == nullptr) return stj_check_launch("stj_loss_fwd_bwd");
-  LossCfg c; c.ogm_w = ogm_w; c.occ_w = occ_w; c.fow = flow_origin_w; c.replica = replica; c.use_warp = use_warp;
-  hipLaunchKernelGGL(loss_finalize_kernel, dim3(1), dim3(256), 0, stream, sums, LOSS_PARTS_FUSED, gate, loss, coef_out, (float)npix, c);
-  return stj_check_launch("stj_loss_fwd_bwd");
+  return stj_loss_fwd_bwd_fin(logits, gt_obs, gt_occ, gt_flow, origin, gate, coef_in, sums, loss, coef_out, dlogits, B, H, W, ogm_w, occ_w,
+                              flow_origin_w, replica, flags, nullptr, stream);
 }
 extern "C" int stj_loss_finalize(const float* sums, const float* gate, float* loss, float* coef_out, int B, int H, int W, float ogm_w,
                                  float occ_w, float flow_origin_w, float replica, int flags, hipStream_t stream) {
diff --git a/strajnet_amd/csrc/nadam.h b/strajnet_amd/csrc/nadam.h
--- a/strajnet_amd/csrc/nadam.h
+++ b/strajnet_amd/csrc/nadam.h
@@ -7,3 +7,14 @@
   v = b2 * v + (1.f - b2) * gg * gg;
   w -= lr * (cg * gg + cm * m) / (sqrtf(v * vhat_scale) + eps);
 }
+
+__device__ __forceinline__ void nadam_shadow4(void* shadow, int dtype, long long i, const float4& W) {
+  uint2 p;
+  if (dtype == STJ_BF16) { p.x = pack2<bf16>(W.x, W.y); p.y = pack2<bf16>(W.z, W.w); }
+  else { p.x = pack2<f16>(W.x, W.y); p.y = pack2<f16>(W.z, W.w); }
+  reinterpret_cast<uint2*>(shadow)[i] = p;
+}
+__device__ __forceinline__ void nadam_shadow1(void* shadow, int dtype, long long i, float w) {
+  if (dtype == STJ_BF16) stf(reinterpret_cast<bf16*>(shadow) + i, w);
+  else stf(reinterpret_cast<f16*>(shadow) + i, w);
+}
diff --git a/strajnet_amd/csrc/optim.hip b/strajnet_amd/csrc/optim.hip
--- a/strajnet_amd/csrc/optim.hip
+++ b/strajnet_amd/csrc/optim.hip
@@ -35,7 +35,7 @@
 
 __global__ __launch_bounds__(256) void nadam_apply_kernel(float* __restrict__ w, const float* __restrict__ g, float* __restrict__ m,
                                                           float* __restrict__ v, long long n, const float* __restrict__ coef, float b1,
-                                                          float b2, float eps) {
+                                                          float b2, float eps, void* __restrict__ shadow, int shadow_dtype) {
   if (coef[5] == 0.f) return;
   const float lr = coef[0], cg = coef[1], cm = coef[2], vhat_scale = coef[3], gscale = coef[4];
   const long long nv = n / 4;
@@ -46,10 +46,12 @@
 #pragma unroll
     for (int e = 0; e < 4; ++e) nadam_update(wp[e], gp[e], mp[e], vp[e], lr, b1, b2, eps, cg, cm, vhat_scale, gscale);
     reinterpret_cast<float4*>(w)[i] = W; reinterpret_cast<float4*>(m)[i] = M; reinterpret_cast<float4*>(v)[i] = V;
+    if (shadow) nadam_shadow4(shadow, shadow_dtype, i, W);
   }
   if (blockIdx.x == 0 && threadIdx.x < (n & 3)) {
     const long long i = nv * 4 + threadIdx.x;
     nadam_update(w[i], g[i], m[i], v[i], lr, b1, b2, eps, cg, cm, vhat_scale, gscale);
+    if (shadow) nadam_shadow1(shadow, shadow_dtype, i, w[i]);
   }
 }
 
@@ -78,16 +80,21 @@
   return stj_check_launch("stj_nadam_prepare");
 }
 
-extern "C" int stj_nadam_apply(float* w, const float* g, float* m, float* v, long long n, const float* coef, float b1, float b2, float eps,
-                               hipStream_t stream) {
+extern "C" int stj_nadam_apply_shadow(float* w, const float* g, float* m, float* v, long long n, const float* coef, float b1, float b2,
+                                      float eps, void* shadow, int shadow_dtype, hipStream_t stream) {
   if (n < 0) { stj_set_error("stj_nadam_apply: n must not be negative (got %lld)", n); return STJ_EINVAL; }
   if (n == 0) return STJ_OK;
   if (!w || !g || !m || !v || !coef) { stj_set_error("stj_nadam_apply: null pointer"); return STJ_EINVAL; }
-  if ((((uintptr_t)w) | ((uintptr_t)g) | ((uintptr_t)m) | ((uintptr_t)v) | ((uintptr_t)coef)) & 15) {
+  if ((((uintptr_t)w) | ((uintptr_t)g) | ((uintptr_t)m) | ((uintptr_t)v) | ((uintptr_t)coef) | ((uintptr_t)shadow)) & 15) {
     stj_set_error("stj_nadam_apply: buffers must be 16-byte aligned"); return STJ_EINVAL;
   }
   long long b = (n / 4 + 255) / 256;
   const int grid = (int)(b < 1 ? 1 : (b > 4096 ? 4096 : b));
-  hipLaunchKernelGGL(nadam_apply_kernel, dim3(grid), dim3(256), 0, stream, w, g, m, v, n, coef, b1, b2, eps);
+  if (shadow && !stj_is16(shadow_dtype)) { stj_set_error("stj_nadam_apply_shadow: the shadow's dtype must be STJ_BF16 or STJ_F16 (got %d)", shadow_dtype); return STJ_EINVAL; }
+  hipLaunchKernelGGL(nadam_apply_kernel, dim3(grid), dim3(256), 0, stream, w, g, m, v, n, coef, b1, b2, eps, shadow, shadow_dtype);
   return stj_check_launch("stj_nadam_apply");
 }
+extern "C" int stj_nadam_apply(float* w, const float* g, float* m, float* v, long long n, const float* coef, float b1, float b2, float eps,
+                               hipStream_t stream) {
+  return stj_nadam_apply_shadow(w, g, m, v, n, coef, b1, b2, eps, nullptr, 0, stream);
+}
diff --git a/strajnet_amd/csrc/rng.hip b/strajnet_amd/csrc/rng.hip
--- a/strajnet_amd/csrc/rng.hip
+++ b/strajnet_amd/csrc/rng.hip
@@ -122,7 +122,7 @@
 
 __global__ __launch_bounds__(256) void nadam_kernel(float* __restrict__ w, const float* __restrict__ g, float* __restrict__ m,
                                                     float* __restrict__ v, long long n, float lr, float b1, float b2, float eps,
-                                                    float cg, float cm, float vhat_scale, float gscale) {
+                                                    float cg, float cm, float vhat_scale, float gscale, void* __restrict__ shadow, int shadow_dtype) {
   const long long nv = n / 4;
   for (long long i = blockIdx.x * 256ll + threadIdx.x; i < nv; i += gridDim.x * 256ll) {
     float4 W = reinterpret_cast<float4*>(w)[i], G = reinterpret_cast<const float4*>(g)[i];
@@ -131,18 +131,25 @@
 #pragma unroll
     for (int e = 0; e < 4; ++e) nadam_update(wp[e], gp[e], mp[e], vp[e], lr, b1, b2, eps, cg, cm, vhat_scale, gscale);
     reinterpret_cast<float4*>(w)[i] = W; reinterpret_cast<float4*>(m)[i] = M; reinterpret_cast<float4*>(v)[i] = V;
+    if (shadow) nadam_shadow4(shadow, shadow_dtype, i, W);
   }
   if (blockIdx.x == 0 && threadIdx.x < (n & 3)) {
     const long long i = nv * 4 + threadIdx.x;
     nadam_update(w[i], g[i], m[i], v[i], lr, b1, b2, eps, cg, cm, vhat_scale, gscale);
+    if (shadow) nadam_shadow1(shadow, shadow_dtype, i, w[i]);
   }
+}
+extern "C" int stj_nadam_step_shadow(float* w, const float* g, float* m, float* v, long long n, float lr, float b1, float b2, float eps,
+                                     float cg, float cm, float vhat_scale, float gscale, void* shadow, int shadow_dtype, hipStream_t stream) {
+  if (n <= 0) return STJ_OK;
+  if ((((uintptr_t)w) | ((uintptr_t)g) | ((uintptr_t)m) | ((uintptr_t)v) | ((uintptr_t)shadow)) & 15) { stj_set_error("stj_nadam_step: buffers must be 16-byte aligned"); return STJ_EINVAL; }
+  long long b = (n / 4 + 255) / 256;
+  const int grid = (int)(b < 1 ? 1 : (b > 4096 ? 4096 : b));
+  if (shadow && !stj_is16(shadow_dtype)) { stj_set_error("stj_nadam_step_shadow: the shadow's dtype must be STJ_BF16 or STJ_F16 (got %d)", shadow_dtype); return STJ_EINVAL; }
+  hipLaunchKernelGGL(nadam_kernel, dim3(grid), dim3(256), 0, stream, w, g, m, v, n, lr, b1, b2, eps, cg, cm, vhat_scale, gscale, shadow, shadow_dtype);
+  return stj_check_launch("stj_nadam_step");
 }
 extern "C" int stj_nadam_step(float* w, const float* g, float* m, float* v, long long n, float lr, float b1, float b2, float eps,
                               float cg, float cm, float vhat_scale, float gscale, hipStream_t stream) {
-  if (n <= 0) return STJ_OK;
-  if ((((uintptr_t)w) | ((uintptr_t)g) | ((uintptr_t)m) | ((uintptr_t)v)) & 15) { stj_set_error("stj_nadam_step: buffers must be 16-byte aligned"); return STJ_EINVAL; }
-  long long b = (n / 4 + 255) / 256;
-  const int grid = (int)(b < 1 ? 1 : (b > 4096 ? 4096 : b));
-  hipLaunchKernelGGL(nadam_kernel, dim3(grid), dim3(256), 0, stream, w, g, m, v, n, lr, b1, b2, eps, cg, cm, vhat_scale, gscale);
-  return stj_check_launch("stj_nadam_step");
+  return stj_nadam_step_shadow(w, g, m, v, n, lr, b1, b2, eps, cg, cm, vhat_scale, gscale, nullptr, 0, stream);
 }
diff --git a/strajnet_amd/csrc/util.hip b/strajnet_amd/csrc/util.hip
--- a/strajnet_amd/csrc/util.hip
+++ b/strajnet_amd/csrc/util.hip
@@ -280,6 +280,25 @@
   }
 }
 __global__ __launch_bounds__(256) void time_fold_kernel(const float* __restrict__ dWz, float* __restrict__ dW, long long n) {
+  for (long long i = blockIdx.x * 256ll + threadIdx.x; i < n; i += gridDim.x * 256ll) {
+    float g[8];
+#pragma unroll
+    for (int t = 0; t < 8; ++t) g[t] = dWz[t * n + i];
+#pragma unroll
+    for (int j = 0; j < 8; ++j) {
+      float a = 0.f;
+#pragma unroll
+      for (int t = 0; t < 8; ++t)
+        if (j >= 3 - t && j <= 10 - t) a += g[t];
+      dW[j * n + i] += a;
+    }
+  }
+}
+struct TimeFoldSegs { const float* src[4]; float* dst[4]; long long n[4]; };
+__global__ __launch_bounds__(256) void time_fold_multi_kernel(TimeFoldSegs s) {
+  const float* __restrict__ dWz = s.src[blockIdx.y];
+  float* __restrict__ dW = s.dst[blockIdx.y];
+  const long long n = s.n[blockIdx.y];
   for (long long i = blockIdx.x * 256ll + threadIdx.x; i < n; i += gridDim.x * 256ll) {
     float g[8];
 #pragma unroll
@@ -547,6 +566,21 @@
   hipLaunchKernelGGL(time_fold_kernel, dim3(ew_grid(n)), dim3(256), 0, stream, dWz, dW, n);
   return stj_check_launch("stj_time_fold");
 }
+extern "C" int stj_time_fold_multi(const float* const* src, float* const* dst, const long long* n, int nseg, hipStream_t stream) {
+  if (nseg < 1 || nseg > 4 || !src || !dst || !n) { stj_set_error("stj_time_fold_multi: 1 to 4 segments (got %d), non-null tables", nseg); return STJ_EINVAL; }
+  TimeFoldSegs s = {};
+  int k = 0, gx = 1;
+  for (int i = 0; i < nseg; ++i) {
+    if (n[i] <= 0) continue;
+    if (!src[i] || !dst[i]) { stj_set_error("stj_time_fold_multi: segment %d: null pointer", i); return STJ_EINVAL; }
+    s.src[k] = src[i]; s.dst[k] = dst[i]; s.n[k] = n[i];
+    gx = max(gx, ew_grid(n[i]));
+    ++k;
+  }
+  if (k == 0) return STJ_OK;
+  hipLaunchKernelGGL(time_fold_multi_kernel, dim3(gx, k), dim3(256), 0, stream, s);
+  return stj_check_launch("stj_time_fold_multi");
+}
 
 __global__ __launch_bounds__(256) void fold_parts_kernel(float* __restrict__ g, const long long* __restrict__ idx, float* __restrict__ parts, long long n) {
   for (long long i = blockIdx.x * 256ll + threadIdx.x; i < n; i += gridDim.x * 256ll) {
diff --git a/strajnet_amd/graph.py b/strajnet_amd/graph.py
--- a/strajnet_amd/graph.py
+++ b/strajnet_amd/graph.py
@@ -2,6 +2,10 @@
 
 from . import ops
 from .loss import get_pred_waypoint_logits, warpped_gt
+
+
+def _cast_will_be_captured(model):
+    return not model._shadow_kept or model._shadow_stale
 
 
 class GraphedTrainStep:
@@ -39,6 +43,7 @@
         torch.cuda.current_stream().wait_stream(side)
         torch.cuda.synchronize()
         g = torch.cuda.CUDAGraph(keep_graph=True) if keep_graph else torch.cuda.CUDAGraph()
+        self._cast_inside = _cast_will_be_captured(model)
         with torch.cuda.graph(g, capture_error_mode='thread_local'):
             self.losses = self._eager()
         self.graph = g
@@ -86,6 +91,7 @@
     def __call__(self, batch=None, between=None):
         if batch is not None:
             self.load(batch)
+        self.model._refresh_compute_weights(cast_follows=self._cast_inside)
         self.graph.replay()
         if self.graph_b is not None:
             if between is not None:
@@ -125,6 +131,7 @@
             self.agent_cur = tuple(t.clone() for t in self.agent_next)
             torch.cuda.synchronize()
             model.agent_override = self.agent_cur
+        self._cast_inside = _cast_will_be_captured(model)
         try:
             self.graph = torch.cuda.CUDAGraph()
             with torch.no_grad(), torch.cuda.graph(self.graph, capture_error_mode='thread_local'):
@@ -192,6 +199,7 @@
                         self.static[k].copy_(next_batch[k], non_blocking=True)
                 self._staged = torch.cuda.Event()
                 self._staged.record(main)
+        self.model._refresh_compute_weights(cast_follows=self._cast_inside)
         self.graph.replay()
         if self.pipeline_agents and next_batch is not None:
             self.prefetch_agents()
@@ -220,6 +228,7 @@
         torch.cuda.synchronize()
         self.running.zero_()
         torch.cuda.synchronize()
+        self._cast_inside = _cast_will_be_captured(model)
         self.graph = torch.cuda.CUDAGraph()
         with torch.no_grad(), torch.cuda.graph(self.graph, capture_error_mode='thread_local'):
             self.logits, self.losses, self.metrics = self._eager()
@@ -239,6 +248,7 @@
     def __call__(self, batch=None):
         if batch is not None:
             self.load(batch)
+        self.model._refresh_compute_weights(cast_follows=self._cast_inside)
         self.graph.replay()
         return self.losses, self.metrics
 
diff --git a/strajnet_amd/modules.py b/strajnet_amd/modules.py
--- a/strajnet_amd/modules.py
+++ b/strajnet_amd/modules.py
@@ -259,11 +259,31 @@
         self._xattn_pack_stale = True
         self._prep_event = None
         self.weights_version = 0
+        self._shadow_kept = False
+        self._shadow_stale = False
+        self.keep_shadow = True
         self._sync_compute_weights()
 
     def _sync_compute_weights(self):
         if self.dtype != torch.float32:
             ops.call('stj_cast', ops._p(self._flat), 0, ops._p(self._cflat), ops.DTYPE_CODE[self.dtype], self._flat.numel(), ops._st())
+        self._shadow_stale = False
+
+    def shadow_for_optimizer(self, keep=True):
+        if not keep or self.dtype == torch.float32 or not self.keep_shadow:
+            self._shadow_kept = False
+            return None
+        self._shadow_kept, self._shadow_stale = True, True
+        return self._cflat
+
+    def mark_weights_written(self):
+        self._shadow_stale = True
+
+    def _refresh_compute_weights(self, cast_follows=False):
+        if cast_follows:
+            self._shadow_stale = False
+        elif self._shadow_stale or not self._shadow_kept:
+            self._sync_compute_weights()
 
     def state_dict(self):
         return OrderedDict((n, p.master.detach().cpu().numpy().copy()) for n, p in self.params.items())
@@ -290,6 +310,7 @@
         self._sync_compute_weights()
 
     def trainable_weights(self):
+        self.mark_weights_written()
         return [p.master for p in self.params.values()]
 
     def parameters(self):
@@ -299,6 +320,7 @@
         return self._gflat
 
     def flat_weights(self):
+        self.mark_weights_written()
         return self._flat
 
     def zero_grad(self):
@@ -535,7 +557,7 @@
         ops.set_serial(self.serial)
         ops.use_arena(self._arena)
         if cast:
-            self._sync_compute_weights()
+            self._refresh_compute_weights()
         self._agent_pack_stale = True
         self._dctx = None
         return tuple(self._traj_net(obs, occ))
@@ -604,9 +626,7 @@
         wz = torch.empty((8, Ci, Co), dtype=self.dtype, device=self.device)
         ops.call('stj_time_collapse', ops._p(pw.master), ops._p(wz), Ci * Co, ops.DTYPE_CODE[self.dtype], ops._st())
         gwz = ops.zeros_f32((8, Ci, Co), self.device)
-
-        def fold():
-            ops.call('stj_time_fold', ops._p(gwz), ops._p(pw.grad), Ci * Co, ops._st())
+        fold = ops.TimeFold(gwz, pw.grad, Ci * Co)
         return ops.linear_z(skip, pw.master, wz[0], Ci * Co, pb.master.detach(), 0, gwz[0], Ci * Co, pb.grad, 8,
                             act=ACT_ELU, shared_x=True, fold=fold, grad_is_pre=grad_is_pre)
 
@@ -767,7 +787,7 @@
         ops.set_serial(self.serial)
         ops.wgrad_schedule(self.device).reset()
         ops.use_arena(self._arena)
-        self._sync_compute_weights()
+        self._refresh_compute_weights()
         self._dctx = None
         if training:
             self.dropctx.begin()
diff --git a/strajnet_amd/ops.py b/strajnet_amd/ops.py
--- a/strajnet_amd/ops.py
+++ b/strajnet_amd/ops.py
@@ -191,6 +191,34 @@
 
 
 WGRAD_SK = os.environ.get('STJ_WGRAD_SK', '1') != '0'
+TIME_FOLD_MULTI = True
+
+
+class TimeFold:
+
+    def __init__(self, gwz, grad, n):
+        self.gwz, self.grad, self.n = gwz, grad, int(n)
+
+    def __call__(self):
+        call('stj_time_fold', _p(self.gwz), _p(self.grad), self.n, _st())
+
+
+def run_posts(posts):
+    i = 0
+    while i < len(posts):
+        j = i
+        while TIME_FOLD_MULTI and j < len(posts) and j - i < 4 and isinstance(posts[j], TimeFold):
+            j += 1
+        if j - i >= 2:
+            seg = posts[i:j]
+            src = (ctypes.c_void_p * len(seg))(*[f.gwz.data_ptr() for f in seg])
+            dst = (ctypes.c_void_p * len(seg))(*[f.grad.data_ptr() for f in seg])
+            n = (ctypes.c_longlong * len(seg))(*[f.n for f in seg])
+            call('stj_time_fold_multi', src, dst, n, len(seg), _st())
+            i = j
+        else:
+            posts[i]()
+            i += 1
 
 
 class _WgradSchedule:
@@ -262,9 +290,7 @@
         for ev in last.values():
             cur.wait_event(ev)
         wgrad_group([it[0] for it in items])
-        for _, post, _, _ in items:
-            if post is not None:
-                post()
+        run_posts([post for _, post, _, _ in items if post is not None])
 
     def join(self, main, streams, post):
         for s in streams:
@@ -2161,8 +2187,12 @@
             sums = zeros_f32(128 * 40, dev)
             dlogits = torch.empty_like(logits)
             w = (B, H, W, float(ogm_w), float(occ_w), float(fow), float(replica), int(flags))
-            call('stj_loss_fwd_bwd', _p(logits), _p(gt_obs), _p(gt_occ), _p(gt_flow), _p(origin), _p(gate), _p(coef_pre), _p(sums), _p(loss),
-                 _p(coef), _p(dlogits), *w, _st())
+            if LOSS_FINISH_IN_LAUNCH:
+                call('stj_loss_fwd_bwd_fin', _p(logits), _p(gt_obs), _p(gt_occ), _p(gt_flow), _p(origin), _p(gate), _p(coef_pre), _p(sums),
+                     _p(loss), _p(coef), _p(dlogits), *w, _p(_loss_arrive(dev)), _st())
+            else:
+                call('stj_loss_fwd_bwd', _p(logits), _p(gt_obs), _p(gt_occ), _p(gt_flow), _p(origin), _p(gate), _p(coef_pre), _p(sums), _p(loss),
+                     _p(coef), _p(dlogits), *w, _st())
             ctx.unit_grad, ctx.dlogits = unit, dlogits
         else:
             sums = zeros_f32(32 * 40, dev)
@@ -2205,6 +2235,16 @@
 
 LOSS_FUSED_BWD = True
 LOSS_FUSED_STATS = {'hits': 0, 'misses': 0}
+LOSS_FINISH_IN_LAUNCH = False
+_LOSS_ARRIVE = {}
+
+
+def _loss_arrive(device):
+    key = str(device)
+    t = _LOSS_ARRIVE.get(key)
+    if t is None:
+        t = _LOSS_ARRIVE[key] = torch.zeros(_ENUMS['stj_loss']['STJ_LOSS_ARRIVE_INTS'], dtype=torch.int32, device=device)
+    return t
 
 
 def loss_coef(gt_flow, gate, ogm_w, occ_w, fow, replica, flags):
diff --git a/strajnet_amd/optim.py b/strajnet_amd/optim.py
--- a/strajnet_amd/optim.py
+++ b/strajnet_amd/optim.py
@@ -5,19 +5,30 @@
 import torch
 
 from ._lib import ENUMS
-from .ops import _p, _st, call
+from .ops import DTYPE_CODE, _p, _st, call
 
 _OPT = ENUMS['stj_optim']
 LOSS_MEAN_KEYS = ('train_loss', 'train_loss_occ', 'train_loss_flow', 'train_loss_wp')
 
 
+def check_shadow(who, shadow, flat_weights):
+    if shadow is None:
+        return None
+    if shadow.dtype not in (torch.bfloat16, torch.float16) or shadow.shape != flat_weights.shape or shadow.device != flat_weights.device \
+            or not shadow.is_contiguous():
+        raise ValueError(f'{who}: shadow must be a contiguous bfloat16 / float16 tensor of the weights\' shape, on their device')
+    return shadow
+
+
 class Nadam:
-    def __init__(self, flat_weights, flat_grads, lr=1e-4, beta_1=0.9, beta_2=0.999, epsilon=1e-7):
+
+    def __init__(self, flat_weights, flat_grads, lr=1e-4, beta_1=0.9, beta_2=0.999, epsilon=1e-7, shadow=None):
         if flat_weights.dtype != torch.float32 or flat_grads.dtype != torch.float32 or flat_weights.shape != flat_grads.shape:
             raise ValueError('Nadam needs matching flat float32 weight and gradient buffers')
         if not flat_weights.is_cuda:
             raise RuntimeError('Nadam: CUDA (ROCm) buffers only: the HIP path has no CPU fallback')
         self.w, self.g = flat_weights, flat_grads
+        self.shadow = check_shadow('Nadam', shadow, flat_weights)
         self.lr, self.b1, self.b2, self.eps = float(lr), float(beta_1), float(beta_2), float(epsilon)
         self.m = torch.zeros_like(flat_weights)
         self.v = torch.zeros_like(flat_weights)
@@ -26,6 +37,7 @@
 
     @classmethod
     def for_model(cls, model, **kw):
+        kw.setdefault('shadow', model.shadow_for_optimizer())
         return cls(model._flat, model._gflat, **kw)
 
     def _mu(self, t):
@@ -40,6 +52,10 @@
         cg = (1.0 - mu_t) / (1.0 - sched_t)
         cm = mu_n / (1.0 - sched_n)
         vs = 1.0 / (1.0 - self.b2 ** self.t)
+        if self.shadow is not None:
+            call('stj_nadam_step_shadow', _p(self.w), _p(self.g), _p(self.m), _p(self.v), self.w.numel(), self.lr, self.b1, self.b2, self.eps,
+                 cg, cm, vs, float(grad_scale), _p(self.shadow), DTYPE_CODE[self.shadow.dtype], _st())
+            return
         call('stj_nadam_step', _p(self.w), _p(self.g), _p(self.m), _p(self.v), self.w.numel(), self.lr, self.b1, self.b2, self.eps,
              cg, cm, vs, float(grad_scale), _st())
 
@@ -144,9 +160,12 @@
     capturable = True
 
     def __init__(self, flat_weights, flat_grads, lr=1e-4, beta_1=0.9, beta_2=0.999, epsilon=1e-7, global_clipnorm=None, skip_nonfinite=False,
-                 clipnorm=None, locate_nonfinite=False, segments=None):
+                 clipnorm=None, locate_nonfinite=False, segments=None, shadow=None):
         if flat_weights.dtype != torch.float32 or flat_grads.dtype != torch.float32 or flat_weights.shape != flat_grads.shape:
             raise ValueError('DeviceNadam needs matching flat float32 weight and gradient buffers')
+        self.shadow = check_shadow('DeviceNadam', shadow, flat_weights)
+        if self.shadow is not None and (clipnorm is not None or locate_nonfinite):
+            raise ValueError('DeviceNadam: the per-tensor step (clipnorm, locate_nonfinite) does not keep a shadow')
         if not flat_weights.is_cuda or not flat_grads.is_cuda:
             raise RuntimeError('DeviceNadam: CUDA (ROCm) buffers only: the HIP path has no CPU fallback')
         if flat_weights.device != flat_grads.device or not flat_weights.is_contiguous() or not flat_grads.is_contiguous():
@@ -192,6 +211,8 @@
     def for_model(cls, model, **kw):
         if 'segments' not in kw and any(kw.get(k) for k in ('clipnorm', 'locate_nonfinite')):
             kw['segments'] = model_segments(model)
+        per_tensor = kw.get('clipnorm') is not None or bool(kw.get('locate_nonfinite'))
+        kw.setdefault('shadow', model.shadow_for_optimizer(keep=not per_tensor))
         return cls(model._flat, model._gflat, **kw)
 
     iterations = property(lambda self: self.state[0], doc='updates applied (device scalar)')
@@ -243,6 +264,10 @@
         call('stj_nadam_prepare', _p(self.state), _p(self.sched), _p(partials), _p(self.coef), _p(self._losses if means else None),
              _p(self.running if means else None), self.b1, self.b2, float(grad_scale), self.clipnorm, self.loss_scale if means else 1.0,
              _OPT['STJ_NADAM_SKIP_NONFINITE'] if self.skip_nonfinite else 0, st)
+        if self.shadow is not None:
+            call('stj_nadam_apply_shadow', _p(self.w), _p(self.g), _p(self.m), _p(self.v), n, _p(self.coef), self.b1, self.b2, self.eps,
+                 _p(self.shadow), DTYPE_CODE[self.shadow.dtype], st)
+            return
         call('stj_nadam_apply', _p(self.w), _p(self.g), _p(self.m), _p(self.v), n, _p(self.coef), self.b1, self.b2, self.eps, st)
 
     def attach_loss_means(self, losses, loss_scale=1.0):
diff --git a/strajnet_amd/prof.py b/strajnet_amd/prof.py
--- a/strajnet_amd/prof.py
+++ b/strajnet_amd/prof.py
@@ -200,6 +200,9 @@
     'stj_eval_fwd': _eval,
     'stj_nadam_step': _elem('nadam', 4, 0, 7, f32=True),
     'stj_gradnorm_partials': _elem('gradnorm', 1, 0, 1, f32=True), 'stj_nadam_apply': _elem('nadam_apply', 4, 0, 7, f32=True),
+    'stj_cast': _elem('cast', 4, 3, 3),
+    'stj_loss_fwd_bwd_fin': _loss('loss_fwd_bwd', 2),
+    'stj_nadam_step_shadow': _elem('nadam', 4, 0, 7.5, f32=True), 'stj_nadam_apply_shadow': _elem('nadam_apply', 4, 0, 7.5, f32=True),
 }
 EXTRA_MODELS = {}
 
```

New measurement: 1413 scenes/s (median of 6 runs). Within noise of the previous version (+0.3%).
